# szhan227/text2protein

Hardware: AMD Instinct MI355X
Metric: 6D backbone samples/sec (128-res, 1000-step) (higher is better)
Workload: dtype f16; 1 GPU; cfg2: test_config.yml L=128 N=1000 chains/GPU=32 C=5 text_tokens=512 condition=none; step = 1 PC step (2 score evals + SDE updates); sample = 1000 PC steps; finite=True

## Files before the change

include/t2p.h:

```cpp
#ifndef T2P_H_
#define T2P_H_

#include <stdint.h>

#ifdef __cplusplus
extern "C" {
#endif

#define T2P_DTYPE_F32 0
#define T2P_DTYPE_BF16 1
#define T2P_DTYPE_F16 2

#define T2P_SDE_VE 0
#define T2P_SDE_VP 1
#define T2P_SDE_SUBVP 2

typedef struct t2p_model_config {
  int32_t num_channels;
  int32_t max_res_num;
  int32_t nf;
  int32_t num_res_blocks;
  int32_t n_ch_mult;
  int32_t ch_mult[8];
  int32_t n_attn_resolutions;
// ... 92 lines not shown
typedef struct t2p_train_config {
  double lr, beta1, eps, weight_decay;
  double warmup;
  double grad_clip;
  double ema_rate;
  double dropout;
  double t_eps;
  int32_t cond_flags;
  uint64_t seed;
} t2p_train_config;

typedef struct t2p_train_batch {
  const float* coords_6d;
  const uint8_t* mask_pair;
  const uint8_t* mask_inpaint;
  const float* context;
  int32_t batch, tokens;
  const float* t;
  const float* z;
} t2p_train_batch;

typedef struct t2p_trainer t2p_trainer;
int t2p_train_create(const t2p_model_config* model, const t2p_train_config* train, t2p_trainer** out);
void t2p_train_destroy(t2p_trainer* t);
int t2p_train_num_params(const t2p_trainer* t);
int t2p_train_param_info(const t2p_trainer* t, int i, const char** name, int64_t shape[4], int* ndim);
int t2p_train_load_param(t2p_trainer* t, const char* name, const float* host_data, const int64_t* shape, int ndim);
int t2p_train_read(t2p_trainer* t, int which, const char* name, float* host_out);
int t2p_train_write(t2p_trainer* t, int which, const char* name, const float* host_in);
int t2p_train_set_step(t2p_trainer* t, int64_t step, int64_t adam_updates, int64_t ema_updates);
int t2p_train_get_step(const t2p_trainer* t, int64_t out3[3]);
int t2p_train_set_sde(t2p_trainer* t, int sde, double beta_min, double beta_max, const float* std_table);
int t2p_train_set_ploss(t2p_trainer* t, int loss_type, int timesteps, const float* sqrt_alphas_cumprod,
                        const float* sqrt_one_minus_alphas_cumprod);
int t2p_train_set_dropout_masks(t2p_trainer* t, const uint8_t* const* device_masks, int n);
int t2p_train_set_ss_blocks(t2p_trainer* t, const int32_t* host_blocks, int n, const uint8_t* host_drop, double p);
int t2p_train_set_inpaint_draw(t2p_trainer* t, const int32_t* host_len_lo_hi, int B, double random_p, double contiguous_p);
int t2p_train_set_context_drop(t2p_trainer* t, const uint8_t* host_drop, int B, double p);
int t2p_train_loss(t2p_trainer* t, const t2p_train_batch* batch, int backward, float* loss_host, float* score_out, void* stream);
int t2p_train_step(t2p_trainer* t, const t2p_train_batch* batch, float* loss_host, void* stream);
int t2p_train_grad_buffer(t2p_trainer* t, float** device_ptr, int64_t* n);
int t2p_train_apply(t2p_trainer* t, void* stream);
int t2p_train_buffer(t2p_trainer* t, int which, float** device_ptr, int64_t* n);
int t2p_train_copy(t2p_trainer* t, int dst, int src, void* stream);
int t2p_engine_load_from_trainer(t2p_engine* e, t2p_trainer* t, int which, void* stream);
int t2p_train_eval_loss(t2p_trainer* t, const t2p_train_batch* batch, float* loss_host, void* stream);
int64_t t2p_train_device_bytes(const t2p_trainer* t);
int t2p_op_tgemm(const float* A, int64_t sAm, int64_t sAk, const float* B, int64_t sBk, int64_t sBn, float* C, int64_t ldc, int M, int N,
                 int K, int nz, int64_t sAz, int64_t sBz, int64_t sCz, float alpha, float beta, const float* bias_n, int ksplit, int conv,
                 int H, int W, int conv_C, void* stream);
int t2p_op_tgemm16(int dtype, const float* A, int64_t sAm, int64_t sAk, const float* B, int64_t sBk, int64_t sBn, float* C, int64_t ldc,
                   int M, int N, int K, int nz, int64_t sAz, int64_t sBz, int64_t sCz, float alpha, float beta, const float* bias_n, int ksplit,
                   int conv, int H, int W, int conv_C, void* stream);
int t2p_op_train_conv3x3(int dtype, const float* x, const float* w, const float* bias, const float* tbias, int batch, int H, int W, int Ci,
                         int Co, int Cip, int Cop, float* y, const float* dy, float* dx, float* dw, float* dbias, float* dtbias,
                         int fixed_order, void* stream);
int t2p_op_ss_block_dropout(const float* x, float* out, int batch, int C, int L, const int32_t* host_blocks, int n,
                            const uint8_t* host_drop, double p, uint64_t seed, uint64_t stream_id, uint8_t* drop_out_device, void* stream);
int t2p_op_inpaint_mask_draw(const int32_t* host_len_lo_hi, int B, int L, double random_p, double contiguous_p, uint64_t seed, uint64_t stream_id,
                             int force_mode, uint8_t* flags_out, uint8_t* pair_out, int* mode_out_host, void* stream);
int t2p_op_ploss_draw_t(uint64_t seed, uint64_t stream_id, int B, int timesteps, int32_t* out_dev, void* stream);
int t2p_op_context_drop(float* x, int batch, int64_t row_floats, const uint8_t* host_drop, double p, uint64_t seed, uint64_t stream_id,
                        uint8_t* drop_out_device, void* stream);
int t2p_op_groupnorm_backward(const float* x, const float* dy, const float* gamma, const float* beta, int silu, int batch, int HW, int C,
                              int groups, float eps, float* dx, float* dgamma, float* dbeta, void* stream);
int t2p_op_layernorm_backward(const float* x, const float* dy, const float* gamma, int64_t rows, int C, float eps, float* dx, float* dgamma,
                              float* dbeta, void* stream);
int t2p_op_groupnorm_backward_form(const float* x, const float* dy, const float* gamma, const float* beta, int silu, int batch, int HW,
                                   int C, int groups, float eps, float* dx, float* dgamma, float* dbeta, int fixed_order, void* stream);
int t2p_op_layernorm_backward_form(const float* x, const float* dy, const float* gamma, int64_t rows, int C, float eps, float* dx,
                                   float* dgamma, float* dbeta, int fixed_order, void* stream);
int t2p_op_colsum(const float* dy, int nz, int64_t rows_per_z, int N, int64_t ld, float* out, int64_t ld_out, int accumulate,
                  int fixed_order, void* stream);
int t2p_op_sumsq(const float* g, int64_t n, int fixed_order, double* result_host, void* stream);
int t2p_op_seed_scale(const float* x, int64_t n, float target, float* s2_host, void* stream);
int t2p_op_softmax_backward(const float* P, float* dP_inout, int64_t rows, int n, float scale, void* stream);
int t2p_op_geglu_backward(const float* u, const float* dy, float* du, int64_t rows, int inner, void* stream);

int t2p_op_gemm(int dtype, const void* A, int a_f32, const void* Bw, void* C, int c_f32, int M, int N, int K,
                int64_t lda, int64_t ldb, int64_t ldc, const float* bias_n, const float* residual, float alpha,
                void* stream);
int t2p_op_gemm_r16(int dtype, const void* A, int a_f32, const void* Bw, void* C, int c_f32, int M, int N, int K, int64_t lda,
                    int64_t ldb, int64_t ldc, const float* bias_n, const void* residual16, float alpha, void* stream);
int t2p_op_conv3x3(int dtype, const void* x, int a_f32, const void* w, const float* bias, float* out, int batch,
                   int H, int W, int Cin, int Cout, int upsample, void* stream);
int t2p_op_conv3x3_shortcut(int dtype, const void* a, const void* w, const float* bias, const void* x0, int CX0,
                            const void* x1, int CX1, float alpha, void* out, int c_f32, int batch, int H, int W, int C,
                            int Cout, void* stream);
int t2p_op_conv3x3_groupnorm(int dtype, const void* a, const void* w, const float* bias, const float* bias_bn, const void* residual,
                             float alpha, int upsample, int groups, const float* gamma, const float* beta, float eps, int silu,
                             void* out, int out_f32, void* normed, float* col_stats, int batch, int H, int W, int C, int Cout, void* stream);
int t2p_op_small_conv_groupnorm(int dtype, const void* a, const void* w, int64_t ldw, const void* x0, int CX0, const void* x1, int CX1,
                                const float* bias, const float* bias_bn, const void* residual, float alpha, void* out, int out_f32,
                                float* col_stats, void* normed, int groups, const float* gamma, const float* beta, float eps, int silu,
                                int batch, int H, int W, int C, int Cout, void* stream);
int t2p_op_st_entry(int dtype, const void* x, const float* col_stats, int groups, const float* gn_gamma, const float* gn_beta,
                    float gn_eps, const void* w_in, const float* b_in, const void* residual, const float* ln_gamma,
                    const float* ln_beta, float ln_eps, const void* w_2, int n2, const float* b_2, int geglu, void* t, void* out2,
                    const void* w_3, const float* b_3, const void* res3, void* y, float* y_stats, int batch, int n, int C,
                    void* stream);
int t2p_op_attn_proj(int dtype, const void* x, const float* col_stats, int groups, const float* gn_gamma, const float* gn_beta,
                     float gn_eps, const void* w_qk, const float* b_qk, const void* w_v, void* qk, void* vt, void* k_fm,
                     int64_t npad, int batch, int n, int C, void* stream);
int t2p_op_input_conv(const float* x, const float* w_tcn, const float* bias, void* out, int out_dtype, int batch, int C,
                      int H, int W, int nf, float* col_stats, void* stream);
int t2p_op_groupnorm(const float* x0, const float* x1, int C0, int C1, int batch, int H, int W, int groups,
                     const float* gamma, const float* beta, float eps, int silu, int down, void* out, int dtype,
                     void* stream);
int t2p_op_layernorm(const float* x, const float* gamma, const float* beta, void* out, int dtype, int64_t rows,
                     int C, float eps, void* stream);
int t2p_op_layernorm16(const void* x16, const float* gamma, const float* beta, void* out16, int dtype, int64_t rows, int C,
                       float eps, void* stream);
int t2p_op_softmax(const float* S, int64_t lds, void* P, int64_t ldp, int dtype, int64_t rows, int n, float scale,
                   void* stream);
int t2p_op_geglu(const float* u, void* out, int dtype, int64_t rows, int inner, void* stream);
int64_t t2p_op_attention_ws(int dtype, int batch, int heads, int nq, int nk);
int t2p_op_attention(int dtype, const void* q, int64_t ldq, const void* k, int64_t ldk, const void* vt,
                     int64_t ldvt, void* out, int batch, int heads, int nq, int nk, int d, float scale,
                     void* workspace, void* stream);
int t2p_op_attention_wide(int dtype, const void* q, int64_t ldq, const void* k, int64_t ldk, const void* vt, int64_t ldvt, void* out,
                          int out_f32, const float* bias, const void* residual, int residual_16bit, float alpha, float* col_stats,
                          int batch, int n, int d, float scale, void* stream);
int t2p_op_attention_wide_fm(int dtype, const void* q, int64_t ldq, const void* k_fm, const void* vt_fm, void* out, int out_f32,
                             const float* bias, const void* residual, int residual_16bit, float alpha, float* col_stats, int batch,
                             int n, int d, float scale, void* stream);
int t2p_op_gemm_frag_major(int dtype, const void* A, const void* Bw, void* C, void* c_frag, int M, int N, int K, int frag_col0,
                           int rows_per_batch, int batch, void* stream);
int t2p_op_attention_qkv(int dtype, const void* qkv, int64_t ld, void* out, int batch, int heads, int n, int d,
                         float scale, void* stream);
int t2p_op_langevin(const float* x, const float* grad, const float* noise, const uint8_t* mask,
                    const float* x_initial, float* x_out, float* x_mean_out, int batch, int64_t per_sample,
                    float snr, float alpha, float* sums_out , void* stream);
int t2p_op_langevin_norms(const float* grad, const float* noise, int batch, int64_t per_sample, float* workspace,
                          float* sums, void* stream);
int t2p_op_langevin_update(const float* x, const float* grad, const float* noise, const uint8_t* mask,
                           const float* x_initial, float* x_out, float* x_mean_out, int64_t n, const float* sums,
                           float batch_total, float snr, float alpha, void* stream);
int t2p_op_predictor(const float* x, const float* score, const float* noise, const uint8_t* mask,
                     const float* x_initial, float* x_out, float* x_mean_out, int64_t n, float G,
                     int probability_flow, void* stream);
int t2p_op_guided_langevin_norms(const float* o_c, const float* o_u, const float* noise, int batch, int64_t per_sample, float w, float w1,
                                 float scale, float* workspace, float* sums, void* stream);
int t2p_op_guided_langevin_update(const float* x, const float* o_c, const float* o_u, const float* noise, const uint8_t* mask,
                                  const float* x_initial, float* x_out, float* x_out2, float* x_mean_out, int64_t n, float w, float w1,
                                  float scale, const float* sums, float batch_total, float snr, float alpha, void* stream);
int t2p_op_guided_predictor(const float* x, const float* o_c, const float* o_u, const float* noise, const uint8_t* mask,
                            const float* x_initial, float* x_out, float* x_out2, float* x_mean_out, int64_t n, float w, float w1,
                            float scale, float G, float x_coef, int probability_flow, void* stream);
typedef struct t2p_inpaint_replace {
  const uint8_t* known;
  const float* data;
  const float* noise;
  const float* mean_table;
  const float* std_table;
  int32_t n_table;
  int32_t step;
  float mean_coef, std;
  uint64_t seed, stream_id;
} t2p_inpaint_replace;
int t2p_op_inpaint_langevin_update(const float* x, const float* o_c, const float* o_u, const float* noise, const uint8_t* mask,
                                   const float* x_initial, float* x_out, float* x_out2, float* x_mean_out, int64_t n, float w, float w1,
                                   float scale, const float* sums, float batch_total, float snr, float alpha,
                                   const t2p_inpaint_replace* replace, void* stream);
int t2p_op_inpaint_predictor(const float* x, const float* o_c, const float* o_u, const float* noise, const uint8_t* mask,
                             const float* x_initial, float* x_out, float* x_out2, float* x_mean_out, int64_t n, float w, float w1,
                             float scale, float G, float x_coef, int probability_flow, const t2p_inpaint_replace* replace, void* stream);
int t2p_op_philox_normal(float* out, int64_t n, uint64_t seed, uint64_t stream_id, void* stream);
int t2p_op_convert(const float* in, void* out, int dtype, int64_t n, void* stream);
int t2p_op_weight_pack(int kind, const float* src0, const float* src1, const float* src2, void* dst, const int64_t* dims, int ndims, int dtype,
                       void* stream);
int t2p_op_decode_6d(const float* x, int batch, int channels, int L, float* clipped, float* absval, int32_t* lengths, void* stream);
int t2p_op_encode_6d(const float* xyz, const int32_t* nres, const uint8_t* atom_ok, int batch, int channels, int L,
                     const int32_t* host_blocks, int n_blocks, float* coords_6d, uint8_t* mask_pair, void* stream);
int t2p_op_embedding_gather(const void* table, int table_dtype, const int32_t* ids, float* out, int64_t n_tokens, int dim, int vocab,
                            int32_t* bad_flag, void* stream);
int t2p_op_apply_mask(float* x, const uint8_t* mask, const float* x_initial, int64_t n, void* stream);

int t2p_profile_begin(void);
int t2p_debug_set(int key, int value);
int t2p_built_with_ablation(void);
int t2p_profile_end(double* out9);
int t2p_profile_dominant(double* out4, char* name, int name_len);
int t2p_profile_attention(double* out3);
int t2p_profile_shapes(char* buf, int len);
int t2p_profile_conv_kernels(char* buf, int len);
int t2p_debug_tap(int block_index, float* dst, int64_t capacity, int64_t* shape4);
int t2p_profile_layers_begin(void);
int t2p_profile_layers_end(char* buf, int len);

#ifdef __cplusplus
}
#endif
#endif
```

text2protein_amd/_lib.py:

```python
from __future__ import annotations

import ctypes as C

from . import build as _build

DT_F32, DT_BF16, DT_F16 = 0, 1, 2
DTYPE_NAMES = {"f32": DT_F32, "fp32": DT_F32, "float32": DT_F32, "bf16": DT_BF16, "bfloat16": DT_BF16,
               "f16": DT_F16, "fp16": DT_F16, "float16": DT_F16}
SDE_VE, SDE_VP, SDE_SUBVP = 0, 1, 2


class T2PError(RuntimeError):
    pass


class ModelConfig(C.Structure):
    _fields_ = [("num_channels", C.c_int32), ("max_res_num", C.c_int32), ("nf", C.c_int32),
                ("num_res_blocks", C.c_int32), ("n_ch_mult", C.c_int32), ("ch_mult", C.c_int32 * 8),
                ("n_attn_resolutions", C.c_int32), ("attn_resolutions", C.c_int32 * 8),
                ("n_heads", C.c_int32), ("context_dim", C.c_int32), ("num_scales", C.c_int32),
                ("sigma_min", C.c_double), ("sigma_max", C.c_double),
                ("skip_rescale", C.c_int32), ("scale_by_sigma", C.c_int32), ("compute_dtype", C.c_int32)]


# ... 16 lines not shown


class TrainConfig(C.Structure):
    _fields_ = [("lr", C.c_double), ("beta1", C.c_double), ("eps", C.c_double), ("weight_decay", C.c_double),
                ("warmup", C.c_double), ("grad_clip", C.c_double), ("ema_rate", C.c_double), ("dropout", C.c_double),
                ("t_eps", C.c_double), ("cond_flags", C.c_int32), ("seed", C.c_uint64)]


class TrainBatch(C.Structure):
    _fields_ = [("coords_6d", C.c_void_p), ("mask_pair", C.c_void_p), ("mask_inpaint", C.c_void_p), ("context", C.c_void_p),
                ("batch", C.c_int32), ("tokens", C.c_int32), ("t", C.c_void_p), ("z", C.c_void_p)]


class InpaintReplace(C.Structure):
    _fields_ = [("known", C.c_void_p), ("data", C.c_void_p), ("noise", C.c_void_p), ("mean_table", C.c_void_p),
                ("std_table", C.c_void_p), ("n_table", C.c_int32), ("step", C.c_int32), ("mean_coef", C.c_float), ("std", C.c_float),
                ("seed", C.c_uint64), ("stream_id", C.c_uint64)]


_vp, _i, _i64, _f, _u64 = C.c_void_p, C.c_int, C.c_int64, C.c_float, C.c_uint64

SIGNATURES = {
    "t2p_last_error": (C.c_char_p, []),
    "t2p_device_count": (_i, []),
    "t2p_engine_create": (_i, [C.POINTER(ModelConfig), C.POINTER(_vp)]),
    "t2p_engine_destroy": (None, [_vp]),
    "t2p_engine_num_params": (_i, [_vp]),
    "t2p_engine_param_info": (_i, [_vp, _i, C.POINTER(C.c_char_p), C.POINTER(_i64), C.POINTER(_i)]),
    "t2p_engine_load_param": (_i, [_vp, C.c_char_p, _vp, C.POINTER(_i64), _i]),
    "t2p_engine_finalize": (_i, [_vp]),
    "t2p_engine_load_flat": (_i, [_vp, _vp, _i64, _vp]),
    "t2p_engine_load_stats": (_i, [_vp, C.POINTER(_i64)]),
    "t2p_engine_set_context": (_i, [_vp, _vp, _i, _i, _vp]),
    "t2p_engine_score": (_i, [_vp, _vp, _vp, _vp, _i, _vp]),
    "t2p_engine_score_ex": (_i, [_vp, _vp, _vp, _vp, _vp, _i, _vp]),
    "t2p_engine_device_bytes": (_i64, [_vp]),
    "t2p_engine_pool_reclaimed": (_i, [_vp]),
    "t2p_sampler_create": (_i, [_vp, C.POINTER(SamplerConfig), _vp, _vp, C.POINTER(_vp)]),
    "t2p_sampler_set_seed": (_i, [_vp, _u64]),
    "t2p_sampler_set_norm_allreduce": (_i, [_vp, _vp, _vp, _vp]),
    "t2p_built_with_ablation": (_i, []),
    "t2p_sampler_destroy": (None, [_vp]),
    "t2p_sampler_set_condition": (_i, [_vp, _vp, _vp]),
    "t2p_sampler_reset": (_i, [_vp, _i, _vp]),
    "t2p_sampler_step": (_i, [_vp, _vp, _vp, _vp, _vp, _vp]),
    "t2p_sampler_step_graph": (_i, [_vp, _vp, _vp, _vp]),
    "t2p_sampler_run": (_i, [_vp, _vp, _vp, _i, _i, _vp]),
    "t2p_sampler_set_vp_tables": (_i, [_vp, _vp, _vp, _vp, _vp]),
    "t2p_sampler_count_dispatches": (_i, [_vp, _vp, _vp, _vp, C.POINTER(C.c_int)]),
    "t2p_sampler_set_guidance": (_i, [_vp, C.c_double, _i]),
    "t2p_sampler_set_context": (_i, [_vp, _vp, _i, _i, _vp]),
    "t2p_op_guided_langevin_norms": (_i, [_vp, _vp, _vp, _i, _i64, _f, _f, _f, _vp, _vp, _vp]),
    "t2p_op_guided_langevin_update": (_i, [_vp, _vp, _vp, _vp, _vp, _vp, _vp, _vp, _vp, _i64, _f, _f, _f, _vp, _f, _f, _f, _vp]),
    "t2p_op_guided_predictor": (_i, [_vp, _vp, _vp, _vp, _vp, _vp, _vp, _vp, _vp, _i64, _f, _f, _f, _f, _f, _i, _vp]),
    "t2p_sampler_set_inpaint": (_i, [_vp, _vp, _vp, _vp, _vp]),
    "t2p_sampler_set_inpaint_noise": (_i, [_vp, _vp, _vp]),
    "t2p_op_inpaint_langevin_update": (_i, [_vp, _vp, _vp, _vp, _vp, _vp, _vp, _vp, _vp, _i64, _f, _f, _f, _vp, _f, _f, _f,
                                            C.POINTER(InpaintReplace), _vp]),
    "t2p_op_inpaint_predictor": (_i, [_vp, _vp, _vp, _vp, _vp, _vp, _vp, _vp, _vp, _i64, _f, _f, _f, _f, _f, _i,
                                      C.POINTER(InpaintReplace), _vp]),
    "t2p_ddim_create": (_i, [_vp, C.POINTER(DdimConfig), C.POINTER(DdimStepRow), C.POINTER(_vp)]),
    "t2p_ddim_destroy": (None, [_vp]),
    "t2p_ddim_set_seed": (_i, [_vp, _u64]),
    "t2p_ddim_set_condition": (_i, [_vp, _vp, _vp]),
    "t2p_ddim_set_context": (_i, [_vp, _vp, _i, _i, _vp]),
    "t2p_ddim_reset": (_i, [_vp, _i, _vp]),
    "t2p_ddim_step": (_i, [_vp, _vp, _vp, _vp, _vp]),
    "t2p_ddim_run": (_i, [_vp, _vp, _vp, _i, _i, _vp]),
    "t2p_op_ddim_update": (_i, [_vp, _vp, _vp, _vp, _vp, _vp, _vp, _vp, _vp, _i64, _f, _f, _f, _f, _f, _f, _f, _i, _i, _u64, _u64, _vp]),
    "t2p_op_gemm": (_i, [_i, _vp, _i, _vp, _vp, _i, _i, _i, _i, _i64, _i64, _i64, _vp, _vp, _f, _vp]),
    "t2p_op_conv3x3_shortcut": (_i, [_i, _vp, _vp, _vp, _vp, _i, _vp, _i, _f, _vp, _i, _i, _i, _i, _i, _i, _vp]),
    "t2p_op_conv3x3_groupnorm": (_i, [_i, _vp, _vp, _vp, _vp, _vp, C.c_float, _i, _i, _vp, _vp, C.c_float, _i, _vp, _i, _vp, _vp,
                                      _i, _i, _i, _i, _i, _vp]),
    "t2p_op_attention_wide": (_i, [_i, _vp, _i64, _vp, _i64, _vp, _i64, _vp, _i, _vp, _vp, _i, _f, _vp, _i, _i, _i, _f, _vp]),
    "t2p_op_attention_wide_fm": (_i, [_i, _vp, _i64, _vp, _vp, _vp, _i, _vp, _vp, _i, _f, _vp, _i, _i, _i, _f, _vp]),
    "t2p_op_gemm_frag_major": (_i, [_i, _vp, _vp, _vp, _vp, _i, _i, _i, _i, _i, _i, _vp]),
    "t2p_op_small_conv_groupnorm": (_i, [_i, _vp, _vp, _i64, _vp, _i, _vp, _i, _vp, _vp, _vp, _f, _vp, _i, _vp, _vp, _i, _vp, _vp, _f, _i,
                                         _i, _i, _i, _i, _i, _vp]),
    "t2p_op_attn_proj": (_i, [_i, _vp, _vp, _i, _vp, _vp, _f, _vp, _vp, _vp, _vp, _vp, _vp, _i64, _i, _i, _i, _vp]),
    "t2p_op_st_entry": (_i, [_i, _vp, _vp, _i, _vp, _vp, _f, _vp, _vp, _vp, _vp, _vp, _f, _vp, _i, _vp, _i, _vp, _vp, _vp, _vp, _vp, _vp, _vp,
                             _i, _i, _i, _vp]),
    "t2p_op_input_conv": (_i, [_vp, _vp, _vp, _vp, _i, _i, _i, _i, _i, _i, _vp, _vp]),
    "t2p_op_gemm_r16": (_i, [_i, _vp, _i, _vp, _vp, _i, _i, _i, _i, _i64, _i64, _i64, _vp, _vp, _f, _vp]),
    "t2p_op_conv3x3": (_i, [_i, _vp, _i, _vp, _vp, _vp, _i, _i, _i, _i, _i, _i, _vp]),
    "t2p_op_groupnorm": (_i, [_vp, _vp, _i, _i, _i, _i, _i, _i, _vp, _vp, _f, _i, _i, _vp, _i, _vp]),
    "t2p_op_layernorm": (_i, [_vp, _vp, _vp, _vp, _i, _i64, _i, _f, _vp]),
    "t2p_op_layernorm16": (_i, [_vp, _vp, _vp, _vp, _i, _i64, _i, _f, _vp]),
    "t2p_op_softmax": (_i, [_vp, _i64, _vp, _i64, _i, _i64, _i, _f, _vp]),
    "t2p_op_geglu": (_i, [_vp, _vp, _i, _i64, _i, _vp]),
    "t2p_op_attention_ws": (_i64, [_i, _i, _i, _i, _i]),
    "t2p_op_attention_qkv": (_i, [_i, _vp, _i64, _vp, _i, _i, _i, _i, _f, _vp]),
    "t2p_op_attention": (_i, [_i, _vp, _i64, _vp, _i64, _vp, _i64, _vp, _i, _i, _i, _i, _i, _f, _vp, _vp]),
    "t2p_op_langevin": (_i, [_vp, _vp, _vp, _vp, _vp, _vp, _vp, _i, _i64, _f, _f, _vp, _vp]),
    "t2p_op_langevin_norms": (_i, [_vp, _vp, _i, _i64, _vp, _vp, _vp]),
    "t2p_op_langevin_update": (_i, [_vp, _vp, _vp, _vp, _vp, _vp, _vp, _i64, _vp, _f, _f, _f, _vp]),
    "t2p_op_apply_mask": (_i, [_vp, _vp, _vp, _i64, _vp]),
    "t2p_op_predictor": (_i, [_vp, _vp, _vp, _vp, _vp, _vp, _vp, _i64, _f, _i, _vp]),
    "t2p_op_philox_normal": (_i, [_vp, _i64, _u64, _u64, _vp]),
    "t2p_profile_begin": (_i, []),
    "t2p_debug_set": (_i, [_i, _i]),
    "t2p_op_decode_6d": (_i, [_vp, _i, _i, _i, _vp, _vp, _vp, _vp]),
    "t2p_op_encode_6d": (_i, [_vp, _vp, _vp, _i, _i, _i, _vp, _i, _vp, _vp, _vp]),
    "t2p_op_embedding_gather": (_i, [_vp, _i, _vp, _vp, _i64, _i, _i, _vp, _vp]),
    "t2p_profile_end": (_i, [C.POINTER(C.c_double)]),
    "t2p_profile_dominant": (_i, [C.POINTER(C.c_double), C.c_char_p, C.c_int]),
    "t2p_profile_attention": (_i, [C.POINTER(C.c_double)]),
    "t2p_profile_shapes": (_i, [C.c_char_p, C.c_int]),
    "t2p_profile_conv_kernels": (_i, [C.c_char_p, C.c_int]),
    "t2p_debug_tap": (_i, [_i, _vp, C.c_int64, C.POINTER(C.c_int64)]),
    "t2p_profile_layers_begin": (_i, []),
    "t2p_profile_layers_end": (_i, [C.c_char_p, C.c_int]),
    "t2p_op_convert": (_i, [_vp, _vp, _i, _i64, _vp]),
    "t2p_op_weight_pack": (_i, [_i, _vp, _vp, _vp, _vp, C.POINTER(_i64), _i, _i, _vp]),
    "t2p_train_create": (_i, [C.POINTER(ModelConfig), C.POINTER(TrainConfig), C.POINTER(_vp)]),
    "t2p_train_destroy": (None, [_vp]),
    "t2p_train_num_params": (_i, [_vp]),
    "t2p_train_param_info": (_i, [_vp, _i, C.POINTER(C.c_char_p), C.POINTER(_i64), C.POINTER(_i)]),
    "t2p_train_load_param": (_i, [_vp, C.c_char_p, _vp, C.POINTER(_i64), _i]),
    "t2p_train_read": (_i, [_vp, _i, C.c_char_p, _vp]),
    "t2p_train_write": (_i, [_vp, _i, C.c_char_p, _vp]),
    "t2p_train_set_step": (_i, [_vp, _i64, _i64, _i64]),
    "t2p_train_get_step": (_i, [_vp, C.POINTER(_i64)]),
    "t2p_train_set_sde": (_i, [_vp, _i, C.c_double, C.c_double, _vp]),
    "t2p_train_set_ploss": (_i, [_vp, _i, _i, _vp, _vp]),
    "t2p_train_set_dropout_masks": (_i, [_vp, C.POINTER(_vp), _i]),
    "t2p_train_set_ss_blocks": (_i, [_vp, _vp, _i, _vp, C.c_double]),
    "t2p_train_set_inpaint_draw": (_i, [_vp, _vp, _i, C.c_double, C.c_double]),
    "t2p_train_set_context_drop": (_i, [_vp, _vp, _i, C.c_double]),
    "t2p_train_loss": (_i, [_vp, C.POINTER(TrainBatch), _i, C.POINTER(_f), _vp, _vp]),
    "t2p_train_step": (_i, [_vp, C.POINTER(TrainBatch), C.POINTER(_f), _vp]),
    "t2p_train_eval_loss": (_i, [_vp, C.POINTER(TrainBatch), C.POINTER(_f), _vp]),
    "t2p_train_apply": (_i, [_vp, _vp]),
    "t2p_train_grad_buffer": (_i, [_vp, C.POINTER(_vp), C.POINTER(_i64)]),
    "t2p_train_buffer": (_i, [_vp, _i, C.POINTER(_vp), C.POINTER(_i64)]),
    "t2p_train_copy": (_i, [_vp, _i, _i, _vp]),
    "t2p_engine_load_from_trainer": (_i, [_vp, _vp, _i, _vp]),
    "t2p_train_device_bytes": (_i64, [_vp]),
    "t2p_op_tgemm": (_i, [_vp, _i64, _i64, _vp, _i64, _i64, _vp, _i64, _i, _i, _i, _i, _i64, _i64, _i64, _f, _f, _vp, _i, _i, _i, _i, _i, _vp]),
    "t2p_op_tgemm16": (_i, [_i, _vp, _i64, _i64, _vp, _i64, _i64, _vp, _i64, _i, _i, _i, _i, _i64, _i64, _i64, _f, _f, _vp, _i, _i, _i, _i, _i,
                            _vp]),
    "t2p_op_train_conv3x3": (_i, [_i, _vp, _vp, _vp, _vp, _i, _i, _i, _i, _i, _i, _i, _vp, _vp, _vp, _vp, _vp, _vp, _i, _vp]),
    "t2p_op_ss_block_dropout": (_i, [_vp, _vp, _i, _i, _i, _vp, _i, _vp, C.c_double, _u64, _u64, _vp, _vp]),
    "t2p_op_inpaint_mask_draw": (_i, [_vp, _i, _i, C.c_double, C.c_double, _u64, _u64, _i, _vp, _vp, C.POINTER(_i), _vp]),
    "t2p_op_context_drop": (_i, [_vp, _i, _i64, _vp, C.c_double, _u64, _u64, _vp, _vp]),
    "t2p_op_ploss_draw_t": (_i, [_u64, _u64, _i, _i, _vp, _vp]),
    "t2p_op_groupnorm_backward": (_i, [_vp, _vp, _vp, _vp, _i, _i, _i, _i, _i, _f, _vp, _vp, _vp, _vp]),
    "t2p_op_layernorm_backward": (_i, [_vp, _vp, _vp, _i64, _i, _f, _vp, _vp, _vp, _vp]),
    "t2p_op_groupnorm_backward_form": (_i, [_vp, _vp, _vp, _vp, _i, _i, _i, _i, _i, _f, _vp, _vp, _vp, _i, _vp]),
    "t2p_op_layernorm_backward_form": (_i, [_vp, _vp, _vp, _i64, _i, _f, _vp, _vp, _vp, _i, _vp]),
    "t2p_op_colsum": (_i, [_vp, _i, _i64, _i, _i64, _vp, _i64, _i, _i, _vp]),
    "t2p_op_sumsq": (_i, [_vp, _i64, _i, C.POINTER(C.c_double), _vp]),
    "t2p_op_seed_scale": (_i, [_vp, _i64, _f, C.POINTER(_f), _vp]),
    "t2p_op_softmax_backward": (_i, [_vp, _vp, _i64, _i, _f, _vp]),
    "t2p_op_geglu_backward": (_i, [_vp, _vp, _vp, _i64, _i, _vp]),
}

_lib = None


def lib_path() -> str:
    return _build.LIB


ALLREDUCE_FN = C.CFUNCTYPE(C.c_int, C.c_void_p, C.c_void_p, C.c_void_p)


def load_path(path):
    global _lib
    if _lib is not None:
        raise T2PError("load_path() must come before any other use of the library")
    lib = C.CDLL(path)
    for name, (res, args) in SIGNATURES.items():
        fn = getattr(lib, name, None)
        if fn is None:
            continue
        fn.restype = res
        fn.argtypes = args
    _lib = lib
    return lib


def load_ablation():
    global _lib
# ... 56 lines not shown
```

text2protein_amd/build.py:

```python
from __future__ import annotations

import hashlib
import os
import re
import subprocess
import sys

CSRC = os.path.join(os.path.dirname(os.path.abspath(__file__)), "csrc")
LIB = os.path.join(CSRC, "libt2p_hip.so")
LIB_ABLATION = os.path.join(CSRC, "libt2p_hip_ablation.so")
SOURCES = ["gemm.hip", "kernels.hip", "attention.hip", "smallconv.hip", "stfuse.hip", "ddim.hip", "weightpack.hip", "engine.cpp", "sampler.cpp", "capi.cpp",
           "train_kernels.hip", "train.cpp", "train_capi.cpp"]
GEMM_PARTS = 7
HEADERS = ["t2p_common.h", "t2p_kernels.h", "philox.h", "update_loop.h", "engine.h", "sampler.h", "ddim.h", "train_kernels.h", "train.h", os.path.join("..", "..", "include", "t2p.h")]
ARCH = "gfx950"


def _hipcc():
    for c in (os.environ.get("HIPCC"), "/opt/rocm/bin/hipcc", "hipcc"):
        if c and (os.path.isabs(c) and os.path.exists(c) or not os.path.isabs(c)):
            return c
    raise RuntimeError("hipcc not found")


STAMP = LIB + ".srchash"
FLAGS = ["-O3", "-std=c++17", "-fPIC", f"--offload-arch={ARCH}", "-Wall", "-Wno-unused-function"]
_COMPILER_ID = None


def compiler_id() -> str:
    global _COMPILER_ID
    if _COMPILER_ID is None:
        try:
            _COMPILER_ID = subprocess.run([_hipcc(), "--version"], capture_output=True, text=True, timeout=60).stdout.strip()
        except (OSError, RuntimeError, subprocess.SubprocessError):
            _COMPILER_ID = ""
    return _COMPILER_ID


def source_hash(ablation: bool = False) -> str:
    h = hashlib.sha256()
    h.update(" ".join(FLAGS + (["-DT2P_ABLATION"] if ablation else [])).encode())
    h.update(compiler_id().encode())
    for f in SOURCES + HEADERS:
        h.update(f.encode())
        with open(os.path.join(CSRC, f), "rb") as fh:
            h.update(fh.read())
    return h.hexdigest()


def unit_hash(src: str, flags) -> str:
    h = hashlib.sha256()
    h.update(" ".join(flags).encode())
    h.update(compiler_id().encode())
    seen, todo = [], [os.path.join(CSRC, src)]
    while todo:
        f = os.path.normpath(todo.pop())
        if f in seen or not os.path.exists(f):
            continue
        seen.append(f)
        with open(f, "rb") as fh:
            data = fh.read()
        h.update(os.path.relpath(f, CSRC).encode())
        h.update(data)
        for inc in re.findall(rb'^\s*#\s*include\s+"([^"]+)"', data, re.M):
            todo.append(os.path.join(os.path.dirname(f), inc.decode()))
    return h.hexdigest()


def _read(path) -> str:
    try:
        with open(path) as f:
            return f.read().strip()
    except OSError:
        return ""


def built_hash() -> str:
    return _read(STAMP)


def needs_build() -> bool:
    return not os.path.exists(LIB) or built_hash() != source_hash()


def scratch_users(remarks: str, kernel_prefix: str = "_kernel"):
    bad, name = [], None
    for line in remarks.splitlines():
        m = re.search(r"Function Name: (\S+)", line)
        if m:
            name = m.group(1)
        m = re.search(r"ScratchSize \[bytes/lane\]: (\d+)", line)
        if m and name and kernel_prefix in name and int(m.group(1)) > 0:
            bad.append((name, int(m.group(1))))
    return bad


# ... 79 lines not shown
```

text2protein_amd/csrc/capi.cpp:

```cpp
#include <new>

#include "ddim.h"
#include "engine.h"
#include "sampler.h"
#include "train.h"

using namespace t2p;

#define API_BEGIN try {
#define API_END                                        \
  }                                                    \
  catch (const std::bad_alloc&) {                      \
    set_last_error("out of host memory");              \
    return T2P_ERR_STATE;                              \
  }                                                    \
  catch (const std::exception& ex) {                   \
    set_last_error(std::string("exception: ") + ex.what()); \
    return T2P_ERR_STATE;                              \
  }

namespace t2p { extern bool g_pre_conv_mfma, g_gn_apply_cols; void layer_profile_begin(); int layer_profile_end(std::string* out);
void debug_tap_set(int index, float* dst, long capacity); void debug_tap_shape(long out[4]); }
extern "C" {

// ... 211 lines not shown

int t2p_sampler_run(t2p_sampler* s, float* x, float* out, int prior_given, int n_steps, void* stream) {
  API_BEGIN
  T2P_REQUIRE(s, "null sampler");
  return s->impl.run(x, out, prior_given, n_steps, (hipStream_t)stream);
  API_END
}

int t2p_ddim_create(t2p_engine* e, const t2p_ddim_config* cfg, const t2p_ddim_step_row* table, t2p_ddim** out) {
  API_BEGIN
  T2P_REQUIRE(e && cfg && out, "null argument");
  t2p_ddim* d = new t2p_ddim(&e->impl, *cfg);
  int rc = d->impl.init(table);
  if (rc != T2P_OK) {
    delete d;
    return rc;
  }
  *out = d;
  return T2P_OK;
  API_END
}

void t2p_ddim_destroy(t2p_ddim* d) { delete d; }

int t2p_ddim_set_seed(t2p_ddim* d, uint64_t seed) {
  API_BEGIN
  T2P_REQUIRE(d, "null ddim sampler");
  d->impl.set_seed(seed);
  return T2P_OK;
  API_END
}

int t2p_ddim_set_condition(t2p_ddim* d, const uint8_t* mask, const float* x_initial) {
  API_BEGIN
  T2P_REQUIRE(d, "null ddim sampler");
  T2P_REQUIRE((mask == nullptr) == (x_initial == nullptr), "mask and x_initial go together");
  return d->impl.set_condition(mask, x_initial);
  API_END
}

int t2p_ddim_set_context(t2p_ddim* d, const float* context, int batch, int tokens, void* stream) {
  API_BEGIN
  T2P_REQUIRE(d, "null ddim sampler");
  return d->impl.set_context(context, batch, tokens, (hipStream_t)stream);
  API_END
}

int t2p_ddim_reset(t2p_ddim* d, int step, void* stream) {
  API_BEGIN
  T2P_REQUIRE(d, "null ddim sampler");
  (void)stream;
  return d->impl.reset(step);
  API_END
}

int t2p_ddim_step(t2p_ddim* d, float* x, float* x0_out, const float* noise, void* stream) {
  API_BEGIN
  T2P_REQUIRE(d, "null ddim sampler");
  return d->impl.step(x, x0_out, noise, (hipStream_t)stream);
  API_END
}

int t2p_ddim_run(t2p_ddim* d, float* x, float* out, int prior_given, int n_steps, void* stream) {
  API_BEGIN
  T2P_REQUIRE(d, "null ddim sampler");
  return d->impl.run(x, out, prior_given, n_steps, (hipStream_t)stream);
  API_END
}

int t2p_op_ddim_update(const float* x, const float* eps_c, const float* eps_u, const float* z, const uint8_t* mask,
                       const float* x_initial, float* x_out, float* x_out2, float* x0_out, int64_t n, float w, float w1,
                       float sqrt_recip, float sqrt_recipm1, float sqrt_an, float c, float sigma, int clip, int last,
                       uint64_t seed, uint64_t stream_id, void* stream) {
  API_BEGIN
  DdimUpdateArgs a;
  a.x = x; a.eps_c = eps_c; a.eps_u = eps_u; a.z = z; a.mask = mask; a.x_initial = x_initial;
  a.x_out = x_out; a.x_out2 = x_out2; a.x0_out = x0_out; a.n = n; a.w = w; a.w1 = w1;
  a.sqrt_recip = sqrt_recip; a.sqrt_recipm1 = sqrt_recipm1; a.sqrt_an = sqrt_an; a.c = c; a.sigma = sigma;
  a.clip = clip; a.last = last; a.seed = seed; a.stream_id = stream_id;
  return launch_ddim_update(a, (hipStream_t)stream);
  API_END
}

int t2p_op_gemm(int dtype, const void* A, int a_f32, const void* Bw, void* C, int c_f32, int M, int N, int K, int64_t lda,
                int64_t ldb, int64_t ldc, const float* bias_n, const float* residual, float alpha, void* stream) {
  API_BEGIN
  GemmParams p;
  p.dtype = dtype; p.A0 = A; p.a_f32 = a_f32; p.C0 = K; p.lda0 = lda; p.Bw = Bw; p.ldb = ldb; p.M = M; p.N = N;
  p.bias_n = bias_n; p.R = residual; p.ldr = ldc; p.alpha = alpha; p.C = C; p.c_f32 = c_f32; p.ldc = ldc;
  return launch_gemm(p, (hipStream_t)stream);
  API_END
}

static void* g_op_ws = nullptr;
static size_t g_op_ws_bytes = 0, g_op_ws_alloc = 0;
static int attach_op_ws(GemmParams& p) {
  if (!g_op_ws_bytes) return T2P_OK;
  if (g_op_ws_alloc < g_op_ws_bytes) {
    if (g_op_ws) { T2P_HIP_CHECK(hipDeviceSynchronize()); T2P_HIP_CHECK(hipFree(g_op_ws)); g_op_ws = nullptr; g_op_ws_alloc = 0; }
    T2P_HIP_CHECK(hipMalloc(&g_op_ws, g_op_ws_bytes));
    g_op_ws_alloc = g_op_ws_bytes;
  }
  p.ws = g_op_ws; p.ws_bytes = g_op_ws_bytes;
  return T2P_OK;
}

int t2p_op_gemm_r16(int dtype, const void* A, int a_f32, const void* Bw, void* C, int c_f32, int M, int N, int K, int64_t lda,
                    int64_t ldb, int64_t ldc, const float* bias_n, const void* residual16, float alpha, void* stream) {
  API_BEGIN
  GemmParams p;
  p.dtype = dtype; p.A0 = A; p.a_f32 = a_f32; p.C0 = K; p.lda0 = lda; p.Bw = Bw; p.ldb = ldb; p.M = M; p.N = N;
  p.bias_n = bias_n; p.R = (const float*)residual16; p.r_lowp = 1; p.ldr = ldc; p.alpha = alpha; p.C = C; p.c_f32 = c_f32; p.ldc = ldc;
  T2P_TRY(attach_op_ws(p));
  return launch_gemm(p, (hipStream_t)stream);
  API_END
}

int t2p_op_conv3x3(int dtype, const void* x, int a_f32, const void* w, const float* bias, float* out, int batch, int H,
                   int W, int Cin, int Cout, int upsample, void* stream) {
  API_BEGIN
  GemmParams p;
  p.dtype = dtype; p.A0 = x; p.a_f32 = a_f32; p.C0 = Cin; p.lda0 = Cin; p.taps = 9; p.H = H; p.W = W; p.a_up = upsample;
  p.Bw = w; p.ldb = 9L * Cin; p.M = batch * H * W; p.N = Cout; p.bias_n = bias; p.rows_per_batch = H * W;
  p.C = out; p.c_f32 = 1; p.ldc = Cout;
  T2P_TRY(attach_op_ws(p));
  return launch_gemm(p, (hipStream_t)stream);
  API_END
}

int t2p_op_conv3x3_shortcut(int dtype, const void* a, const void* w, const float* bias, const void* x0, int CX0, const void* x1,
                            int CX1, float alpha, void* out, int c_f32, int batch, int H, int W, int C, int Cout, void* stream) {
  API_BEGIN
  GemmParams p;
  p.dtype = dtype; p.A0 = a; p.a_f32 = 0; p.C0 = C; p.lda0 = C; p.taps = 9; p.H = H; p.W = W;
  p.Bw = w; p.ldb = 9L * C + CX0 + CX1; p.M = batch * H * W; p.N = Cout; p.bias_n = bias; p.rows_per_batch = H * W;
  p.alpha = alpha; p.C = out; p.c_f32 = c_f32; p.ldc = Cout;
  T2P_TRY(attach_op_ws(p));
  T2P_REQUIRE(gemm_can_fuse_shortcut(p), "this convolution does not take the shortcut segment (LDS-DMA 3x3 convolutions only)");
  p.X0 = x0; p.CX0 = CX0; p.ldx0 = CX0; p.X1 = x1; p.CX1 = CX1; p.ldx1 = CX1;
  return launch_gemm(p, (hipStream_t)stream);
  API_END
}

int t2p_op_conv3x3_groupnorm(int dtype, const void* a, const void* w, const float* bias, const float* bias_bn, const void* residual,
                             float alpha, int upsample, int groups, const float* gamma, const float* beta, float eps, int silu,
                             void* out, int out_f32, void* normed, float* col_stats, int batch, int H, int W, int C, int Cout, void* stream) {
  API_BEGIN
  GemmParams p;
  p.dtype = dtype; p.A0 = a; p.a_f32 = 0; p.C0 = C; p.lda0 = C; p.taps = 9; p.H = H; p.W = W; p.a_up = upsample;
  p.Bw = w; p.ldb = 9L * C; p.M = batch * H * W; p.N = Cout; p.bias_n = bias; p.rows_per_batch = H * W;
  p.bias_bn = bias_bn; p.ld_bn = Cout;
  p.R = (const float*)residual; p.r_lowp = residual ? 1 : 0; p.ldr = Cout;
  p.alpha = alpha; p.C = out; p.c_f32 = out_f32; p.ldc = Cout; p.col_stats = col_stats;
  T2P_TRY(attach_op_ws(p));
  T2P_REQUIRE(gemm_fuses_post_gn(p, groups), "this convolution does not take the split-K plan whose second pass applies a GroupNorm");
  p.gn_gamma = gamma; p.gn_beta = beta; p.gn_groups = groups; p.gn_silu = silu; p.gn_eps = eps; p.gn_out = normed;
  return launch_gemm(p, (hipStream_t)stream);
  API_END
}

int t2p_op_small_conv_groupnorm(int dtype, const void* a, const void* w, int64_t ldw, const void* x0, int CX0, const void* x1, int CX1,
                                const float* bias, const float* bias_bn, const void* residual, float alpha, void* out, int out_f32,
                                float* col_stats, void* normed, int groups, const float* gamma, const float* beta, float eps, int silu,
                                int batch, int H, int W, int C, int Cout, void* stream) {
  API_BEGIN
  SmallConvArgs s;
  s.dtype = dtype; s.A = a; s.B = batch; s.H = H; s.W = W; s.C = C; s.N = Cout; s.Wt = w; s.ldw = ldw;
  s.X0 = x0; s.CX0 = CX0; s.X1 = x1; s.CX1 = CX1; s.bias = bias; s.bias_bn = bias_bn; s.ld_bn = Cout; s.R = residual; s.alpha = alpha;
  s.out = out; s.out_f32 = out_f32; s.col_stats = col_stats; s.normed = normed; s.gn_gamma = gamma; s.gn_beta = beta; s.groups = groups;
  s.gn_silu = silu; s.gn_eps = eps;
  return launch_small_conv_gn(s, (hipStream_t)stream);
  API_END
}

int t2p_op_st_entry(int dtype, const void* x, const float* col_stats, int groups, const float* gn_gamma, const float* gn_beta, float gn_eps,
                    const void* w_in, const float* b_in, const void* residual, const float* ln_gamma, const float* ln_beta, float ln_eps,
                    const void* w_qkv, int n2, const float* b2, int geglu, void* t, void* qkv, const void* w3, const float* b3,
                    const void* res3, void* y, float* y_stats, int batch, int n, int C, void* stream) {
  API_BEGIN
  StEntryArgs e;
  e.dtype = dtype; e.B = batch; e.n = n; e.C = C; e.x = x; e.cstats = col_stats; e.groups = groups; e.gn_gamma = gn_gamma;
  e.gn_beta = gn_beta; e.gn_eps = gn_eps; e.w_in = w_in; e.b_in = b_in; e.ln_gamma = ln_gamma; e.ln_beta = ln_beta; e.ln_eps = ln_eps;
  e.w_qkv = w_qkv; e.n2 = n2; e.b2 = b2; e.geglu = geglu; e.res = residual; e.t = t; e.qkv = qkv;
  e.w3 = w3; e.b3 = b3; e.res3 = res3; e.y = y; e.y_stats = y_stats;
  T2P_REQUIRE(st_entry_eligible(e), "st_entry: C = 256 (or 512 without geglu), n2 in {C, 3 C} (8 C with geglu), 16-bit dtype, n % 32 == 0 (64 with column sums), batch n <= 8192");
  void* fm = nullptr;
  T2P_HIP_CHECK(hipMalloc(&fm, ((size_t)C * C + (size_t)n2 * C + (w3 ? (size_t)5 * C * C : 0)) * 2));
  void* fm2 = (char*)fm + (size_t)C * C * 2;
  void* fm3 = (char*)fm2 + (size_t)n2 * C * 2;
  int rc = launch_sf_frag_major(dtype, w_in, fm, C, C, (hipStream_t)stream);
  if (rc == T2P_OK) rc = launch_sf_frag_major(dtype, w_qkv, fm2, n2, C, (hipStream_t)stream);
  if (rc == T2P_OK && w3) rc = launch_sf_frag_major(dtype, w3, fm3, C, 5 * C, (hipStream_t)stream);
  if (rc == T2P_OK && w3 && y_stats && hipMemsetAsync(y_stats, 0, (size_t)batch * n / 64 * C * 2 * 4, (hipStream_t)stream) != hipSuccess) rc = T2P_ERR_HIP;
  e.w_in = fm; e.w_qkv = fm2;
  if (w3) e.w3 = fm3;
  if (rc == T2P_OK) rc = launch_st_entry(e, (hipStream_t)stream);
// ... 325 lines not shown
  a.x = x; a.noise = noise; a.mask = mask; a.x_initial = x_initial; a.x_out = x_out; a.x_mean_out = x_mean_out; a.n = n;
  GuidedScore g;
  g.o_c = o_c; g.o_u = o_u; g.w = w; g.w1 = w1; g.scale = scale;
  InpaintReplace r;
  int* counter = nullptr;
  int rc = op_inpaint_replace(replace, &r, &counter, s);
  if (rc == T2P_OK) rc = launch_predictor_update(a, g, x_out2, nullptr, G, probability_flow, s, nullptr, x_coef, &r);
  return op_inpaint_done(rc, counter, s);
  API_END
}

int t2p_op_philox_normal(float* out, int64_t n, uint64_t seed, uint64_t stream_id, void* stream) {
  API_BEGIN
  return launch_philox_normal(out, n, seed, stream_id, nullptr, (hipStream_t)stream);
  API_END
}

int t2p_op_convert(const float* in, void* out, int dtype, int64_t n, void* stream) {
  API_BEGIN
  return launch_convert(in, out, dtype, n, (hipStream_t)stream);
  API_END
}

int t2p_op_decode_6d(const float* x, int batch, int channels, int L, float* clipped, float* absval, int32_t* lengths, void* stream) {
  API_BEGIN
  return launch_decode6d(x, batch, channels, L, clipped, absval, lengths, (hipStream_t)stream);
  API_END
}

int t2p_op_encode_6d(const float* xyz, const int32_t* nres, const uint8_t* atom_ok, int batch, int channels, int L,
                     const int32_t* host_blocks, int n_blocks, float* coords_6d, uint8_t* mask_pair, void* stream) {
  API_BEGIN
  T2P_REQUIRE(xyz && nres && coords_6d && mask_pair && batch > 0 && L > 0, "encode_6d arguments");
  T2P_REQUIRE(channels == 5 || channels == 8, "encode_6d: the channel count must be 5 or 8, not " + std::to_string(channels));
  T2P_REQUIRE(n_blocks >= 0 && (n_blocks == 0 || host_blocks), "encode_6d: block list arguments");
  T2P_REQUIRE(n_blocks == 0 || channels == 8, "encode_6d: secondary-structure blocks need the 8-channel layout");
  T2P_REQUIRE((long)L * L < (1L << 30) && batch <= 65535, "encode_6d: map or batch too large");
  hipStream_t s = (hipStream_t)stream;
  std::vector<int32_t> n((size_t)batch);
  T2P_HIP_CHECK(hipMemcpyAsync(n.data(), nres, (size_t)batch * 4, hipMemcpyDeviceToHost, s));
  T2P_HIP_CHECK(hipStreamSynchronize(s));
  for (int b = 0; b < batch; ++b)
    T2P_REQUIRE(n[b] >= 1 && n[b] <= L, "encode_6d: nres[" + std::to_string(b) + "] = " + std::to_string(n[b]) + " is outside [1, " + std::to_string(L) + "]");
  std::vector<std::vector<int32_t>> of_sample((size_t)batch);
  for (int k = 0; k < n_blocks; ++k) {
    const int32_t* q = host_blocks + 4 * (size_t)k;
    const std::string name = "encode_6d: block " + std::to_string(k);
    T2P_REQUIRE(q[0] >= 0 && q[0] < batch, name + " names a sample outside the batch");
    T2P_REQUIRE(q[1] <= q[2], name + " starts after its last residue");
    T2P_REQUIRE(q[1] >= 0 && q[2] < n[q[0]], name + " lies outside the " + std::to_string(n[q[0]]) + " residues of its sample");
    T2P_REQUIRE(q[3] == 0 || q[3] == 1, name + " is neither a helix (0) nor a strand (1)");
    of_sample[q[0]].push_back(k);
  }
  if (n_blocks == 0) return launch_encode6d(xyz, nres, atom_ok, batch, channels, L, nullptr, nullptr, 0, coords_6d, mask_pair, s);
  std::vector<int32_t> up(host_blocks, host_blocks + 4 * (size_t)n_blocks);
  for (const auto& ks : of_sample)
    for (int32_t k1 : ks)
      for (int32_t k2 : ks) { up.push_back(k1); up.push_back(k2); }
  const size_t npairs = (up.size() - 4 * (size_t)n_blocks) / 2;
  T2P_REQUIRE(npairs < (1u << 30), "encode_6d: too many block pairs");
  struct Scratch {
    int32_t* p = nullptr; hipStream_t s;
    ~Scratch() { if (p) { (void)hipStreamSynchronize(s); (void)hipFree(p); } }
  } dev;
  dev.s = s;
  T2P_HIP_CHECK(hipMalloc(&dev.p, up.size() * 4));
  T2P_HIP_CHECK(hipMemcpyAsync(dev.p, up.data(), up.size() * 4, hipMemcpyHostToDevice, s));
  return launch_encode6d(xyz, nres, atom_ok, batch, channels, L, dev.p, dev.p + 4 * (size_t)n_blocks, (int)npairs, coords_6d, mask_pair, s);
  API_END
}

int t2p_op_embedding_gather(const void* table, int table_dtype, const int32_t* ids, float* out, int64_t n_tokens, int dim, int vocab,
                            int32_t* bad_flag, void* stream) {
  API_BEGIN
  return launch_embedding_gather(table, table_dtype, ids, out, n_tokens, dim, vocab, bad_flag, (hipStream_t)stream);
  API_END
}

int t2p_op_apply_mask(float* x, const uint8_t* mask, const float* x_initial, int64_t n, void* stream) {
  API_BEGIN
  return launch_apply_mask(x, mask, x_initial, n, (hipStream_t)stream);
  API_END
}

int t2p_debug_set(int key, int value) {
  if (key == 10) { g_op_ws_bytes = (size_t)value << 20; return T2P_OK; }
  if (key == 11) { set_gemm_force_nsplit(value); return T2P_OK; }
  if (key == 12) { set_gemm_midsplit(value != 0); return T2P_OK; }
  if (key == 13) { g_gn_small = value != 0; return T2P_OK; }
  if (key == 14) { g_lowp_residual = value != 0; return T2P_OK; }
  if (key == 15) { set_gemm_thin_conv(value != 0); return T2P_OK; }
  if (key == 17) { g_gn_apply16 = value != 0; return T2P_OK; }
  if (key == 20) { g_layernorm16 = value != 0; return T2P_OK; }
  if (key == 21) { set_gemm_up4(value != 0); return T2P_OK; }
  if (key == 22) { set_gemm_deep_ring(value != 0); return T2P_OK; }
  if (key == 23) { set_gemm_fuse_shortcut(value != 0); return T2P_OK; }
  if (key == 25) { g_qkv_fused = value != 0; return T2P_OK; }
  if (key == 26) { t2p::g_pre_conv_mfma = value != 0; return T2P_OK; }
  if (key == 27) { t2p::g_gn_apply_cols = value != 0; return T2P_OK; }
  if (key == 28) { set_gemm_post_gn(value != 0); return T2P_OK; }
  if (key == 29) { t2p::g_attn_strip = value != 0; return T2P_OK; }
  if (key == 36) { t2p::g_small_conv = value != 0; return T2P_OK; }
  if (key == 38) { t2p::g_pre_conv_split = value != 0; return T2P_OK; }
  if (key == 39) { t2p::g_st_fuse = value != 0; return T2P_OK; }
  if (key == 40) { t2p::g_st_tail = value != 0; return T2P_OK; }
  if (key == 41) { t2p::g_small_conv_fm = value != 0; return T2P_OK; }
  if (key == 42) { t2p::g_st_ffpo = value != 0; return T2P_OK; }
  if (key == 43) { t2p::g_st_tail_rows = value; return T2P_OK; }
  if (key == 45) { t2p::g_attn_fm = value != 0; return T2P_OK; }
  if (key == 46) { t2p::g_attn_proj = value != 0; return T2P_OK; }
  if (key == 47) { set_gemm_dxs(value != 0); return T2P_OK; }
  if (key == 48) { t2p::g_train_plumbing16 = value != 0; return T2P_OK; }
  if (key == 34) { set_gemm_a_norm(value != 0); return T2P_OK; }
  if (key == 32) { g_attn_merged = value != 0; return T2P_OK; }
  if (key == 33) { g_ffpo_merged = value != 0; return T2P_OK; }
  if (key == 30) { set_gemm_split_consts(value, 0); return T2P_OK; }
  if (key == 31) { set_gemm_split_consts(0, value); return T2P_OK; }
  if (key == 0) set_gemm_dma(value != 0);
  else if (key == 1) {
#ifndef T2P_ABLATION
    if (value & ~(128 | 256 | 4096 | 8192)) {
      set_last_error("ablation bits that skip work exist only in a -DT2P_ABLATION build");
      return T2P_ERR_INVALID;
    }
#endif
    set_gemm_debug(value);
  }
  else if (key == 2) set_gemm_geom(value);
  else if (key == 3) set_gemm_splitk(value != 0);
  else if (key == 4) g_raw_copies = value != 0;
  else if (key == 5) g_flash_attention = value != 0;
  else if (key == 6) g_fuse_gn_stats = value != 0;
  else if (key == 7) g_fuse_geglu = value != 0;
  else if (key == 8) set_gemm_ring(value);
  else if (key == 9) g_lowp_h1 = value != 0;
  else return T2P_ERR_INVALID;
  return T2P_OK;
}

#ifdef T2P_ABLATION
extern "C" int t2p_ablation_dxs_stamps(unsigned long long* out, int n) { return t2p::dxs_stamps_read(out, n); }
#endif

int t2p_built_with_ablation(void) {
#ifdef T2P_ABLATION
  return 1;
#else
  return 0;
#endif
}

int t2p_profile_begin(void) {
  profile_begin();
  return T2P_OK;
}

int t2p_profile_end(double* out9) {
  API_BEGIN
  T2P_REQUIRE(out9, "null argument");
  double o[3][3];
  T2P_TRY(profile_end(o));
  for (int k = 0; k < 3; ++k)
    for (int j = 0; j < 3; ++j) out9[k * 3 + j] = o[k][j];
  return T2P_OK;
  API_END
}

int t2p_profile_attention(double* out3) {
  API_BEGIN
  T2P_REQUIRE(out3, "null argument");
  return profile_attention(out3);
  API_END
}

int t2p_profile_shapes(char* buf, int len) {
  API_BEGIN
  T2P_REQUIRE(buf && len > 0, "null argument");
  return profile_shapes(buf, len);
  API_END
}

int t2p_profile_conv_kernels(char* buf, int len) {
  API_BEGIN
  T2P_REQUIRE(buf && len > 0, "null argument");
  return profile_conv_kernels(buf, len);
  API_END
}

int t2p_debug_tap(int block_index, float* dst, int64_t capacity, int64_t* shape4) {
  API_BEGIN
  if (shape4) {
    long sh[4];
    t2p::debug_tap_shape(sh);
    for (int i = 0; i < 4; ++i) shape4[i] = sh[i];
  }
// ... 33 lines not shown
```

text2protein_amd/csrc/engine.cpp:

```cpp
#include "engine.h"

#include <algorithm>
#include <cmath>
#include <cstdio>
#include <cstring>
#include <map>
#include <mutex>
#include <thread>

namespace t2p {

bool g_fuse_gn_stats = true;
bool g_fuse_geglu = true;
bool g_lowp_h1 = true;
bool g_gn_small = true;
bool g_lowp_residual = true;
bool g_raw_copies = true;
bool g_flash_attention = true;
bool g_attn_merged = true;
bool g_ffpo_merged = true;
bool g_qkv_fused = true;
static thread_local std::string g_last_error;
void set_last_error(const std::string& msg) { g_last_error = msg; }
const char* get_last_error() { return g_last_error.c_str(); }
// ... 406 lines not shown
              for (int64_t n = 0; n < co; ++n)
                for (int64_t c = 0; c < ci; ++c)
                  m[((ph * co + n) * 4 + tap) * ci + c] += s[0][(((size_t)n * ci + c) * 3 + kh) * 3 + kw];
            }
      break;
    }
    case WP_ADD:
      m.resize((size_t)d[0]);
      for (int64_t i = 0; i < d[0]; ++i) m[i] = s[0][i] + s[1][i];
      break;
    case WP_PRODUCT: {
      const int64_t M = d[0], K = d[1], N = d[2];
      m = host_matmul(s[0], s[1], M, K, N);
      if (s[2])
        for (int64_t i = 0; i < M; ++i)
          for (int64_t n = 0; n < N; ++n) m[i * N + n] += s[2][n];
      if (d[3]) {
        std::vector<float> t((size_t)M * N);
        for (int64_t i = 0; i < M; ++i)
          for (int64_t n = 0; n < N; ++n) t[n * M + i] = m[i * N + n];
        m.swap(t);
      }
      break;
    }
    case WP_DOT64: {
      const int64_t N = d[0], K = d[1];
      m.resize((size_t)N);
      for (int64_t n = 0; n < N; ++n) {
        double acc = s[2][n];
        for (int64_t j = 0; j < K; ++j) acc += (double)s[0][n * K + j] * s[1][j];
        m[n] = (float)acc;
      }
      break;
    }
  }
}

int Engine::dest(void** slot, size_t bytes) {
  if (!*slot) *slot = pool_.persistent(bytes);
  return *slot ? T2P_OK : T2P_ERR_HIP;
}

const float* Engine::psrc(const std::string& name, int64_t numel) {
  auto it = poff_.find(name);
  if (it == poff_.end() || it->second.second != numel) {
    set_last_error((it == poff_.end() ? "no parameter " : "unexpected shape for ") + name);
    return nullptr;
  }
  if (flat_) return flat_ + it->second.first;
  auto h = host_.find(name);
  if (h == host_.end() || (int64_t)h->second.data.size() != numel) {
    set_last_error("parameter not loaded: " + name);
    return nullptr;
  }
  return h->second.data.data();
}
#define T2P_SRC(var, name, numel)                         \
  const float* var = psrc((name), (int64_t)(numel));      \
  if (!var) return T2P_ERR_STATE;

int Engine::pack(int kind, void* dst, int64_t off, int dtype, std::initializer_list<const float*> srcs, std::initializer_list<int64_t> dims) {
  WeightPack p;
  p.kind = kind; p.dtype = dtype; p.dst = (char*)dst + (size_t)off * dtype_size(dtype);
  int i = 0;
  for (const float* s : srcs) p.src[i++] = s;
  i = 0;
  for (int64_t d : dims) p.d[i++] = d;
  int64_t rows = 0, width = 0, ld = 0, rd = 0, wr = 0;
  T2P_TRY(weight_pack_shape(p, &rows, &width, &ld));
  weight_pack_bytes(p, rows, width, &rd, &wr);
  load_stats_[0] += rd; load_stats_[1] += wr; load_stats_[2] += 1;
  if (flat_) return launch_weight_pack(p, pack_stream_);
  std::vector<float> m;
  weight_pack_host(p, &m);
  return upload_block(m, dtype, p.dst, rows, width, ld);
}

int Engine::pack_frag(void** slot, const void* w, int N, int K) {
  T2P_TRY(dest(slot, (size_t)N * K * 2));
  load_stats_[0] += (int64_t)N * K * 2; load_stats_[1] += (int64_t)N * K * 2; load_stats_[2] += 1;
  return launch_sf_frag_major(cfg_.compute_dtype, w, *slot, N, K, pack_stream_);
}

int Engine::pack_linear(const std::string& wname, const std::string& bname, int N, int K, DevLinear* out, bool conv3x3, bool nin,
                        int force_dtype, int cin_pad) {
  const int dt = force_dtype >= 0 ? force_dtype : cfg_.compute_dtype;
  const int ci = K / 9, cp = cin_pad ? cin_pad : ci;
  const int Kd = conv3x3 ? 9 * cp : K;
  T2P_SRC(w, wname, (int64_t)N * K);
  T2P_TRY(dest(&out->w, (size_t)N * Kd * dtype_size(dt)));
  if (conv3x3) T2P_TRY(pack(WP_CONV3, out->w, 0, dt, {w}, {N, ci, cp, 0}));
  else if (nin) T2P_TRY(pack(WP_NIN, out->w, 0, dt, {w}, {K, N, 1}));
  else T2P_TRY(pack(WP_COPY, out->w, 0, dt, {w}, {(int64_t)N * K}));
  out->N = N;
  out->K = Kd;
  if (!bname.empty()) {
    T2P_SRC(b, bname, N);
    T2P_TRY(dest((void**)&out->b, (size_t)N * 4));
    T2P_TRY(pack(WP_COPY, out->b, 0, DT_F32, {b}, {N}));
  }
  return T2P_OK;
}

int Engine::pack_stack2(const std::string& w0, const std::string& b0, const std::string& w1, const std::string& b1,
                        int N, int K, bool nin, bool has_bias, DevLinear* out) {
  const int dt = cfg_.compute_dtype;
  T2P_SRC(t0, w0, (int64_t)N * K);
  T2P_SRC(t1, w1, (int64_t)N * K);
  T2P_TRY(dest(&out->w, (size_t)2 * N * K * dtype_size(dt)));
  if (nin) T2P_TRY(pack(WP_NIN, out->w, 0, dt, {t0, t1}, {K, N, 2}));
  else T2P_TRY(pack(WP_COPY, out->w, 0, dt, {t0, t1}, {(int64_t)N * K, (int64_t)N * K}));
  out->N = 2 * N;
  out->K = K;
  if (has_bias) {
    T2P_SRC(c0, b0, N);
    T2P_SRC(c1, b1, N);
    T2P_TRY(dest((void**)&out->b, (size_t)2 * N * 4));
    T2P_TRY(pack(WP_COPY, out->b, 0, DT_F32, {c0, c1}, {N, N}));
  }
  return T2P_OK;
}

int Engine::pack_norm(const std::string& prefix, int C, int G, DevNorm* out) {
  T2P_SRC(g, prefix + ".weight", C);
  T2P_SRC(b, prefix + ".bias", C);
  T2P_TRY(dest((void**)&out->gamma, (size_t)C * 4));
  T2P_TRY(dest((void**)&out->beta, (size_t)C * 4));
  T2P_TRY(pack(WP_COPY, out->gamma, 0, DT_F32, {g}, {C}));
  T2P_TRY(pack(WP_COPY, out->beta, 0, DT_F32, {b}, {C}));
  out->C = C;
  out->G = G;
  return T2P_OK;
}

int Engine::pack_weights() {
  load_stats_[0] = load_stats_[1] = load_stats_[2] = 0;
  const int td = arch_.temb_dim, dt = cfg_.compute_dtype, nf = arch_.nf, Cx = cfg_.num_channels;
  const size_t es = dtype_size(dt);
  T2P_TRY(pack_linear("pre_blocks.0.weight", "pre_blocks.0.bias", td, nf, &pre0_, false, false, DT_F32));
  T2P_TRY(pack_linear("pre_blocks.1.weight", "pre_blocks.1.bias", td, td, &pre1_, false, false, DT_F32));
  T2P_TRY(pack_linear("pre_conv.weight", "pre_conv.bias", nf, 9 * Cx, &pre_conv_, true, false, DT_F32, cpad_));
  {
    T2P_SRC(w, "pre_conv.weight", (int64_t)nf * Cx * 9);
    T2P_TRY(dest((void**)&pre_conv_direct_, (size_t)9 * Cx * nf * 4));
    T2P_TRY(pack(WP_CONV3_T, pre_conv_direct_, 0, DT_F32, {w}, {nf, Cx}));
    if (dt != DT_F32 && (Cx == 5 || Cx == 8) && cfg_.sigma_max <= 4096.0) {
      T2P_TRY(dest(&pre_conv_split_, pre_conv_split_weight_bytes(Cx, nf)));
      T2P_TRY(launch_pre_conv_split_weights(pre_conv_direct_, pre_conv_split_, Cx, nf, pack_stream_));
      load_stats_[0] += (int64_t)9 * Cx * nf * 4; load_stats_[1] += (int64_t)pre_conv_split_weight_bytes(Cx, nf); load_stats_[2] += 1;
    }
  }
  T2P_TRY(dest(&dense_all_.w, (size_t)arch_.temb_total * td * 4));
  T2P_TRY(dest((void**)&dense_all_.b, (size_t)arch_.temb_total * 4));
  dense_all_.N = arch_.temb_total;
  dense_all_.K = td;
  auto each_layer = [&](auto&& fn) -> int {
    for (Stage& st : arch_.input_stages) for (Layer& l : st.layers) T2P_TRY(fn(l));
    for (Layer& l : arch_.mid_stage.layers) T2P_TRY(fn(l));
    for (Stage& st : arch_.out_stages) for (Layer& l : st.layers) T2P_TRY(fn(l));
    return T2P_OK;
  };
  T2P_TRY(each_layer([&](Layer& l) -> int {
    const std::string& p = l.prefix;
    const int ci = l.in_ch, co = l.out_ch;
    if (l.kind == 0) {
      T2P_TRY(pack_norm(p + ".GroupNorm_0", ci, gn_groups(ci), &l.gn0));
// ... 12 lines not shown
        T2P_SRC(b1, p + ".Conv_1.bias", co);
        T2P_SRC(b2, p + ".Conv_2.bias", co);
        const int64_t K1 = (int64_t)9 * co, Kx = K1 + ci;
        T2P_TRY(dest(&l.conv1x.w, (size_t)co * Kx * es));
        T2P_TRY(dest((void**)&l.conv1x.b, (size_t)co * 4));
        T2P_TRY(pack(WP_CONV3, l.conv1x.w, 0, dt, {w1}, {co, co, co, Kx}));
        T2P_TRY(pack(WP_ROWS, l.conv1x.w, K1, dt, {w2}, {co, ci, Kx}));
        T2P_TRY(pack(WP_ADD, l.conv1x.b, 0, DT_F32, {b1, b2}, {co}));
        l.conv1x.N = co; l.conv1x.K = (int)Kx;
      }
      T2P_SRC(w, p + ".Dense_0.weight", (int64_t)co * td);
      T2P_SRC(b, p + ".Dense_0.bias", co);
      T2P_TRY(pack(WP_COPY, dense_all_.w, (int64_t)l.temb_off * td, DT_F32, {w}, {(int64_t)co * td}));
      T2P_TRY(pack(WP_COPY, dense_all_.b, l.temb_off, DT_F32, {b}, {co}));
      if (l.fm_conv0) {
        const DevLinear& c1 = l.has_conv2 ? l.conv1x : l.conv1;
        T2P_TRY(pack_frag(&l.fm_conv0, l.conv0.w, co, l.conv0.K));
        T2P_TRY(pack_frag(&l.fm_conv1, c1.w, co, c1.K));
      }
    } else if (l.kind == 1) {
      T2P_TRY(pack_norm(p + ".GroupNorm_0", ci, gn_groups(ci), &l.gn0));
      T2P_TRY(pack_stack2(p + ".NIN_0.W", p + ".NIN_0.b", p + ".NIN_1.W", p + ".NIN_1.b", ci, ci, true, true, &l.qk));
      T2P_TRY(pack_linear(p + ".NIN_2.W", p + ".NIN_2.b", ci, ci, &l.v, false, true));
      T2P_TRY(pack_linear(p + ".NIN_3.W", p + ".NIN_3.b", ci, ci, &l.out, false, true));
      if (dt != DT_F32) {
        T2P_SRC(w2, p + ".NIN_2.W", (int64_t)ci * ci);
        T2P_SRC(w3, p + ".NIN_3.W", (int64_t)ci * ci);
        T2P_SRC(b2, p + ".NIN_2.b", ci);
        T2P_SRC(b3, p + ".NIN_3.b", ci);
        T2P_TRY(dest(&l.v3.w, (size_t)ci * ci * es));
        T2P_TRY(dest((void**)&l.v3.b, (size_t)ci * 4));
        T2P_TRY(pack(WP_PRODUCT, l.v3.w, 0, dt, {w2, w3}, {ci, ci, ci, 1, 0}));
        T2P_TRY(pack(WP_PRODUCT, l.v3.b, 0, DT_F32, {b2, w3, b3}, {1, ci, ci, 0, 0}));
        l.v3.N = ci; l.v3.K = ci;
        if (ci == 256 && l.qk.w && l.qk.b) {
          T2P_TRY(pack_frag(&l.fm_qk, l.qk.w, 2 * ci, ci));
          T2P_TRY(pack_frag(&l.fm_v3, l.v3.w, ci, ci));
        }
      }
    } else {
      const std::string t = p + ".transformer_blocks.0";
      const int ctx = cfg_.context_dim;
      T2P_TRY(pack_norm(p + ".norm", ci, 32, &l.gn0));
      T2P_TRY(pack_linear(p + ".proj_in.weight", p + ".proj_in.bias", ci, ci, &l.proj_in));
      T2P_TRY(pack_linear(p + ".proj_out.weight", p + ".proj_out.bias", ci, ci, &l.proj_out));
      T2P_TRY(pack_stack2(t + ".attn1.to_q.weight", "", t + ".attn1.to_k.weight", "", ci, ci, false, false, &l.a1_qk));
      T2P_TRY(pack_linear(t + ".attn1.to_v.weight", "", ci, ci, &l.a1_v));
      if (dt != DT_F32) {
        const int64_t cc = (int64_t)ci * ci;
        T2P_SRC(wq, t + ".attn1.to_q.weight", cc);
        T2P_SRC(wk, t + ".attn1.to_k.weight", cc);
        T2P_SRC(wv, t + ".attn1.to_v.weight", cc);
        T2P_TRY(dest(&l.a1_qkv.w, (size_t)3 * cc * es));
        T2P_TRY(pack(WP_COPY, l.a1_qkv.w, 0, dt, {wq, wk, wv}, {cc, cc, cc}));
        l.a1_qkv.N = 3 * ci; l.a1_qkv.K = ci; l.a1_qkv.b = nullptr;
      }
      T2P_TRY(pack_linear(t + ".attn1.to_out.0.weight", t + ".attn1.to_out.0.bias", ci, ci, &l.a1_out));
      T2P_TRY(pack_linear(t + ".attn2.to_q.weight", "", ci, ci, &l.a2_q));
      T2P_TRY(pack_linear(t + ".attn2.to_k.weight", "", ci, ctx, &l.a2_k));
      T2P_TRY(pack_linear(t + ".attn2.to_v.weight", "", ci, ctx, &l.a2_v));
      T2P_TRY(pack_linear(t + ".attn2.to_out.0.weight", t + ".attn2.to_out.0.bias", ci, ci, &l.a2_out));
      {
        const int64_t inner = 4 * ci;
        T2P_SRC(w, t + ".ff.net.0.proj.weight", 2 * inner * ci);
        T2P_SRC(b, t + ".ff.net.0.proj.bias", 2 * inner);
        T2P_TRY(dest(&l.ff1.w, (size_t)2 * inner * ci * es));
        T2P_TRY(dest((void**)&l.ff1.b, (size_t)2 * inner * 4));
        T2P_TRY(pack(WP_GEGLU, l.ff1.w, 0, dt, {w}, {inner, ci}));
        T2P_TRY(pack(WP_GEGLU, l.ff1.b, 0, DT_F32, {b}, {inner, 1}));
        l.ff1.N = 8 * ci;
        l.ff1.K = ci;
      }
      T2P_TRY(pack_linear(t + ".ff.net.2.weight", t + ".ff.net.2.bias", ci, 4 * ci, &l.ff2));
      if (dt != DT_F32 && ci == 256 && l.a1_qkv.w) {
        T2P_TRY(pack_frag(&l.fm_in, l.proj_in.w, ci, ci));
        T2P_TRY(pack_frag(&l.fm_qkv, l.a1_qkv.w, 3 * ci, ci));
        T2P_TRY(pack_frag(&l.fm_out1, l.a1_out.w, ci, ci));
        T2P_TRY(pack_frag(&l.fm_q2, l.a2_q.w, ci, ci));
        if (ci == 256) {
          T2P_TRY(pack_frag(&l.fm_out2, l.a2_out.w, ci, ci));
          T2P_TRY(pack_frag(&l.fm_ff1, l.ff1.w, 8 * ci, ci));
        }
      }
      if (dt != DT_F32 && ci % 64 == 0) {
        T2P_SRC(wpo, p + ".proj_out.weight", (int64_t)ci * ci);
        T2P_SRC(bpo, p + ".proj_out.bias", ci);
        T2P_SRC(wf, t + ".ff.net.2.weight", (int64_t)ci * 4 * ci);
        T2P_SRC(bf, t + ".ff.net.2.bias", ci);
        T2P_TRY(dest(&l.ffpo.w, (size_t)ci * 5 * ci * es));
        T2P_TRY(dest((void**)&l.ffpo.b, (size_t)ci * 4));
        T2P_TRY(pack(WP_PRODUCT, l.ffpo.w, 0, dt, {wpo, wf}, {ci, ci, 4 * ci, 0, 5 * ci}));
        T2P_TRY(pack(WP_ROWS, l.ffpo.w, 4 * ci, dt, {wpo}, {ci, ci, 5 * ci}));
        T2P_TRY(pack(WP_DOT64, l.ffpo.b, 0, DT_F32, {wpo, bf, bpo}, {ci, ci}));
        l.ffpo.N = ci; l.ffpo.K = 5 * ci;
        if (ci == 256 && l.fm_in) T2P_TRY(pack_frag(&l.fm_ffpo, l.ffpo.w, ci, 5 * ci));
      }
      T2P_TRY(pack_norm(t + ".norm1", ci, 1, &l.ln1));
      T2P_TRY(pack_norm(t + ".norm2", ci, 1, &l.ln2));
      T2P_TRY(pack_norm(t + ".norm3", ci, 1, &l.ln3));
    }
    return T2P_OK;
  }));
  T2P_TRY(pack_norm("out.0", arch_.final_ch, gn_groups(arch_.final_ch), &head_norm_));
  T2P_TRY(pack_linear("out.2.weight", "out.2.bias", Cx, 9 * arch_.final_ch, &head_conv_, true));

  if (!inv_sigma_) {
    const int N = cfg_.num_scales;
    std::vector<float> inv(N);
    const double a = std::log(cfg_.sigma_max), b = std::log(cfg_.sigma_min);
    for (int i = 0; i < N; ++i) {
      const double s = std::exp(a + (b - a) * (double)i / (double)(N - 1));
      inv[i] = (float)(1.0 / s);
    }
    T2P_TRY(dest((void**)&inv_sigma_, (size_t)N * 4));
    T2P_TRY(dest((void**)&unit_scale_, (size_t)N * 4));
    T2P_TRY(upload_block(inv, DT_F32, inv_sigma_, 1, N, N));
    T2P_TRY(upload_block(std::vector<float>(N, 1.f), DT_F32, unit_scale_, 1, N, N));
  }
  return T2P_OK;
}

int Engine::finalize() {
  T2P_REQUIRE(!finalized_, "engine already finalized");
  for (const ParamInfo& p : arch_.params) {
    if (!host_.count(p.name)) {
      set_last_error("parameter not loaded: " + p.name);
      return T2P_ERR_STATE;
    }
  }
  flat_ = nullptr;
  pack_stream_ = nullptr;
  T2P_TRY(pack_weights());
  T2P_HIP_CHECK(hipStreamSynchronize(nullptr));
  host_.clear();
  finalized_ = true;
  return T2P_OK;
}

int Engine::load_flat(const float* device_flat, int64_t n, hipStream_t s) {
  T2P_REQUIRE(device_flat, "load_flat: null buffer");
  T2P_REQUIRE(n == total_, "load_flat: n must equal the element count of the engine's parameter table (" + std::to_string(total_) + ")");
  int dev = -1;
  T2P_HIP_CHECK(hipGetDevice(&dev));
  T2P_REQUIRE(dev == device_, "load_flat: the engine lives on device " + std::to_string(device_) + ", the current device is " + std::to_string(dev));
  flat_ = device_flat;
  pack_stream_ = s;
  const int rc = pack_weights();
  flat_ = nullptr;
  pack_stream_ = nullptr;
  T2P_TRY(rc);
  host_.clear();
  finalized_ = true;
  ctx_B_ = 0;
  return T2P_OK;
}

int Engine::attach_ws(GemmParams& p) {
  if (!splitk_ws_) {
    splitk_ws_bytes_ = (size_t)256 << 20;
    splitk_ws_ = pool_.persistent(splitk_ws_bytes_);
    if (!splitk_ws_) return T2P_ERR_HIP;
  }
  p.ws = splitk_ws_;
  p.ws_bytes = splitk_ws_bytes_;
  return T2P_OK;
}

int Engine::gemm(GemmParams& p, hipStream_t s) {
  T2P_TRY(attach_ws(p));
  return launch_gemm(p, s);
}

int Engine::gemm_stats(GemmParams& p, float** cstats, hipStream_t s) {
  *cstats = nullptr;
  T2P_TRY(attach_ws(p));
  if (g_fuse_gn_stats && (gemm_fuses_col_stats(p) || gemm_fuses_col_stats_lowp(p))) {
    *cstats = (float*)pool_.get((size_t)(p.M / 64) * p.N * 2 * 4);
    if (!*cstats) return T2P_ERR_HIP;
    p.col_stats = *cstats;
  }
  return gemm(p, s);
}

int Engine::linear(const void* a, bool a_is_f32, const DevLinear& w, long rows, void* c, bool c_f32,
                   const float* residual, float alpha, hipStream_t s, bool use_bias, float** cstats, bool r_lowp) {
  GemmParams p;
  p.dtype = dtype();
  p.A0 = a; p.a_f32 = a_is_f32 || p.dtype == DT_F32; p.C0 = w.K; p.lda0 = w.K;
  p.Bw = w.w; p.ldb = w.K;
  p.M = (int)rows; p.N = w.N;
  p.bias_n = use_bias ? w.b : nullptr;
  p.R = residual; p.ldr = w.N; p.r_lowp = (residual && r_lowp) ? 1 : 0;
  p.alpha = alpha;
  p.C = c; p.c_f32 = c_f32; p.ldc = w.N;
  if (cstats) return gemm_stats(p, cstats, s);
  return gemm(p, s);
}

int Engine::group_norm(const Act& x, const Act* x1, const DevNorm& n, float eps, int silu, int down, int B, void** out,
                       hipStream_t s, void** raw_out) {
  const int C = x.C + (x1 ? x1->C : 0);
  T2P_REQUIRE(C == n.C, "GroupNorm channel mismatch");
  T2P_REQUIRE(!x1 || x1->lowp == x.lowp, "concatenated sources must share a storage type");
  T2P_REQUIRE(!x.lowp || dtype() != DT_F32, "16-bit activations exist in the 16-bit modes only");
  if (x.pre_norm && !x1 && x.pre_for == &n && x.pre_silu == silu && !down && !raw_out) {
    *out = x.pre_norm;
    x.pre_norm = nullptr;
    return T2P_OK;
  }
  {
    GroupNormApplyArgs g;
    g.x0 = (const float*)x.p; g.x1 = x1 ? (const float*)x1->p : nullptr; g.C0 = x.C; g.C1 = x1 ? x1->C : 0;
    g.B = B; g.H = x.H; g.W = x.W; g.G = n.G; g.gamma = n.gamma; g.beta = n.beta; g.silu = silu; g.down = down;
    g.dtype = dtype(); g.x0_lowp = x.lowp; g.eps = eps;
    if (g_gn_small && gn_small_eligible(g)) {
      const size_t bytes = (size_t)B * x.H * x.W * C * dtype_size(dtype());
      POOL_GET(o, void*, bytes);
      g.out = o;
      if (raw_out) {
        *raw_out = pool_.get(bytes);
        if (!*raw_out) return T2P_ERR_HIP;
        g.raw_out = *raw_out;
      }
      T2P_TRY(launch_gn_small(g, s));
      *out = o;
      return T2P_OK;
    }
  }
  GroupNormArgs a;
  a.x0 = x.p; a.x1 = x1 ? x1->p : nullptr; a.C0 = x.C; a.C1 = x1 ? x1->C : 0;
  a.B = B; a.HW = x.H * x.W; a.G = n.G; a.eps = eps;
  const bool have_cols = x.cstats && (!x1 || x1->cstats) && a.HW % 64 == 0;
  if (have_cols && !raw_out) {
    GroupNormApplyArgs g;
    g.x0 = a.x0; g.x1 = a.x1; g.C0 = a.C0; g.C1 = a.C1; g.B = B; g.H = x.H; g.W = x.W; g.G = n.G;
    g.gamma = n.gamma; g.beta = n.beta; g.silu = silu; g.down = down; g.dtype = dtype(); g.x0_lowp = x.lowp;
    g.cs0 = x.cstats; g.cs1 = x1 ? x1->cstats : nullptr; g.eps = eps;
    if (gn_apply_cols_eligible(g)) {
      POOL_GET(o, void*, (size_t)B * a.HW * C * dtype_size(dtype()));
      g.out = o;
      T2P_TRY(launch_gn_apply_cols(g, s));
      *out = o;
      return T2P_OK;
    }
  }
  const int nparts = gn_num_chunks(a.HW) * ((C + 1023) / 1024);
  POOL_GET(stats, float*, (size_t)B * n.G * 2 * 4);
  float* partial = nullptr;
  if (have_cols) {
    T2P_TRY(launch_gn_finalize_cols(x.cstats, x1 ? x1->cstats : nullptr, a.C0, a.C1, B, a.HW, n.G, eps, stats, s));
  } else {
    partial = (float*)pool_.get((size_t)B * nparts * n.G * 2 * 4);
    if (!partial) return T2P_ERR_HIP;
    a.partial = partial; a.stats = stats;
    a.lowp_dtype = x.lowp ? dtype() : DT_F32;
    T2P_TRY(launch_gn_stats(a, s));
  }
  GroupNormApplyArgs g;
  g.x0 = a.x0; g.x1 = a.x1; g.C0 = a.C0; g.C1 = a.C1; g.B = B; g.H = x.H; g.W = x.W; g.G = n.G;
  g.stats = stats; g.gamma = n.gamma; g.beta = n.beta; g.silu = silu; g.down = down; g.dtype = dtype();
  g.x0_lowp = x.lowp;
  const size_t opix = (size_t)B * (down ? x.H / 2 : x.H) * (down ? x.W / 2 : x.W);
  POOL_GET(o, void*, opix * C * dtype_size(dtype()));
  g.out = o;
  if (raw_out) {
    *raw_out = pool_.get(opix * C * dtype_size(dtype()));
    if (!*raw_out) return T2P_ERR_HIP;
    g.raw_out = *raw_out;
  }
  T2P_TRY(launch_gn_apply(g, s));
  pool_.put(partial);
  pool_.put(stats);
// ... 399 lines not shown
    StEntryArgs e;
    e.dtype = dt; e.B = B; e.n = n; e.C = C;
    const bool normed = x.pre_norm && x.pre_for == &L.gn0 && x.pre_silu == 0;
    e.x = normed ? x.pre_norm : (const void*)x.p;
    e.cstats = normed ? nullptr : x.cstats;
    e.gn_gamma = L.gn0.gamma; e.gn_beta = L.gn0.beta; e.groups = L.gn0.G; e.gn_eps = 1e-6f;
    e.w_in = L.fm_in; e.b_in = L.proj_in.b;
    e.ln_gamma = L.ln1.gamma; e.ln_beta = L.ln1.beta; e.ln_eps = 1e-5f;
    e.w_qkv = L.fm_qkv; e.n2 = 3 * C;
    void* a_small = nullptr;
    if (!normed && !x.cstats && L.proj_in.b && L.fm_in && g_st_fuse) {
      StEntryArgs probe = e;
      probe.x = x.p; probe.cstats = nullptr;
      if (st_entry_eligible(probe)) {
        T2P_TRY(group_norm(x, nullptr, L.gn0, 1e-6f, 0, 0, B, &a_small, s));
        e.x = a_small; e.cstats = nullptr;
      }
    }
    if ((normed || x.cstats || a_small) && L.proj_in.b && L.fm_in && st_entry_eligible(e)) {
      qkv_pre = (char*)pool_.get((size_t)rows * 3 * C * es);
      if (!qkv_pre) return T2P_ERR_HIP;
      if (mega) {
        y2 = (float*)pool_.get((size_t)rows * C * es);
        if (!y2) return T2P_ERR_HIP;
        if (g_fuse_gn_stats) {
          y2_stats = (float*)pool_.get((size_t)(rows / 64) * C * 2 * 4);
          if (!y2_stats) return T2P_ERR_HIP;
          e.zero = y2_stats; e.zero_n = (long)(rows / 64) * C * 2;
        }
      }
      e.t = t; e.qkv = qkv_pre;
      T2P_TRY(launch_st_entry(e, s));
      if (normed) { pool_.put(x.pre_norm); x.pre_norm = nullptr; }
    }
    pool_.put(a_small);
  }
  if (!qkv_pre) {
    void* a = nullptr;
    T2P_TRY(group_norm(x, nullptr, L.gn0, 1e-6f, 0, 0, B, &a, s));
    T2P_TRY(linear(a, false, L.proj_in, rows, t, !tl, nullptr, 1.f, s));
    pool_.put(a);
  }
  POOL_GET(ln, void*, (size_t)rows * C * es);
  POOL_GET(o, void*, (size_t)rows * C * es);
  if (!qkv_pre) T2P_TRY(launch_layernorm(t, L.ln1.gamma, L.ln1.beta, ln, dt, rows, C, 1e-5f, s, tl));
  if (qkv_flash) {
    char* qkv = qkv_pre;
    if (!qkv) {
      qkv = (char*)pool_.get((size_t)rows * 3 * C * es);
      if (!qkv) return T2P_ERR_HIP;
      T2P_TRY(linear(ln, false, L.a1_qkv, rows, qkv, false, nullptr, 1.f, s, false));
    }
    T2P_TRY(launch_attention_flash(dt, qkv, 3 * C, qkv + (size_t)C * es, 3 * C, qkv + (size_t)2 * C * es, 3 * C, o, B, heads, n, n, d, scale, s,
                                   true));
    pool_.put(qkv);
  } else {
    POOL_GET(qk, char*, (size_t)rows * 2 * C * es);
    T2P_TRY(linear(ln, false, L.a1_qk, rows, qk, false, nullptr, 1.f, s, false));
    POOL_GET(vt, void*, (size_t)B * C * npad * es);
    T2P_TRY(project_vt(dt, L.a1_v, ln, C, B, n, npad, vt, s));
    T2P_TRY(attention(qk, 2 * C, qk + (size_t)C * es, 2 * C, vt, npad, o, B, heads, n, n, d, scale, s));
    pool_.put(qk);
    pool_.put(vt);
  }
  {
    POOL_GET(q, void*, (size_t)rows * C * es);
    StEntryArgs e;
    e.dtype = dt; e.B = B; e.n = n; e.C = C; e.x = o; e.w_in = L.fm_out1; e.b_in = L.a1_out.b; e.res = t;
    e.ln_gamma = L.ln2.gamma; e.ln_beta = L.ln2.beta; e.ln_eps = 1e-5f; e.w_qkv = L.fm_q2; e.n2 = C; e.t = t; e.qkv = q;
    if (tl && qkv_pre && L.a1_out.b && !L.a2_q.b && st_entry_eligible(e)) {
      T2P_TRY(launch_st_entry(e, s));
    } else {
      T2P_TRY(linear(o, false, L.a1_out, rows, t, !tl, t, 1.f, s, true, nullptr, tl));
      T2P_TRY(launch_layernorm(t, L.ln2.gamma, L.ln2.beta, ln, dt, rows, C, 1e-5f, s, tl));
      T2P_TRY(linear(ln, false, L.a2_q, rows, q, false, nullptr, 1.f, s, false));
    }
    T2P_TRY(attention(q, C, L.ctx_k, C, L.ctx_vt, ctx_Tpad_, o, B, heads, n, ctx_T_, d, scale, s));
    pool_.put(q);
  }
  {
    POOL_GET(g, void*, (size_t)rows * 4 * C * es);
    GemmParams p;
    p.dtype = dt; p.A0 = ln; p.a_f32 = dt == DT_F32; p.C0 = C; p.lda0 = C;
    p.Bw = L.ff1.w; p.ldb = C; p.M = (int)rows; p.N = 8 * C; p.bias_n = L.ff1.b;
    p.C = g; p.c_f32 = 0; p.ldc = 4 * C; p.geglu = 1;
    T2P_TRY(attach_ws(p));
    StEntryArgs e;
    e.dtype = dt; e.B = B; e.n = n; e.C = C; e.x = o; e.w_in = L.fm_out2; e.b_in = L.a2_out.b; e.res = t;
    e.ln_gamma = L.ln3.gamma; e.ln_beta = L.ln3.beta; e.ln_eps = 1e-5f; e.w_qkv = L.fm_ff1; e.b2 = L.ff1.b; e.n2 = 8 * C; e.geglu = 1;
    e.t = t; e.qkv = g;
    const bool tail_chain = tl && qkv_pre && g_st_tail && (y2 || rows >= 2 * g_st_tail_rows) && L.fm_ff1 && g_fuse_geglu && gemm_fuses_geglu(p) && L.a2_out.b && L.ff1.b && st_entry_eligible(e);
    if (tail_chain && y2) {
      e.w3 = L.fm_ffpo; e.b3 = L.ffpo.b; e.res3 = x.p; e.y = y2; e.y_stats = y2_stats; e.qkv = nullptr;
      T2P_REQUIRE(st_entry_eligible(e), "row chain with the third product");
      T2P_TRY(launch_st_entry(e, s));
      pool_.put(g); pool_.put(o); pool_.put(ln); pool_.put(t);
      *out = Act{y2, C, x.H, x.W, y2_stats, true};
      return T2P_OK;
    }
    if (y2) { pool_.put(y2); pool_.put(y2_stats); y2 = nullptr; y2_stats = nullptr; }
    if (tail_chain) {
      T2P_TRY(launch_st_entry(e, s));
    } else {
      T2P_TRY(linear(o, false, L.a2_out, rows, t, !tl, t, 1.f, s, true, nullptr, tl));
      T2P_TRY(launch_layernorm(t, L.ln3.gamma, L.ln3.beta, ln, dt, rows, C, 1e-5f, s, tl));
    }
    if (tail_chain) {
    } else if (g_fuse_geglu && gemm_fuses_geglu(p)) {
      T2P_TRY(gemm(p, s));
    } else {
      POOL_GET(u, float*, (size_t)rows * 8 * C * 4);
      T2P_TRY(linear(ln, false, L.ff1, rows, u, true, nullptr, 1.f, s));
      T2P_TRY(launch_geglu(u, g, dt, rows, 4 * C, s, 1));
      pool_.put(u);
    }
    if (g_ffpo_merged && tl && L.ffpo.w) {
      pool_.put(o);
      const bool olp2 = res_lowp();
      POOL_GET(y2, float*, (size_t)rows * C * (olp2 ? es : 4));
      float* y2_stats = nullptr;
      GemmParams q;
      q.dtype = dt; q.a_f32 = 0; q.A0 = g; q.C0 = 4 * C; q.lda0 = 4 * C; q.A1 = t; q.C1 = C; q.lda1 = C;
      q.Bw = L.ffpo.w; q.ldb = L.ffpo.K; q.M = (int)rows; q.N = C; q.bias_n = L.ffpo.b;
      q.R = x.p; q.ldr = C; q.r_lowp = x.lowp ? 1 : 0;
      q.C = y2; q.c_f32 = olp2 ? 0 : 1; q.ldc = C; q.rows_per_batch = n;
      T2P_TRY(gemm_stats(q, &y2_stats, s));
      pool_.put(g);
      pool_.put(ln);
      pool_.put(t);
      *out = Act{y2, C, x.H, x.W, y2_stats, olp2};
      return T2P_OK;
    }
    T2P_TRY(linear(g, false, L.ff2, rows, t, !tl, t, 1.f, s, true, nullptr, tl));
    pool_.put(g);
  }
  pool_.put(o);
  const bool olp = res_lowp();
  POOL_GET(y, float*, (size_t)rows * C * (olp ? es : 4));
  float* y_stats = nullptr;
  if (tl) {
    T2P_TRY(linear(t, false, L.proj_out, rows, y, !olp, x.p, 1.f, s, true, &y_stats, x.lowp));
  } else if (dt != DT_F32 && g_raw_copies) {
    T2P_TRY(launch_convert(t, ln, dt, rows * C, s));
    T2P_TRY(linear(ln, false, L.proj_out, rows, y, !olp, x.p, 1.f, s, true, &y_stats, x.lowp));
  } else {
    T2P_TRY(linear(t, true, L.proj_out, rows, y, !olp, x.p, 1.f, s, true, &y_stats, x.lowp));
  }
  pool_.put(ln);
  pool_.put(t);
  *out = Act{y, C, x.H, x.W, y_stats, olp};
  return T2P_OK;
}

static NormHint first_norm_of(const Layer* l, bool concat_input) {
  NormHint h;
  if (!l || concat_input || l->down) return h;
  h.norm = &l->gn0;
  h.silu = l->kind == 0 ? 1 : 0;
  return h;
}

int Engine::run_stage(Stage& st, Act& h, const Act* skip, int B, hipStream_t s, const Layer* next_after) {
  Act cur = h;
  bool own = false;
  for (size_t i = 0; i < st.layers.size(); ++i) {
    Layer& L = st.layers[i];
    Act nxt;
// ... 179 lines not shown
```

text2protein_amd/csrc/engine.h:

```cpp
#pragma once
#include <initializer_list>
#include <map>
#include <memory>
#include <string>
#include <unordered_map>
#include <unordered_set>
#include <vector>

#include "../../include/t2p.h"
#include "t2p_kernels.h"

namespace t2p {

class DevPool {
 public:
  ~DevPool();
  void* get(size_t bytes);
  void put(void* p);
  size_t held_bytes() const { return held_; }
  void* persistent(size_t bytes);
  void lease_begin();
  int lease_end();
  void keep(void* p) { leased_.erase(p); }
  int last_reclaimed() const { return last_reclaimed_; }
 private:
  std::multimap<size_t, void*> free_;
  std::unordered_map<void*, size_t> size_of_;
  std::vector<void*> all_;
  std::unordered_set<void*> leased_;
  int lease_depth_ = 0, last_reclaimed_ = 0;
  size_t held_ = 0;
};
struct PoolLease {
  explicit PoolLease(DevPool& p) : pool(p) { pool.lease_begin(); }
  ~PoolLease() { pool.lease_end(); }
  PoolLease(const PoolLease&) = delete;
  PoolLease& operator=(const PoolLease&) = delete;
  DevPool& pool;
};

struct HostTensor {
  std::vector<float> data;
  std::vector<int64_t> shape;
};

struct ParamInfo {
  std::string name;
  std::vector<int64_t> shape;
};

struct DevLinear {
  void* w = nullptr;
  float* b = nullptr;
  int N = 0, K = 0;
};
struct DevNorm {
  float* gamma = nullptr;
  float* beta = nullptr;
  int C = 0, G = 0;
};

struct Layer {
  int kind = 0;
  std::string prefix;
  int in_ch = 0, out_ch = 0, up = 0, down = 0;
  DevNorm gn0, gn1;
  DevLinear conv0, conv1, conv2;
  void* conv0_up4 = nullptr;
  DevLinear conv1x;
  void* fm_conv0 = nullptr; void* fm_conv1 = nullptr;
  bool has_conv2 = false;
  int temb_off = 0;
  DevLinear qk, v, out;
  DevLinear v3;
  void* fm_qk = nullptr; void* fm_v3 = nullptr;
  DevLinear a1_qkv;
  DevLinear proj_in, proj_out, a1_qk, a1_v, a1_out, a2_q, a2_k, a2_v, a2_out, ff1, ff2;
  DevLinear ffpo;
  void* fm_in = nullptr; void* fm_qkv = nullptr; void* fm_out1 = nullptr; void* fm_q2 = nullptr; void* fm_out2 = nullptr; void* fm_ff1 = nullptr; void* fm_ffpo = nullptr;
  DevNorm ln1, ln2, ln3;
  void* ctx_k = nullptr;
  void* ctx_vt = nullptr;
};

struct Stage {
  std::vector<Layer> layers;
  int skip_ch = 0;
};

struct NetArch {
  std::vector<Stage> input_stages, out_stages;
  Stage mid_stage;
  std::vector<ParamInfo> params;
  int nf = 0, temb_dim = 0, temb_total = 0, final_ch = 0;
  int build(const t2p_model_config& c);
};

struct Act {
  float* p = nullptr;
  int C = 0, H = 0, W = 0;
  float* cstats = nullptr;
  bool lowp = false;
  mutable void* pre_norm = nullptr;
  const DevNorm* pre_for = nullptr;
  int pre_silu = 0;
};
struct NormHint {
  const DevNorm* norm = nullptr;
  int silu = 0;
};

class Engine {
 public:
  explicit Engine(const t2p_model_config& cfg);
  ~Engine();
  int build();
  const std::vector<ParamInfo>& params() const { return arch_.params; }
  int load_param(const char* name, const float* data, const int64_t* shape, int ndim);
  int finalize();
  int load_flat(const float* device_flat, int64_t n, hipStream_t s);
  int64_t num_elements() const { return total_; }
  const int64_t* load_stats() const { return load_stats_; }
  int device() const { return device_; }
  bool finalized() const { return finalized_; }
  int set_context(const float* ctx, int B, int T, hipStream_t s);
  int score(const float* x, const int* labels, const int* step_counter, float* out, int B, hipStream_t s,
            const float* labels_f = nullptr, const int* label_table = nullptr, const float* label_f_table = nullptr);
  int64_t device_bytes() const { return (int64_t)pool_.held_bytes(); }
  int pool_reclaimed() const { return pool_.last_reclaimed(); }
  const t2p_model_config& cfg() const { return cfg_; }
  DevPool& pool() { return pool_; }
  int dtype() const { return cfg_.compute_dtype; }

 private:
  int pack_weights();
  int dest(void** slot, size_t bytes);
  const float* psrc(const std::string& name, int64_t numel);
  int pack(int kind, void* dst, int64_t off, int dtype, std::initializer_list<const float*> srcs, std::initializer_list<int64_t> dims);
  int pack_frag(void** slot, const void* w, int N, int K);
  int pack_linear(const std::string& wname, const std::string& bname, int N, int K, DevLinear* out,
                  bool conv3x3 = false, bool nin = false, int force_dtype = -1, int cin_pad = 0);
  int pack_stack2(const std::string& w0, const std::string& b0, const std::string& w1, const std::string& b1,
                  int N, int K, bool nin, bool has_bias, DevLinear* out);
  int pack_norm(const std::string& prefix, int C, int G, DevNorm* out);

  int run_stage(Stage& st, Act& h, const Act* skip, int B, hipStream_t s, const Layer* next_after = nullptr);
  int res_block(Layer& L, const Act& x, const Act* skip, Act* out, int B, hipStream_t s, NormHint hint = NormHint());
  int attn_block(Layer& L, const Act& x, Act* out, int B, hipStream_t s);
  int st_block(Layer& L, const Act& x, Act* out, int B, hipStream_t s);
  int group_norm(const Act& x, const Act* x1, const DevNorm& n, float eps, int silu, int down, int B, void** out,
                 hipStream_t s, void** raw_out = nullptr);
  int gemm(GemmParams& p, hipStream_t s);
  int attach_ws(GemmParams& p);
  int gemm_stats(GemmParams& p, float** cstats, hipStream_t s);
  void free_act(Act& a) { pool_.put(a.p); pool_.put(a.cstats); pool_.put(a.pre_norm); a.p = nullptr; a.cstats = nullptr; a.pre_norm = nullptr; }
  void drop_pre_norm(const Act& a) { pool_.put(a.pre_norm); a.pre_norm = nullptr; }
  int attention(const void* q, long ldq, const void* k, long ldk, const void* vt, long ldvt, void* out, int B,
                int heads, int nq, int nk, int d, float scale, hipStream_t s);
  int linear(const void* a, bool a_is_f32, const DevLinear& w, long rows, void* c, bool c_f32, const float* residual,
             float alpha, hipStream_t s, bool use_bias = true, float** cstats = nullptr, bool r_lowp = false);
  bool res_lowp() const { return g_lowp_residual && cfg_.compute_dtype == DT_F16; }

  t2p_model_config cfg_;
  NetArch arch_;
  std::unordered_map<std::string, HostTensor> host_;
  bool finalized_ = false;
  DevPool pool_;
  std::unordered_map<std::string, std::pair<int64_t, int64_t>> poff_;
  int64_t total_ = 0;
  int device_ = 0;
  const float* flat_ = nullptr;
  hipStream_t pack_stream_ = nullptr;
  int64_t load_stats_[3] = {0, 0, 0};

  int cpad_ = 8;
  DevLinear pre0_, pre1_, pre_conv_, head_conv_, dense_all_;
  DevNorm head_norm_;
  float* pre_conv_direct_ = nullptr;
  void* pre_conv_split_ = nullptr;
  float* inv_sigma_ = nullptr;
  float* unit_scale_ = nullptr;
  int ctx_B_ = 0, ctx_T_ = 0, ctx_Tpad_ = 0;
  int ctx_cap_B_ = 0, ctx_cap_T_ = 0;
  void* splitk_ws_ = nullptr;
  size_t splitk_ws_bytes_ = 0;
  const float* tb_ = nullptr;
  long tb_ld_ = 0;
};

}

struct t2p_engine { t2p::Engine impl; explicit t2p_engine(const t2p_model_config& c) : impl(c) {} };
```

text2protein_amd/csrc/gemm.hip:

```cpp
#include <algorithm>
#include <array>
#include <cstdio>
#include <cstring>
#include <map>
#include <string>
#include <type_traits>
#include <vector>

#include "t2p_common.h"

namespace t2p {

typedef float f32x16 __attribute__((ext_vector_type(16)));
typedef __bf16 bf16x8_t __attribute__((ext_vector_type(8)));
typedef _Float16 f16x8_t __attribute__((ext_vector_type(8)));

[[maybe_unused]] static constexpr int ROWB = 144;

template <typename TC> struct VecInfo { static constexpr int VEC = 16 / (int)sizeof(TC); };

template <typename TC> __device__ inline uint4 pack16(const float* f);
template <> __device__ inline uint4 pack16<float>(const float* f) {
  uint4 r;
  r.x = __builtin_bit_cast(uint32_t, f[0]); r.y = __builtin_bit_cast(uint32_t, f[1]);
  r.z = __builtin_bit_cast(uint32_t, f[2]); r.w = __builtin_bit_cast(uint32_t, f[3]);
  return r;
}
template <> __device__ inline uint4 pack16<bf16_t>(const float* f) {
  uint4 r;
  r.x = (uint32_t)f32_to_bf16_bits(f[0]) | ((uint32_t)f32_to_bf16_bits(f[1]) << 16);
  r.y = (uint32_t)f32_to_bf16_bits(f[2]) | ((uint32_t)f32_to_bf16_bits(f[3]) << 16);
  r.z = (uint32_t)f32_to_bf16_bits(f[4]) | ((uint32_t)f32_to_bf16_bits(f[5]) << 16);
  r.w = (uint32_t)f32_to_bf16_bits(f[6]) | ((uint32_t)f32_to_bf16_bits(f[7]) << 16);
  return r;
}
template <> __device__ inline uint4 pack16<f16_t>(const float* f) {
  typedef _Float16 h2 __attribute__((ext_vector_type(2)));
  uint4 r;
  h2 a = {(_Float16)f[0], (_Float16)f[1]}, b = {(_Float16)f[2], (_Float16)f[3]};
  h2 c = {(_Float16)f[4], (_Float16)f[5]}, d = {(_Float16)f[6], (_Float16)f[7]};
  r.x = __builtin_bit_cast(uint32_t, a); r.y = __builtin_bit_cast(uint32_t, b);
  r.z = __builtin_bit_cast(uint32_t, c); r.w = __builtin_bit_cast(uint32_t, d);
  return r;
}

template <typename TC> __device__ inline uint4 mask_tail(uint4 v, int nvalid) {
  constexpr int VEC = VecInfo<TC>::VEC;
  union { uint4 u; TC e[VEC]; } x;
  x.u = v;
#pragma unroll
  for (int i = 0; i < VEC; ++i)
    if (i >= nvalid) x.e[i] = from_f32<TC>(0.f);
  return x.u;
}

template <typename TC, bool SRC_F32>
__device__ inline uint4 load_vec(const void* base, long off) {
  constexpr int VEC = VecInfo<TC>::VEC;
  if constexpr (SRC_F32) {
    const float* p = (const float*)base + off;
    float f[VEC];
#pragma unroll
    for (int i = 0; i < VEC; i += 4) {
      float4 t = *(const float4*)(p + i);
      f[i] = t.x; f[i + 1] = t.y; f[i + 2] = t.z; f[i + 3] = t.w;
    }
    return pack16<TC>(f);
  } else {
    return *(const uint4*)((const TC*)base + off);
  }
}

template <typename TC> struct Mma;
template <> struct Mma<float> {
  __device__ static inline void run(const uint4& a, const uint4& b, f32x16& c) {
    c = __builtin_amdgcn_mfma_f32_32x32x2f32(__builtin_bit_cast(float, a.x), __builtin_bit_cast(float, b.x), c, 0, 0, 0);
    c = __builtin_amdgcn_mfma_f32_32x32x2f32(__builtin_bit_cast(float, a.y), __builtin_bit_cast(float, b.y), c, 0, 0, 0);
    c = __builtin_amdgcn_mfma_f32_32x32x2f32(__builtin_bit_cast(float, a.z), __builtin_bit_cast(float, b.z), c, 0, 0, 0);
    c = __builtin_amdgcn_mfma_f32_32x32x2f32(__builtin_bit_cast(float, a.w), __builtin_bit_cast(float, b.w), c, 0, 0, 0);
  }
};
template <> struct Mma<bf16_t> {
  __device__ static inline void run(const uint4& a, const uint4& b, f32x16& c) {
    c = __builtin_amdgcn_mfma_f32_32x32x16_bf16(__builtin_bit_cast(bf16x8_t, a), __builtin_bit_cast(bf16x8_t, b), c, 0, 0, 0);
  }
};
template <> struct Mma<f16_t> {
  __device__ static inline void run(const uint4& a, const uint4& b, f32x16& c) {
    c = __builtin_amdgcn_mfma_f32_32x32x16_f16(__builtin_bit_cast(f16x8_t, a), __builtin_bit_cast(f16x8_t, b), c, 0, 0, 0);
  }
};

typedef float f32x4_res_t __attribute__((ext_vector_type(4)));
typedef unsigned u32x2_res_t __attribute__((ext_vector_type(2)));
template <typename TC> __device__ inline float res_load1(const float* R, long idx, int lowp) {
  if constexpr (sizeof(TC) == 2) { if (lowp) return to_f32(((const TC*)R)[idx]); }
  return R[idx];
}
template <typename TC> __device__ inline f32x4_res_t unpack4(u32x2_res_t u) {
  TC e[4];
  e[0] = __builtin_bit_cast(TC, (uint16_t)u.x); e[1] = __builtin_bit_cast(TC, (uint16_t)(u.x >> 16));
  e[2] = __builtin_bit_cast(TC, (uint16_t)u.y); e[3] = __builtin_bit_cast(TC, (uint16_t)(u.y >> 16));
  return (f32x4_res_t){to_f32(e[0]), to_f32(e[1]), to_f32(e[2]), to_f32(e[3])};
}
template <typename TC> __device__ inline float4 res_load4(const float* R, long idx, int lowp) {
  if constexpr (sizeof(TC) == 2) {
    if (lowp) {
      const f32x4_res_t v = unpack4<TC>(*(const u32x2_res_t*)((const TC*)R + idx));
      return make_float4(v[0], v[1], v[2], v[3]);
    }
  }
  return *(const float4*)(R + idx);
}

#ifndef T2P_GEMM_PART
#define T2P_GEMM_PART -1
#endif
#define T2P_PART_HOST (T2P_GEMM_PART <= 0)
#define T2P_PART_DMA (T2P_GEMM_PART != 0)

struct ProfRec { hipEvent_t a, b; double flops; int kind; const char* name; double bytes; int M = 0, N = 0, K = 0, taps = 0, z = 0; };
inline void prof_shape(ProfRec& r, const GemmParams& p) {
  r.M = p.M; r.N = p.N; r.K = p.C0 + p.C1; r.taps = p.a_up ? -p.taps : p.taps; r.z = p.nz0 * p.nz1;
  if (p.CX0 + p.CX1) r.K = r.K * 1000000 + p.CX0 + p.CX1;
}
struct DmaPlan { int geom, nsplit; };
extern bool g_prof_on;
extern std::vector<ProfRec> g_prof;
extern int g_dma_ring, g_dbg;
extern bool g_up4, g_deep_ring, g_dxs;
int num_cus();
DmaPlan dma_plan(const GemmParams& p);
int launch_splitk_reduce(const GemmParams& p, int nsplit, hipStream_t stream);
template <typename TC, int MODE> int launch_dma_mode(const GemmParams& p, hipStream_t stream);

__host__ __device__ __forceinline__ bool reg_epilogue_ok(const GemmParams& p, const int nsplit, const int dbg) {
  if (dbg & 4096) return false;
  const long c_cols = p.geglu ? p.N / 2 : p.N;
  const long c_bytes = nsplit > 1 ? (long)p.M * p.N * 4 : ((long)(p.M - 1) * p.ldc + c_cols) * (p.c_f32 ? 4 : 2);
  const int HW = p.H * p.W;
  const long r_rows = p.r_up ? (long)(p.M / HW) * (p.H >> 1) * (p.W >> 1) : (long)p.M;
  const long r_bytes = p.R ? ((r_rows - 1) * p.ldr + p.N) * (p.r_lowp ? 2 : 4) : 0;
  if ((p.N & 7) || c_bytes >= (1L << 31) || r_bytes >= (1L << 31)) return false;
  if (nsplit > 1) return true;
  if (p.geglu ? (p.ldc & 3) : (p.ldc & 7)) return false;
  if (p.R && (p.ldr & 7)) return false;
  if (p.bias_bn && ((p.ld_bn & 3) || p.rows_per_batch % 16)) return false;
  if (p.r_up && (p.W % 16 || p.rows_per_batch != HW)) return false;
  return true;
}


#if T2P_PART_HOST
template <typename TC, bool AF32, int BM, int BN>
__global__ __launch_bounds__(256) void gemm_kernel(const GemmParams p) {
  constexpr int VEC = VecInfo<TC>::VEC;
  constexpr int BK = 8 * VEC;
  constexpr int AR = BM / 32, BR = BN / 32;
  constexpr int TM = BM / 64, TN = BN / 64;
  extern __shared__ __attribute__((aligned(16))) unsigned char smem[];
  unsigned char* As = smem;
  unsigned char* Bs = smem + 2 * BM * ROWB;

  const int tid = threadIdx.x;
  const int lane = tid & 63, wave = tid >> 6;
  const int wm = wave >> 1, wn = wave & 1;
  const int lr = lane & 31, lh = lane >> 5;
  const int n0 = blockIdx.x * BN, m0 = blockIdx.y * BM;
  const int z0 = blockIdx.z / p.nz1, z1 = blockIdx.z % p.nz1;

  const int Ctot = p.C0 + p.C1;
  const int nch = (Ctot + BK - 1) / BK;
  const int nk = nch * p.taps;
  const bool spatial = (p.taps == 9) || p.a_up;
  const int HW = p.H * p.W;
  const int Hs = p.a_up ? (p.H >> 1) : p.H, Ws = p.a_up ? (p.W >> 1) : p.W;

  const long aoff = (long)z0 * p.sA_z0 + (long)z1 * p.sA_z1;
  const char* A0 = (const char*)p.A0 + aoff * (AF32 ? 4 : (long)sizeof(TC));
  const char* A1 = (const char*)p.A1;
  const TC* Bw = (const TC*)p.Bw + (long)z0 * p.sB_z0 + (long)z1 * p.sB_z1;

  const int cv = tid & 7, srow = tid >> 3;
  int a_b[AR], a_y[AR], a_x[AR];
  bool a_ok[AR];
#pragma unroll
// ... 52 lines not shown
  };
  auto sstore = [&](int buf) {
    unsigned char* a = As + buf * BM * ROWB;
    unsigned char* b = Bs + buf * BN * ROWB;
#pragma unroll
    for (int i = 0; i < AR; ++i) *(uint4*)(a + (srow + 32 * i) * ROWB + cv * 16) = ra[i];
#pragma unroll
    for (int j = 0; j < BR; ++j) *(uint4*)(b + (srow + 32 * j) * ROWB + cv * 16) = rb[j];
  };

  f32x16 acc[TM][TN];
#pragma unroll
  for (int i = 0; i < TM; ++i)
#pragma unroll
    for (int j = 0; j < TN; ++j)
#pragma unroll
      for (int v = 0; v < 16; ++v) acc[i][j][v] = 0.f;

  gload(0);
  sstore(0);
  __syncthreads();
  for (int kt = 0; kt < nk; ++kt) {
    const int buf = kt & 1;
    if (kt + 1 < nk) gload(kt + 1);
    const unsigned char* a = As + buf * BM * ROWB + (wm * (BM / 2) + lr) * ROWB + lh * 16;
    const unsigned char* b = Bs + buf * BN * ROWB + (wn * (BN / 2) + lr) * ROWB + lh * 16;
#pragma unroll
    for (int s = 0; s < 4; ++s) {
      uint4 af[TM], bf[TN];
#pragma unroll
      for (int i = 0; i < TM; ++i) af[i] = *(const uint4*)(a + i * 32 * ROWB + s * 32);
#pragma unroll
      for (int j = 0; j < TN; ++j) bf[j] = *(const uint4*)(b + j * 32 * ROWB + s * 32);
#pragma unroll
      for (int i = 0; i < TM; ++i)
#pragma unroll
        for (int j = 0; j < TN; ++j) Mma<TC>::run(af[i], bf[j], acc[i][j]);
    }
    if (kt + 1 < nk) sstore(buf ^ 1);
    __syncthreads();
  }

  const long coff = (long)z0 * p.sC_z0 + (long)z1 * p.sC_z1;
  const float* R = p.R ? (p.r_lowp ? (const float*)((const uint16_t*)p.R + (long)z0 * p.sR_z0 + (long)z1 * p.sR_z1)
                                   : p.R + (long)z0 * p.sR_z0 + (long)z1 * p.sR_z1) : nullptr;
#pragma unroll
  for (int i = 0; i < TM; ++i) {
#pragma unroll
    for (int v = 0; v < 16; ++v) {
      const int row = m0 + wm * (BM / 2) + i * 32 + (v & 3) + 8 * (v >> 2) + 4 * lh;
      if (row >= p.M) continue;
      const int bidx = row / p.rows_per_batch;
      long rrow = row;
      if (p.r_up) {
        int rem = row - bidx * HW;
        int y = rem / p.W, x = rem - y * p.W;
        rrow = ((long)bidx * (p.H >> 1) + (y >> 1)) * (p.W >> 1) + (x >> 1);
      }
      const float bm = p.bias_m ? p.bias_m[row] : 0.f;
#pragma unroll
      for (int j = 0; j < TN; ++j) {
        const int col = n0 + wn * (BN / 2) + j * 32 + lr;
        if (col >= p.N) continue;
        float val = acc[i][j][v] + bm;
        if (p.bias_n) val += p.bias_n[col];
        if (p.bias_bn) val += p.bias_bn[(long)bidx * p.ld_bn + col];
        if (R) val += res_load1<TC>(R, rrow * p.ldr + col, p.r_lowp);
        val *= p.alpha;
        if (p.c_nchw) {
          const int pix = row - bidx * p.rows_per_batch;
          ((float*)p.C)[((long)bidx * p.N + col) * p.rows_per_batch + pix] = val * p.row_scale[bidx];
        } else if (p.c_f32) {
          ((float*)p.C)[coff + (long)row * p.ldc + col] = val;
        } else {
          ((TC*)p.C)[coff + (long)row * p.ldc + col] = from_f32<TC>(val);
        }
      }
    }
  }
}

#endif

typedef int v4i_t __attribute__((ext_vector_type(4)));
typedef unsigned u32x4_t __attribute__((ext_vector_type(4)));
#define T2P_LDS_PTR(p) ((__attribute__((address_space(3))) void*)(p))
[[maybe_unused]] static constexpr unsigned DMA_OOB = 0x80000000u;

__device__ inline float gelu_erf_fast(float g) {
  const float x = g * 0.70710678118654752440f, ax = fabsf(x);
  const float t = __builtin_amdgcn_rcpf(fmaf(0.3275911f, ax, 1.f));
  float q = fmaf(t, 1.061405429f, -1.453152027f);
  q = fmaf(q, t, 1.421413741f);
  q = fmaf(q, t, -0.284496736f);
  q = fmaf(q, t, 0.254829592f);
  const float e = __builtin_amdgcn_exp2f(-ax * ax * 1.44269504088896340736f);
  const float erf_abs = fmaf(-q * t, e, 1.f);
  return 0.5f * g * (1.f + copysignf(erf_abs, x));
}
typedef unsigned u32x2_t __attribute__((ext_vector_type(2)));
template <typename TC> __device__ inline uint32_t pack2(float a, float b) {
  const TC x = from_f32<TC>(a), y = from_f32<TC>(b);
  return (uint32_t)__builtin_bit_cast(uint16_t, x) | ((uint32_t)__builtin_bit_cast(uint16_t, y) << 16);
}

template <int I> __device__ inline void lds_read_b128(u32x4_t& dst, unsigned addr) {
  asm volatile("ds_read_b128 %0, %1 offset:%2" : "=v"(dst) : "v"(addr), "n"(I * 4096));
}

typedef float f32x4_t __attribute__((ext_vector_type(4)));
template <typename TC> struct Mma16;
template <> struct Mma16<bf16_t> {
  __device__ static inline void run(const u32x4_t& a, const u32x4_t& b, f32x4_t& c) {
    c = __builtin_amdgcn_mfma_f32_16x16x32_bf16(__builtin_bit_cast(bf16x8_t, a), __builtin_bit_cast(bf16x8_t, b), c, 0, 0, 0);
  }
};
template <> struct Mma16<f16_t> {
  __device__ static inline void run(const u32x4_t& a, const u32x4_t& b, f32x4_t& c) {
    c = __builtin_amdgcn_mfma_f32_16x16x32_f16(__builtin_bit_cast(f16x8_t, a), __builtin_bit_cast(f16x8_t, b), c, 0, 0, 0);
  }
};
#if T2P_PART_DMA
__device__ inline bool g_stagger_dbg(int dbg) { return (dbg & 128) == 0; }
template <int I> __device__ inline void lds_read_b128_2k(u32x4_t& dst, unsigned addr) {
  asm volatile("ds_read_b128 %0, %1 offset:%2" : "=v"(dst) : "v"(addr), "n"(I * 2048));
}
template <int I> __device__ inline void lds_read_b128_1k(u32x4_t& dst, unsigned addr) {
  asm volatile("ds_read_b128 %0, %1 offset:%2" : "=v"(dst) : "v"(addr), "n"(I * 1024));
}

struct LeanRup { int on, W, HW, b_first, b_edge, hw4, w2; unsigned row_bytes, col_bytes; };

template <typename TC, int OUT, bool HAS_R, bool STATS, bool RL = false>
__device__ __forceinline__ void lean_slab(const float* sp, const __amdgpu_buffer_rsrc_t rC, const __amdgpu_buffer_rsrc_t rR,
                                          unsigned voc, const unsigned stc, unsigned vor, const unsigned str,
                                          const float4 bn0, const float4 bn1, const int row_first, const int b_edge,
                                          const float alpha, float* stats_dst, const LeanRup rup) {
  if constexpr (OUT == 3) {
#pragma unroll
    for (int h8 = 0; h8 < 2; ++h8) {
      f32x4_t v[8];
#pragma unroll
      for (int i = 0; i < 8; ++i) v[i] = *(const f32x4_t*)(sp + (h8 * 8 + i) * 256);
#pragma unroll
      for (int i = 0; i < 8; ++i) {
        __builtin_amdgcn_raw_buffer_store_b128(__builtin_bit_cast(u32x4_t, v[i]), rC, voc, 0, 0);
        voc += stc;
      }
    }
    return;
  }
  float cs0 = 0.f, cs1 = 0.f, cs2 = 0.f, cs3 = 0.f, cq0 = 0.f, cq1 = 0.f, cq2 = 0.f, cq3 = 0.f;
#pragma unroll
  for (int h8 = 0; h8 < 2; ++h8) {
    f32x4_t v[8], rv[8];
    if constexpr (!HAS_R) {
#pragma unroll
      for (int i = 0; i < 8; ++i) v[i] = *(const f32x4_t*)(sp + (h8 * 8 + i) * 256);
    }
    if constexpr (HAS_R) {
#pragma unroll
      for (int i = 0; i < 8; ++i) {
        unsigned off = vor;
        if (rup.on) {
          const int row = row_first + 4 * (h8 * 8 + i);
          const int bidx = rup.b_first + (row >= rup.b_edge ? 1 : 0);
          const int rem = row - bidx * rup.HW;
          const int y = rem / rup.W, x = rem - y * rup.W;
          off = vor == DMA_OOB ? DMA_OOB : (unsigned)(bidx * rup.hw4 + (y >> 1) * rup.w2 + (x >> 1)) * rup.row_bytes + rup.col_bytes;
        }
        if constexpr (RL) rv[i] = unpack4<TC>(__builtin_amdgcn_raw_buffer_load_b64(rR, off, 0, 0));
        else rv[i] = __builtin_bit_cast(f32x4_t, __builtin_amdgcn_raw_buffer_load_b128(rR, off, 0, 0));
        if (!rup.on) vor += str;
      }
    }
#pragma unroll
    for (int i = 0; i < 8; ++i) {
      const int it = h8 * 8 + i;
      if constexpr (HAS_R) {
        if (i % 4 == 0) {
#pragma unroll
          for (int k = 0; k < 4; ++k) v[i + k] = *(const f32x4_t*)(sp + (it + k) * 256);
        }
      }
      const bool second = row_first + 4 * it >= b_edge;
      float a0 = v[i][0] + (second ? bn1.x : bn0.x), a1 = v[i][1] + (second ? bn1.y : bn0.y);
      float a2 = v[i][2] + (second ? bn1.z : bn0.z), a3 = v[i][3] + (second ? bn1.w : bn0.w);
      if constexpr (HAS_R) { a0 += rv[i][0]; a1 += rv[i][1]; a2 += rv[i][2]; a3 += rv[i][3]; }
      if constexpr (OUT == 2) {
        __builtin_amdgcn_raw_buffer_store_b32(pack2<TC>(a0 * gelu_erf_fast(a1), a2 * gelu_erf_fast(a3)), rC, voc, 0, 0);
      } else {
        a0 *= alpha; a1 *= alpha; a2 *= alpha; a3 *= alpha;
        if constexpr (STATS) {
          cs0 += a0; cs1 += a1; cs2 += a2; cs3 += a3;
          cq0 += a0 * a0; cq1 += a1 * a1; cq2 += a2 * a2; cq3 += a3 * a3;
        }
        if constexpr (OUT == 0) {
          __builtin_amdgcn_raw_buffer_store_b128(__builtin_bit_cast(u32x4_t, (f32x4_t){a0, a1, a2, a3}), rC, voc, 0, 0);
        } else {
          __builtin_amdgcn_raw_buffer_store_b64((u32x2_t){pack2<TC>(a0, a1), pack2<TC>(a2, a3)}, rC, voc, 0, 0);
        }
      }
      voc += stc;
    }
  }
  if constexpr (STATS) {
    cs0 += __shfl_xor(cs0, 16, 64); cs1 += __shfl_xor(cs1, 16, 64); cs2 += __shfl_xor(cs2, 16, 64); cs3 += __shfl_xor(cs3, 16, 64);
    cq0 += __shfl_xor(cq0, 16, 64); cq1 += __shfl_xor(cq1, 16, 64); cq2 += __shfl_xor(cq2, 16, 64); cq3 += __shfl_xor(cq3, 16, 64);
    cs0 += __shfl_xor(cs0, 32, 64); cs1 += __shfl_xor(cs1, 32, 64); cs2 += __shfl_xor(cs2, 32, 64); cs3 += __shfl_xor(cs3, 32, 64);
    cq0 += __shfl_xor(cq0, 32, 64); cq1 += __shfl_xor(cq1, 32, 64); cq2 += __shfl_xor(cq2, 32, 64); cq3 += __shfl_xor(cq3, 32, 64);
    if (stats_dst) {
      *(float4*)stats_dst = make_float4(cs0, cq0, cs1, cq1);
      *(float4*)(stats_dst + 4) = make_float4(cs2, cq2, cs3, cq3);
    }
  }
}


__device__ __forceinline__ __amdgpu_buffer_rsrc_t make_rsrc(const void* base, int bytes) {
  const unsigned long long b = (unsigned long long)base;
  const unsigned lo = __builtin_amdgcn_readfirstlane((unsigned)b);
  const unsigned hi = __builtin_amdgcn_readfirstlane((unsigned)(b >> 32));
  const int nb = __builtin_amdgcn_readfirstlane(bytes);
  return __builtin_amdgcn_make_buffer_rsrc((void*)(((unsigned long long)hi << 32) | lo), 0, nb, 0x00020000);
}

template <typename TC, int BM, int BN, int WM, int WN, bool MF16, int TI, int TJ>
__device__ __forceinline__ void dma_epilogue(const GemmParams& p, unsigned char* smem, f32x16 (&acc)[MF16 ? 1 : TI][MF16 ? 1 : TJ],
                                             f32x4_t (&acc16)[MF16 ? 8 : 1][MF16 ? 4 : 1], const int m0, const int n0, const int z0,
                                             const int z1, const int nsplit, const int ks, const int dbg) {
  const int tid = threadIdx.x;
  const int lane = tid & 63;
  const int wave = __builtin_amdgcn_readfirstlane(tid >> 6);
  const int wm = wave / WN, wn = wave % WN;
  const int lr = lane & 31, lh = lane >> 5;
  const int HW = p.H * p.W;

  if ((dbg & 1) && (MF16 ? acc16[0][0][0] : acc[0][0][0]) != 123.456f) return;
  __builtin_amdgcn_s_barrier();
  float* stg = (float*)(smem + wave * 16384);
  const long coff = (long)z0 * p.sC_z0 + (long)z1 * p.sC_z1;
  const float* R = p.R ? (p.r_lowp ? (const float*)((const uint16_t*)p.R + (long)z0 * p.sR_z0 + (long)z1 * p.sR_z1)
                                   : p.R + (long)z0 * p.sR_z0 + (long)z1 * p.sR_z1) : nullptr;
  const bool need_b = p.bias_bn || p.r_up;
  const int rpb = p.rows_per_batch;
  const int b_first = need_b ? m0 / rpb : 0;
  const int b_edge = (b_first + 1) * rpb;
  const int cq = (lane & 15) * 4;
  float* ws = nsplit > 1 ? (float*)p.ws + (long)ks * p.M * p.N : nullptr;

  const int c_cols = p.geglu ? p.N / 2 : p.N;
  const long c_bytes = ws ? (long)p.M * p.N * 4 : ((long)(p.M - 1) * p.ldc + c_cols) * (p.c_f32 ? 4 : 2);
  const long r_rows = p.r_up ? (long)(p.M / HW) * (p.H >> 1) * (p.W >> 1) : (long)p.M;
  const long r_bytes = R ? ((r_rows - 1) * p.ldr + p.N) * (p.r_lowp ? 2 : 4) : 0;
  const bool lean = !(dbg & 512) && (p.N & 3) == 0 && c_bytes < (1L << 31) && r_bytes < (1L << 31) &&
                    (ws != nullptr || (!p.bias_m && (!need_b || rpb >= BM) && (p.geglu ? p.ldc % 2 == 0 : p.ldc % 4 == 0) &&
                                       (!R || p.ldr % 4 == 0) && (!p.bias_bn || p.ld_bn % 4 == 0)));
  const __amdgpu_buffer_rsrc_t rC =
      make_rsrc(ws ? (const void*)ws : (p.c_f32 ? (const void*)((float*)p.C + coff) : (const void*)((TC*)p.C + coff)), lean ? (int)c_bytes : 0);
  const __amdgpu_buffer_rsrc_t rR = make_rsrc(R ? (const void*)R : (const void*)p.C, lean ? (int)r_bytes : 0);
  const bool two_b = p.bias_bn && b_edge < m0 + BM && b_edge < p.M;

  auto slab = [&](auto HI, auto HJ) {
      constexpr int hi = decltype(HI)::value, hj = decltype(HJ)::value;
      if (hi + hj > 0) asm volatile("s_waitcnt lgkmcnt(0)" ::: "memory");
      if (!(dbg & 2048)) {
      if constexpr (MF16) {
#pragma unroll
        for (int i = 0; i < 4; ++i)
#pragma unroll
          for (int j = 0; j < 4; ++j)
            *(f32x4_t*)(stg + (i * 16 + (lane & 15)) * 64 + 32 * (j >> 1) + 8 * (lane >> 4) + 4 * (j & 1)) = acc16[4 * hi + i][4 * hj + j];
      } else {
#pragma unroll
        for (int i = 0; i < 2; ++i)
#pragma unroll
          for (int j = 0; j < 2; ++j)
#pragma unroll
            for (int v = 0; v < 16; ++v)
              stg[(i * 32 + (v & 3) + 8 * (v >> 2) + 4 * lh) * 64 + j * 32 + lr] = acc[2 * hi + i][2 * hj + j][v];
      }
      }
      const int row0 = m0 + wm * (BM / WM) + hi * 64;
      const int col = n0 + wn * (BN / WN) + hj * 64 + cq;
      if (lean) {
        const int rq = lane >> 4;
        const bool col_ok = col < p.N;
        const float* sp = stg + rq * 64 + cq;
        const unsigned esz = (ws || p.c_f32) ? 4u : 2u;
        const unsigned ldc_e = ws ? (unsigned)p.N : (unsigned)p.ldc;
        const unsigned voc = (col_ok && !(dbg & 1024)) ? ((unsigned)(row0 + rq) * ldc_e + (unsigned)(p.geglu ? col >> 1 : col)) * esz : DMA_OOB;
        const unsigned stc = 4u * ldc_e * esz;
        const unsigned rsz = p.r_lowp ? 2u : 4u;
        const unsigned vor = col_ok ? ((unsigned)(row0 + rq) * (unsigned)p.ldr + (unsigned)col) * rsz : DMA_OOB;
        const unsigned str = 4u * rsz * (unsigned)p.ldr;
        const LeanRup rup = {p.r_up, p.W, HW, b_first, b_edge, (p.H >> 1) * (p.W >> 1), p.W >> 1, rsz * (unsigned)p.ldr, rsz * (unsigned)col};
        float4 bn0 = make_float4(0.f, 0.f, 0.f, 0.f);
        if (!ws && p.bias_n && col_ok) bn0 = *(const float4*)(p.bias_n + col);
        float4 bn1 = bn0;
        if (!ws && p.bias_bn && col_ok) {
          const float4 t = *(const float4*)(p.bias_bn + (long)b_first * p.ld_bn + col);
          bn0.x += t.x; bn0.y += t.y; bn0.z += t.z; bn0.w += t.w;
          if (two_b) {
            const float4 u = *(const float4*)(p.bias_bn + (long)(b_first + 1) * p.ld_bn + col);
            bn1.x += u.x; bn1.y += u.y; bn1.z += u.z; bn1.w += u.w;
          }
        }
        const int edge = two_b ? b_edge : 0x7fffffff;
// ... 43 lines not shown
          if (col + 2 < p.N) bn.z = p.bias_n[col + 2];
        }
      }
      const bool vec_ok = full4 && (p.ldc % 4 == 0 || p.geglu) && (!R || p.ldr % 4 == 0) && (!p.bias_bn || p.ld_bn % 4 == 0);
      float cs0 = 0.f, cs1 = 0.f, cs2 = 0.f, cs3 = 0.f, cq0 = 0.f, cq1 = 0.f, cq2 = 0.f, cq3 = 0.f;
#pragma unroll 4
      for (int it = 0; it < 16; ++it) {
        const int rl = it * 4 + (lane >> 4);
        const int row = row0 + rl;
        if (row >= p.M || col >= p.N) continue;
        float4 a = *(const float4*)(stg + rl * 64 + cq);
        int bidx = 0;
        if (need_b) bidx = rpb >= BM ? b_first + (row >= b_edge ? 1 : 0) : row / rpb;
        long rrow = row;
        if (p.r_up) {
          const int rem = row - bidx * HW;
          const int y = rem / p.W, x = rem - y * p.W;
          rrow = ((long)bidx * (p.H >> 1) + (y >> 1)) * (p.W >> 1) + (x >> 1);
        }
        const float bm = p.bias_m ? p.bias_m[row] : 0.f;
        a.x += bm + bn.x; a.y += bm + bn.y; a.z += bm + bn.z; a.w += bm + bn.w;
        if (vec_ok) {
          if (p.bias_bn) {
            const float4 t = *(const float4*)(p.bias_bn + (long)bidx * p.ld_bn + col);
            a.x += t.x; a.y += t.y; a.z += t.z; a.w += t.w;
          }
          if (R) {
            const float4 t = res_load4<TC>(R, rrow * p.ldr + col, p.r_lowp);
            a.x += t.x; a.y += t.y; a.z += t.z; a.w += t.w;
          }
          if (p.geglu) {
            const float g0 = 0.5f * a.y * (1.f + erff(a.y * 0.70710678118654752440f));
            const float g1 = 0.5f * a.w * (1.f + erff(a.w * 0.70710678118654752440f));
            TC* dst = (TC*)p.C + coff + (long)row * p.ldc + (col >> 1);
            union { TC e[2]; uint32_t u; } o;
            o.e[0] = from_f32<TC>(a.x * g0); o.e[1] = from_f32<TC>(a.z * g1);
            *(uint32_t*)dst = o.u;
            continue;
          }
          a.x *= p.alpha; a.y *= p.alpha; a.z *= p.alpha; a.w *= p.alpha;
          cs0 += a.x; cs1 += a.y; cs2 += a.z; cs3 += a.w;
          cq0 += a.x * a.x; cq1 += a.y * a.y; cq2 += a.z * a.z; cq3 += a.w * a.w;
          if (p.c_f32) {
            *(float4*)((float*)p.C + coff + (long)row * p.ldc + col) = a;
          } else {
            TC* dst = (TC*)p.C + coff + (long)row * p.ldc + col;
            union { TC e[4]; uint2 u; } o;
            o.e[0] = from_f32<TC>(a.x); o.e[1] = from_f32<TC>(a.y); o.e[2] = from_f32<TC>(a.z); o.e[3] = from_f32<TC>(a.w);
            *(uint2*)dst = o.u;
          }
        } else {
          float vals[4] = {a.x, a.y, a.z, a.w};
          for (int k = 0; k < 4; ++k) {
            if (col + k >= p.N) break;
            float val = vals[k];
            if (p.bias_bn) val += p.bias_bn[(long)bidx * p.ld_bn + col + k];
            if (R) val += res_load1<TC>(R, rrow * p.ldr + col + k, p.r_lowp);
            val *= p.alpha;
            if (p.c_f32) ((float*)p.C)[coff + (long)row * p.ldc + col + k] = val;
            else ((TC*)p.C)[coff + (long)row * p.ldc + col + k] = from_f32<TC>(val);
          }
        }
      }
      if (p.col_stats) {
        cs0 += __shfl_xor(cs0, 16, 64); cs1 += __shfl_xor(cs1, 16, 64); cs2 += __shfl_xor(cs2, 16, 64); cs3 += __shfl_xor(cs3, 16, 64);
        cq0 += __shfl_xor(cq0, 16, 64); cq1 += __shfl_xor(cq1, 16, 64); cq2 += __shfl_xor(cq2, 16, 64); cq3 += __shfl_xor(cq3, 16, 64);
        cs0 += __shfl_xor(cs0, 32, 64); cs1 += __shfl_xor(cs1, 32, 64); cs2 += __shfl_xor(cs2, 32, 64); cs3 += __shfl_xor(cs3, 32, 64);
        cq0 += __shfl_xor(cq0, 32, 64); cq1 += __shfl_xor(cq1, 32, 64); cq2 += __shfl_xor(cq2, 32, 64); cq3 += __shfl_xor(cq3, 32, 64);
        if (lane < 16 && vec_ok) {
          float* dst = p.col_stats + ((long)(row0 >> 6) * p.N + col) * 2;
          *(float4*)dst = make_float4(cs0, cq0, cs1, cq1);
          *(float4*)(dst + 4) = make_float4(cs2, cq2, cs3, cq3);
        }
      }
  };
  slab(std::integral_constant<int, 0>{}, std::integral_constant<int, 0>{});
  if constexpr (TJ / 2 > 1) slab(std::integral_constant<int, 0>{}, std::integral_constant<int, 1>{});
  if constexpr (TI / 2 > 1) {
    slab(std::integral_constant<int, 1>{}, std::integral_constant<int, 0>{});
    if constexpr (TJ / 2 > 1) slab(std::integral_constant<int, 1>{}, std::integral_constant<int, 1>{});
  }
}

__device__ __forceinline__ int hperm(int rho) {
  const int j = rho >> 4, g = (rho >> 2) & 3, v = rho & 3;
  return 32 * (j >> 1) + 8 * g + 4 * (j & 1) + v;
}
__device__ __forceinline__ float row16_sum(float x) {
  x += __builtin_bit_cast(float, __builtin_amdgcn_update_dpp(0, __builtin_bit_cast(int, x), 0xB1, 0xF, 0xF, false));
  x += __builtin_bit_cast(float, __builtin_amdgcn_update_dpp(0, __builtin_bit_cast(int, x), 0x4E, 0xF, 0xF, false));
  x += __builtin_bit_cast(float, __builtin_amdgcn_update_dpp(0, __builtin_bit_cast(int, x), 0x141, 0xF, 0xF, false));
  x += __builtin_bit_cast(float, __builtin_amdgcn_update_dpp(0, __builtin_bit_cast(int, x), 0x140, 0xF, 0xF, false));
  return x;
}

#ifndef T2P_C_AUX
#define T2P_C_AUX 0
#endif
typedef __attribute__((address_space(4))) GemmParams KernArgs;
__device__ __forceinline__ const KernArgs* kernel_args() {
  const KernArgs* pk = (const KernArgs*)__builtin_amdgcn_kernarg_segment_ptr();
  asm volatile("" : "+s"(pk));
  return pk;
}
template <typename TC, int BM, int BN, int WM, int WN, bool CFRAG = false, bool PLAIN = false, typename PT = GemmParams>
__device__ __forceinline__ void reg_epilogue(const PT& p, f32x4_t (&acc16)[8][4], const int m0, const int n0, const int z0,
                                             const int z1, const int nsplit, const int ks, const int dbg) {
  if ((dbg & 1) && acc16[0][0][0] != 123.456f) return;
  int tx = threadIdx.x;
  asm volatile("" : "+v"(tx));
  const int lane = tx & 63;
  const int wave = __builtin_amdgcn_readfirstlane(tx >> 6);
  const int wm = wave / WN, wn = wave % WN;
  const int l16 = lane & 15, g4 = lane >> 4;
  const int HW = p.H * p.W;
  const long coff = (long)z0 * p.sC_z0 + (long)z1 * p.sC_z1;
  const float* R = p.R ? (p.r_lowp ? (const float*)((const uint16_t*)p.R + (long)z0 * p.sR_z0 + (long)z1 * p.sR_z1)
                                   : p.R + (long)z0 * p.sR_z0 + (long)z1 * p.sR_z1) : nullptr;
  static_assert(!(PLAIN && CFRAG), "the plain form stores row-major only");
  float* ws = (!PLAIN && nsplit > 1) ? (float*)p.ws + (long)ks * p.M * p.N : nullptr;
  const bool p_geglu = PLAIN ? false : p.geglu != 0, p_c_f32 = PLAIN ? false : p.c_f32 != 0;
  const float* const p_bias_m = PLAIN ? nullptr : p.bias_m;
  const int c_cols = p_geglu ? p.N / 2 : p.N;
  const long c_bytes = ws ? (long)p.M * p.N * 4 : ((long)(p.M - 1) * p.ldc + c_cols) * (p_c_f32 ? 4 : 2);
  const long r_rows = p.r_up ? (long)(p.M / HW) * (p.H >> 1) * (p.W >> 1) : (long)p.M;
  const long r_bytes = R ? ((r_rows - 1) * p.ldr + p.N) * (p.r_lowp ? 2 : 4) : 0;
  const __amdgpu_buffer_rsrc_t rC =
      make_rsrc(ws ? (const void*)ws : (p_c_f32 ? (const void*)((float*)p.C + coff) : (const void*)((TC*)p.C + coff)), (int)c_bytes);
  const __amdgpu_buffer_rsrc_t rR = make_rsrc(R ? (const void*)R : (const void*)p.C, (int)r_bytes);

  const int row_w = m0 + wm * (BM / WM);
  const int upp = PLAIN ? 0 : (p.up_phase == 5 ? 1 + (int)blockIdx.y : p.up_phase);
  const int Mrows = upp ? p.M >> 2 : p.M;
  const int Wl = p.W >> 1, HWl = (p.H >> 1) * (p.W >> 1);
  const int col0 = n0 + wn * (BN / WN) + 8 * g4;
  const bool ok0 = col0 < p.N, ok1 = col0 + 32 < p.N;
  float bs[16];
#pragma unroll
  for (int k = 0; k < 16; ++k) bs[k] = 0.f;
  const int rpb = p.rows_per_batch;
  const bool need_b = p.bias_bn || p.r_up;
  const int b_first = upp ? m0 / HWl : (need_b ? m0 / rpb : 0);
  if (!ws) {
#pragma unroll
    for (int h = 0; h < 2; ++h) {
      const int c = col0 + 32 * h;
      if (c < p.N) {
#pragma unroll
        for (int q = 0; q < 2; ++q) {
          float4 t = make_float4(0.f, 0.f, 0.f, 0.f);
          if (p.bias_n) t = *(const float4*)(p.bias_n + c + 4 * q);
          if (p.bias_bn) {
            const float4 a = *(const float4*)(p.bias_bn + (long)b_first * p.ld_bn + c + 4 * q);
            t.x += a.x; t.y += a.y; t.z += a.z; t.w += a.w;
          }
          const int k = 8 * h + 4 * q;
          bs[k] = t.x; bs[k + 1] = t.y; bs[k + 2] = t.z; bs[k + 3] = t.w;
        }
      }
    }
  }
  const unsigned esz = (ws || p_c_f32) ? 4u : 2u;
  const unsigned ldc_e = ws ? (unsigned)p.N : (unsigned)p.ldc;
  const unsigned rsz = p.r_lowp ? 2u : 4u;
  const bool nostore = (dbg & 1024) != 0;
  const bool alpha_not_one = p.alpha != 1.0f;
  float cs[16], cq[16];

  auto rows_of = [&](int i, int& row, unsigned& rrow, int& bsel) __attribute__((always_inline)) {
    row = row_w + 16 * i + l16;
// ... 1540 lines not shown
        v = *(const u32x4_t*)(xb + ((long)gy * a.W + gx) * a.Cin + c0 + j * 8);
        if (norm) {
          union { u32x4_t u; TC e[8]; } in, o;
          in.u = v;
#pragma unroll
          for (int e = 0; e < 8; ++e) {
            const int c = c0 + j * 8 + e;
            float y = to_f32(in.e[e]) * nsc[c] + nsh[c];
            if (a.gn_silu) y = y * __builtin_amdgcn_rcpf(1.f + __builtin_amdgcn_exp2f(y * -1.44269504088896341f));
            o.e[e] = from_f32<TC>(y);
          }
          v = o.u;
        }
      }
      *(u32x4_t*)(halo + P * cb + (((j & ~sw) | ((j ^ P) & sw)) << 4)) = v;
    }
    for (int i = tid; i < a.Cout * 9 * nchunk; i += 512) {
      const int co = i / (9 * nchunk), k = i - co * 9 * nchunk, tap = k / nchunk, j = k - tap * nchunk;
      *(u32x4_t*)(wl + co * wrow + k * 16) = *(const u32x4_t*)((const TC*)a.w + (long)co * a.ldw + (long)tap * a.Cin + c0 + j * 8);
    }
    __syncthreads();
#pragma unroll
    for (int tap = 0; tap < 9; ++tap) {
      const int dy = tap / 3, dx = tap % 3;
      const int P = (wave + dy) * WP + r + dx;
      u32x4_t af[CH / 32], bf[CH / 32];
#pragma unroll
      for (int kc = 0; kc < CH / 32; ++kc) {
        const int j = kc * 4 + g;
        af[kc] = *(const u32x4_t*)(halo + P * cb + (((j & ~sw) | ((j ^ P) & sw)) << 4));
        bf[kc] = (u32x4_t){0u, 0u, 0u, 0u};
        if (colv) bf[kc] = *(const u32x4_t*)(wl + r * wrow + (tap * nchunk + j) * 16);
      }
#pragma unroll
      for (int kc = 0; kc < CH / 32; ++kc) Mma16<TC>::run(af[kc], bf[kc], acc);
    }
  }
  if (!colv) return;
  const int y = y0 + wave;
  if (y >= a.H) return;
  const float bias = a.bias ? a.bias[r] : 0.f, sc = a.row_scale ? a.row_scale[b] : 1.f;
  float* o = a.out + (((long)b * a.Cout + r) * a.H + y) * a.W;
#pragma unroll
  for (int v = 0; v < 4; ++v) {
    const int x = x0 + g * 4 + v;
    if (x < a.W) o[x] = (acc[v] + bias) * sc;
  }
}

static bool g_thin_conv = true;
static bool g_a_norm = true;
void set_gemm_thin_conv(bool on) { g_thin_conv = on; }
void set_gemm_a_norm(bool on) { g_a_norm = on; }

static bool thin_conv_eligible(const GemmParams& p) {
  if (p.dtype == DT_F32 || p.a_f32 || p.taps != 9 || p.a_up || !p.c_nchw || !p.c_f32) return false;
  if (p.A1 || p.R || p.bias_m || p.bias_bn || p.nz0 * p.nz1 != 1 || p.alpha != 1.f || p.geglu) return false;
  if (p.N > 8 || (p.C0 != 32 && p.C0 != 64 && p.C0 != 128 && p.C0 != 256) || p.lda0 != p.C0) return false;
  return p.rows_per_batch == p.H * p.W && p.M % (p.H * p.W) == 0;
}

bool gemm_applies_a_norm(const GemmParams& p) { return g_thin_conv && g_a_norm && thin_conv_eligible(p) && p.C0 <= 256; }

template <typename TC, int CH>
static int launch_thin_conv_ch(const ThinConvArgs& a, hipStream_t stream) {
  constexpr int smem = 180 * CH * 2 + 8 * (9 * CH * 2 + 16);
  const int tiles = ((a.W + 15) / 16) * ((a.H + 7) / 8);
  hipLaunchKernelGGL((thin_conv_kernel<TC, CH>), dim3((unsigned)((long)a.B * tiles)), dim3(512), smem, stream, a);
  T2P_HIP_CHECK(hipGetLastError());
  return T2P_OK;
}

template <typename TC>
static int launch_thin_conv(const GemmParams& p, hipStream_t stream) {
  ThinConvArgs a;
  a.x = p.A0; a.w = p.Bw; a.bias = p.bias_n; a.row_scale = p.row_scale; a.out = (float*)p.C;
  a.B = p.M / (p.H * p.W); a.H = p.H; a.W = p.W; a.Cin = p.C0; a.Cout = p.N; a.ldw = p.ldb;
  a.gn_stats = p.an_stats; a.gn_gamma = p.an_gamma; a.gn_beta = p.an_beta; a.gn_groups = p.an_groups; a.gn_silu = p.an_silu;
  if (p.C0 == 32) return launch_thin_conv_ch<TC, 32>(a, stream);
  if (p.C0 == 64) return launch_thin_conv_ch<TC, 64>(a, stream);
  return launch_thin_conv_ch<TC, 128>(a, stream);
}

int launch_gemm(const GemmParams& p, hipStream_t stream) {
  const int vec = p.dtype == DT_F32 ? 4 : 8;
  const int Ctot = p.C0 + p.C1;
  T2P_REQUIRE(p.A0 && p.Bw && (p.C || p.gn_out), "null operand");
  if (p.gn_out) {
    GemmParams q = p;
    q.gn_out = nullptr; q.gn_gamma = q.gn_beta = nullptr;
    T2P_REQUIRE(p.gn_gamma && p.gn_beta && gemm_fuses_post_gn(q, p.gn_groups), "a following GroupNorm rides only on the split-K second pass (ask gemm_fuses_post_gn)");
  }
  T2P_REQUIRE(p.M > 0 && p.N > 0 && Ctot > 0, "empty problem");
  T2P_REQUIRE(p.taps == 1 || p.taps == 9, "taps must be 1 or 9");
  T2P_REQUIRE(p.dtype != DT_F32 || p.a_f32, "fp32 compute takes fp32 sources");
  T2P_REQUIRE(!p.r_lowp || (p.R && p.dtype != DT_F32), "a 16-bit residual needs a 16-bit compute dtype");
  T2P_REQUIRE(p.lda0 % vec == 0 && p.ldb % vec == 0, "row strides must be multiples of the 16-byte vector");
  T2P_REQUIRE(p.lda0 >= ((p.C0 + vec - 1) / vec) * vec, "lda0 too small");
  T2P_REQUIRE(p.ldb >= (long)(p.taps - 1) * Ctot + ((Ctot + vec - 1) / vec) * vec, "ldb too small");
  if (p.A1) {
    T2P_REQUIRE(p.C0 % vec == 0 && p.lda1 % vec == 0 && p.C1 % vec == 0, "concat sources must be vector aligned");
    T2P_REQUIRE(p.nz0 * p.nz1 == 1, "batched GEMM takes a single A source");
  } else {
    T2P_REQUIRE(p.C1 == 0, "C1 without A1");
  }
  if (p.taps == 9) T2P_REQUIRE(Ctot % vec == 0, "3x3 convolution needs channels % vector == 0");
  if (p.taps == 9 || p.a_up || p.r_up || p.c_nchw) {
    T2P_REQUIRE(p.H > 0 && p.W > 0 && p.M % (p.H * p.W) == 0, "spatial mode needs H, W with M = batch*H*W");
    T2P_REQUIRE(p.nz0 * p.nz1 == 1, "spatial modes are not batched");
  }
  if (p.a_up || p.r_up) T2P_REQUIRE(p.H % 2 == 0 && p.W % 2 == 0, "up-sampling needs even H, W");
  if (p.r_up || p.c_nchw) T2P_REQUIRE(p.rows_per_batch == p.H * p.W, "rows_per_batch must be H*W");
  T2P_REQUIRE(p.rows_per_batch > 0, "rows_per_batch");
  T2P_REQUIRE(!p.c_nchw || (p.row_scale && p.c_f32), "nchw store needs row_scale and fp32 output");
  T2P_REQUIRE(((uintptr_t)p.A0 % 16) == 0 && ((uintptr_t)p.Bw % 16) == 0 && ((uintptr_t)p.A1 % 16) == 0,
              "operands must be 16-byte aligned");
  T2P_REQUIRE((long)(p.M + 127) / 128 < 65536, "M too large for grid.y");
  if (p.X0 || p.X1 || p.CX0 || p.CX1) {
    GemmParams q = p;
    q.X0 = q.X1 = nullptr; q.CX0 = q.CX1 = 0;
    T2P_REQUIRE(p.X0 && p.CX0 > 0 && p.CX0 % 64 == 0 && p.CX1 % 64 == 0 && (p.X1 != nullptr) == (p.CX1 > 0), "shortcut segment: whole 64-channel K-tiles");
    T2P_REQUIRE(gemm_can_fuse_shortcut(q), "shortcut segment: only on the LDS-DMA 3x3 convolution (ask gemm_can_fuse_shortcut)");
    T2P_REQUIRE(((uintptr_t)p.X0 % 16) == 0 && ((uintptr_t)p.X1 % 16) == 0 && p.ldx0 % 8 == 0 && p.ldx1 % 8 == 0, "shortcut segment: 16-byte aligned rows");
    T2P_REQUIRE(((long)p.M + 512) * std::max(p.ldx0, p.ldx1) * 2 < (1L << 31) - 64 && std::max(p.ldx0, p.ldx1) * 2 < (1L << 24), "shortcut segment: 32-bit offsets");
    T2P_REQUIRE(p.ldb >= 9L * (p.C0 + p.C1) + p.CX0 + p.CX1, "shortcut segment: weight rows hold 9 (C0 + C1) + CX0 + CX1 columns");
  }
  if (p.an_stats) {
    GemmParams q = p;
    q.an_stats = nullptr;
    T2P_REQUIRE(p.an_gamma && p.an_beta && p.an_groups > 0 && p.C0 % p.an_groups == 0 && gemm_applies_a_norm(q),
                "a GroupNorm of the A operand rides only on the thin-output head convolution (ask gemm_applies_a_norm)");
  }
  if (g_thin_conv && thin_conv_eligible(p)) {
    ProfRec rec;
    if (g_prof_on) {
      T2P_HIP_CHECK(hipEventCreate(&rec.a));
      T2P_HIP_CHECK(hipEventCreate(&rec.b));
      prof_shape(rec, p);
    prof_shape(rec, p);
      rec.flops = 2.0 * p.M * p.N * 9.0 * p.C0; rec.kind = 2; rec.name = nullptr; rec.bytes = 0;
      T2P_HIP_CHECK(hipEventRecord(rec.a, stream));
    }
    const int rc = p.dtype == DT_BF16 ? launch_thin_conv<bf16_t>(p, stream) : launch_thin_conv<f16_t>(p, stream);
    if (g_prof_on) {
      T2P_HIP_CHECK(hipEventRecord(rec.b, stream));
      g_prof.push_back(rec);
    }
    return rc;
  }
  if (dma_eligible(p)) return p.dtype == DT_BF16 ? launch_dma<bf16_t>(p, stream) : launch_dma<f16_t>(p, stream);
  switch (p.dtype) {
    case DT_F32: return launch_tile<float, true>(p, stream);
    case DT_BF16: return p.a_f32 ? launch_tile<bf16_t, true>(p, stream) : launch_tile<bf16_t, false>(p, stream);
    case DT_F16: return p.a_f32 ? launch_tile<f16_t, true>(p, stream) : launch_tile<f16_t, false>(p, stream);
  }
  set_last_error("launch_gemm: unknown dtype");
  return T2P_ERR_INVALID;
}

#endif

#if T2P_GEMM_PART == -1 || T2P_GEMM_PART == 1
template int launch_dma_mode<f16_t, 0>(const GemmParams&, hipStream_t);
#endif
#if T2P_GEMM_PART == -1 || T2P_GEMM_PART == 2
template int launch_dma_mode<f16_t, 1>(const GemmParams&, hipStream_t);
#endif
#if T2P_GEMM_PART == -1 || T2P_GEMM_PART == 3
template int launch_dma_mode<f16_t, 2>(const GemmParams&, hipStream_t);
#endif
#if T2P_GEMM_PART == -1 || T2P_GEMM_PART == 4
template int launch_dma_mode<bf16_t, 0>(const GemmParams&, hipStream_t);
#endif
#if T2P_GEMM_PART == -1 || T2P_GEMM_PART == 5
template int launch_dma_mode<bf16_t, 1>(const GemmParams&, hipStream_t);
#endif
#if T2P_GEMM_PART == -1 || T2P_GEMM_PART == 6
template int launch_dma_mode<bf16_t, 2>(const GemmParams&, hipStream_t);
#endif

}
```

text2protein_amd/csrc/t2p_common.h:

```cpp
#pragma once
#include <hip/hip_runtime.h>
#include <stdint.h>
#include <string>

namespace t2p {

enum DType : int { DT_F32 = 0, DT_BF16 = 1, DT_F16 = 2 };

inline size_t dtype_size(int dt) { return dt == DT_F32 ? 4 : 2; }

struct bf16_t { uint16_t v; };
struct f16_t { _Float16 v; };

template <typename T> struct dtype_of;
template <> struct dtype_of<float> { static constexpr int value = DT_F32; };
template <> struct dtype_of<bf16_t> { static constexpr int value = DT_BF16; };
template <> struct dtype_of<f16_t> { static constexpr int value = DT_F16; };

__host__ __device__ inline uint16_t f32_to_bf16_bits(float f) {
#if defined(__HIP_DEVICE_COMPILE__)
  return __builtin_bit_cast(uint16_t, (__bf16)f);
#endif
  uint32_t u = __builtin_bit_cast(uint32_t, f);
  if ((u & 0x7fffffffu) > 0x7f800000u) return (uint16_t)((u >> 16) | 0x40);
// ... 22 lines not shown
#define T2P_ERR_HIP 2
#define T2P_ERR_STATE 3

#define T2P_HIP_CHECK(expr)                                                                   \
  do {                                                                                        \
    hipError_t _e = (expr);                                                                   \
    if (_e != hipSuccess) {                                                                   \
      ::t2p::set_last_error(std::string(#expr) + ": " + hipGetErrorString(_e) + " at " +      \
                            __FILE__ + ":" + std::to_string(__LINE__));                       \
      return T2P_ERR_HIP;                                                                     \
    }                                                                                         \
  } while (0)

#define T2P_REQUIRE(cond, msg)                                                                \
  do {                                                                                        \
    if (!(cond)) {                                                                            \
      ::t2p::set_last_error(std::string("requirement failed: ") + #cond + " -- " + (msg) +    \
                            " at " + __FILE__ + ":" + std::to_string(__LINE__));              \
      return T2P_ERR_INVALID;                                                                 \
    }                                                                                         \
  } while (0)

#define T2P_TRY(expr)                                                                         \
  do {                                                                                        \
    int _rc = (expr);                                                                         \
    if (_rc != T2P_OK) return _rc;                                                            \
  } while (0)

int ensure_dynamic_lds(const void* kernel, int bytes);

struct GemmParams {
  const void* A0 = nullptr;
  const void* A1 = nullptr;
  int a_f32 = 0;
  int C0 = 0, C1 = 0;
  long lda0 = 0, lda1 = 0;
  int taps = 1;
  int H = 0, W = 0;
  int a_up = 0;
  const void* Bw = nullptr;
  long ldb = 0;
  const void* Bw4 = nullptr;
  long ldb4 = 0;
  int up_phase = 0;
  const void* X0 = nullptr;
  const void* X1 = nullptr;
  int CX0 = 0, CX1 = 0;
  long ldx0 = 0, ldx1 = 0;
  int M = 0, N = 0;
  int nz0 = 1, nz1 = 1;
  long sA_z0 = 0, sA_z1 = 0, sB_z0 = 0, sB_z1 = 0, sC_z0 = 0, sC_z1 = 0, sR_z0 = 0, sR_z1 = 0;
  const float* bias_n = nullptr;
  const float* bias_m = nullptr;
  const float* bias_bn = nullptr;
  int rows_per_batch = 1;
  long ld_bn = 0;
  const float* R = nullptr;
  int r_lowp = 0;
  long ldr = 0;
  int r_up = 0;
  float alpha = 1.f;
  void* C = nullptr;
  int c_f32 = 1;
  long ldc = 0;
  int c_nchw = 0;
  const float* row_scale = nullptr;
  int dtype = DT_F32;
  int geglu = 0;
  float* col_stats = nullptr;
  void* ws = nullptr;
  size_t ws_bytes = 0;
  const float* gn_gamma = nullptr;
  const float* gn_beta = nullptr;
  int gn_groups = 0, gn_silu = 0;
  float gn_eps = 1e-6f;
  void* gn_out = nullptr;
  const float* an_stats = nullptr;
  const float* an_gamma = nullptr;
  const float* an_beta = nullptr;
  int an_groups = 0, an_silu = 0;
  void* c_frag = nullptr;
  int frag_col0 = 0, frag_ns = 0;
  long frag_bstride = 0;
};
bool gemm_writes_frag_major(const GemmParams& p);

int launch_gemm(const GemmParams& p, hipStream_t stream);
bool gemm_fuses_col_stats(const GemmParams& p);
bool gemm_can_fuse_shortcut(const GemmParams& p);
bool gemm_fuses_geglu(const GemmParams& p);
bool gemm_fuses_col_stats_lowp(const GemmParams& p);
bool gemm_fuses_post_gn(const GemmParams& p, int groups);
void set_gemm_post_gn(bool on);
bool gemm_applies_a_norm(const GemmParams& p);
void set_gemm_split_consts(int tiles, int target);
void set_gemm_dma(bool on);
void set_gemm_debug(int v);
void set_gemm_geom(int v);
void set_gemm_ring(int v);
void set_gemm_splitk(bool on);
void set_gemm_force_nsplit(int v);
void set_gemm_midsplit(bool on);
void set_gemm_thin_conv(bool on);
void set_gemm_a_norm(bool on);
void set_gemm_up4(bool on);
void set_gemm_deep_ring(bool on);
void set_gemm_fuse_shortcut(bool on);
void set_gemm_dxs(bool on);
#ifdef T2P_ABLATION
int dxs_stamps_read(unsigned long long* out, int n);
#endif
extern bool g_qkv_fused;
extern bool g_attn_merged, g_ffpo_merged;
extern bool g_flash_attention;
extern bool g_lowp_h1;
extern bool g_lowp_residual;
extern bool g_layernorm16;
extern bool g_gn_apply16;
extern bool g_gn_small;
extern bool g_fuse_geglu;
extern bool g_fuse_gn_stats;
extern bool g_raw_copies;
void profile_begin();
int profile_end(double out[3][3]);
int profile_dominant(double out[4], const char** name);
int profile_shapes(char* buf, int len);
int profile_conv_kernels(char* buf, int len);
bool prof_on();
void prof_attention(hipEvent_t a, hipEvent_t b, double flops);
int profile_attention(double out[3]);

}
```

text2protein_amd/csrc/t2p_kernels.h:

```cpp
#pragma once
#include "t2p_common.h"

namespace t2p {

struct GroupNormArgs {
  const float* x0 = nullptr; const float* x1 = nullptr;
  int C0 = 0, C1 = 0;
  int B = 0, HW = 0;
  int G = 0;
  float eps = 1e-6f;
  int lowp_dtype = DT_F32;
  float* partial = nullptr;
  float* stats = nullptr;
};
int gn_num_chunks(int HW);
int launch_gn_stats(const GroupNormArgs& a, hipStream_t s);

int launch_gn_finalize_cols(const float* cs0, const float* cs1, int C0, int C1, int B, int HW, int G, float eps,
                            float* stats, hipStream_t s);

struct GroupNormApplyArgs {
  const float* x0 = nullptr; const float* x1 = nullptr;
  int C0 = 0, C1 = 0, B = 0, H = 0, W = 0, G = 0;
  const float* stats = nullptr;
// ... 92 lines not shown
                           void* out, int B, int heads, int nq, int nk, int d, float scale, hipStream_t s, bool v_rowmajor = false);

extern bool g_attn_strip;
bool attention_strip_eligible(int dtype, int heads, int nq, int nk, int d, long ldq, long ldk, long ldvt, long ldo);
struct StripEpilogue {
  const float* bias = nullptr;
  const void* residual = nullptr;
  int r_lowp = 0;
  long ldr = 0;
  float alpha = 1.f;
  int out_f32 = 0;
  float* col_stats = nullptr;
  int frag_major = 0;
};
bool attention_strip_frag_major_ok(int dtype, int n, int d);
int launch_attention_strip(int dtype, const void* q, long ldq, const void* k, long ldk, const void* vt, long ldvt, void* out, long ldo,
                           int B, int n, int d, float scale, hipStream_t s, const StripEpilogue* ep = nullptr);

struct SmallConvArgs {
  int dtype = DT_F16;
  const void* A = nullptr;
  int B = 0, H = 0, W = 0, C = 0, N = 0;
  const void* Wt = nullptr;
  long ldw = 0;
  int w_fm = 0;
  const void* X0 = nullptr; const void* X1 = nullptr;
  int CX0 = 0, CX1 = 0;
  const float* bias = nullptr;
  const float* bias_bn = nullptr;
  long ld_bn = 0;
  const void* R = nullptr;
  float alpha = 1.f;
  void* out = nullptr;
  int out_f32 = 0;
  float* col_stats = nullptr;
  void* normed = nullptr;
  const float* gn_gamma = nullptr; const float* gn_beta = nullptr;
  int groups = 0, gn_silu = 0;
  float gn_eps = 1e-6f;
};
extern bool g_small_conv;

struct StEntryArgs {
  int dtype = DT_F16;
  int B = 0, n = 0, C = 0;
  const void* x = nullptr;
  const float* cstats = nullptr;
  const float* gn_gamma = nullptr; const float* gn_beta = nullptr; int groups = 0; float gn_eps = 1e-6f;
  const void* w_in = nullptr; const float* b_in = nullptr;
  const float* ln_gamma = nullptr; const float* ln_beta = nullptr; float ln_eps = 1e-5f;
  const void* res = nullptr;
  const void* w_qkv = nullptr;
  int n2 = 0;
  const float* b2 = nullptr;
  int geglu = 0;
  const void* w3 = nullptr; const float* b3 = nullptr; const void* res3 = nullptr; void* y = nullptr; float* y_stats = nullptr;
  float* zero = nullptr; long zero_n = 0;
  void* t = nullptr;
  void* qkv = nullptr;
};
struct AttnProjArgs {
  int dtype = DT_F16;
  int B = 0, n = 0, C = 0;
  long npad = 0;
  const void* x = nullptr; const float* cstats = nullptr;
  const float* gn_gamma = nullptr; const float* gn_beta = nullptr; int groups = 0; float gn_eps = 1e-6f;
  const void* w_qk = nullptr; const float* b_qk = nullptr;
  const void* w_v = nullptr;
  void* qk = nullptr; void* vt = nullptr;
  void* k_fm = nullptr;
};
bool attn_proj_eligible(const AttnProjArgs& a);
int launch_attn_proj(const AttnProjArgs& a, hipStream_t s);
extern bool g_st_fuse;
extern bool g_small_conv_fm;
extern bool g_attn_proj;
extern bool g_attn_fm;
extern int g_st_tail_rows;
extern bool g_st_ffpo;
extern bool g_st_tail;
bool st_entry_eligible(const StEntryArgs& a);
int launch_st_entry(const StEntryArgs& a, hipStream_t s);
int launch_sf_frag_major(int dtype, const void* W, void* out, int N, int K, hipStream_t s);
bool small_conv_eligible(const SmallConvArgs& a);
int launch_small_conv_gn(const SmallConvArgs& a, hipStream_t s);

int launch_convert(const float* in, void* out, int dtype, long n, hipStream_t s);
int launch_widen(const void* in, int dtype, float* out, long n, hipStream_t s);
int launch_gather_label(const int* labels, const int* step_counter, const float* table, float* out, int B, int N,
                        hipStream_t s, const int* label_table = nullptr);
int launch_apply_mask(float* x, const unsigned char* mask, const float* x_initial, long n, hipStream_t s);
int launch_put_known(float* x, const unsigned char* known, const float* data, long n, hipStream_t s);
int launch_decode6d(const float* x, int B, int C, int L, float* clipped, float* absval, int* lengths, hipStream_t s);
int launch_encode6d(const float* xyz, const int* nres, const unsigned char* atom_ok, int B, int C, int L, const int* blocks, const int* pairs,
                    int npairs, float* coords_6d, unsigned char* mask_pair, hipStream_t s);
int launch_embedding_gather(const void* table, int dtype, const int* ids, float* out, long ntok, int dim, int vocab, int* bad, hipStream_t s);

enum { WP_COPY = 0, WP_ROWS = 1, WP_CONV3 = 2, WP_CONV3_T = 3, WP_NIN = 4, WP_GEGLU = 5, WP_UP4 = 6, WP_ADD = 7, WP_PRODUCT = 8, WP_DOT64 = 9 };
struct WeightPack {
  int kind = WP_COPY;
  const float* src[3] = {nullptr, nullptr, nullptr};
  void* dst = nullptr;
  int64_t d[6] = {0, 0, 0, 0, 0, 0};
  int dtype = DT_F32;
};
int weight_pack_shape(WeightPack& p, int64_t* rows, int64_t* width, int64_t* ld);
int launch_weight_pack(const WeightPack& p, hipStream_t s);
void weight_pack_bytes(const WeightPack& p, int64_t rows, int64_t width, int64_t* bytes_read, int64_t* bytes_written);

}
```

text2protein_amd/csrc/weightpack.hip:

```cpp
#include <algorithm>

#include "t2p_kernels.h"

#pragma clang fp contract(off)

namespace t2p {
namespace {

constexpr int CT = 256;
constexpr int NT = 64;
constexpr int PT = 32;

inline int wp_grid(long n, int per_block = 256) { return (int)std::min<long>((n + per_block - 1) / per_block, 4096); }

template <typename T>
__global__ __launch_bounds__(256) void wp_copy_kernel(const float* __restrict__ s0, long n0, const float* __restrict__ s1, long n1,
                                                      const float* __restrict__ s2, long n2, T* __restrict__ dst) {
  const long n = n0 + n1 + n2;
  for (long i = (long)blockIdx.x * 256 + threadIdx.x; i < n; i += (long)gridDim.x * 256) {
    const float v = i < n0 ? s0[i] : (i < n0 + n1 ? s1[i - n0] : s2[i - n0 - n1]);
    dst[i] = from_f32<T>(v);
  }
}
template <typename T>
// ... 222 lines not shown
      break;
    case WP_ROWS:
      T2P_REQUIRE(d[0] > 0 && d[1] > 0 && (d[2] == 0 || d[2] >= d[1]), "weight_pack rows: rows, rowlen > 0, ld >= rowlen");
      if (!d[2]) d[2] = d[1];
      R = d[0]; W = d[1]; L = d[2];
      break;
    case WP_CONV3:
      T2P_REQUIRE(d[0] > 0 && d[0] <= 65535 && d[1] > 0 && (d[2] == 0 || d[2] >= d[1]), "weight_pack conv3: N, Ci > 0, cin_pad >= Ci");
      if (!d[2]) d[2] = d[1];
      T2P_REQUIRE(d[3] == 0 || d[3] >= 9 * d[2], "weight_pack conv3: ld >= 9 * cin_pad");
      if (!d[3]) d[3] = 9 * d[2];
      R = d[0]; W = 9 * d[2]; L = d[3];
      break;
    case WP_CONV3_T:
      T2P_REQUIRE(d[0] > 0 && d[1] > 0 && d[1] <= 32, "weight_pack conv3_t: N > 0, 0 < C <= 32");
      W = 9 * d[0] * d[1];
      break;
    case WP_NIN:
      T2P_REQUIRE(d[0] > 0 && d[1] > 0 && (d[2] == 1 || d[2] == 2), "weight_pack nin: K, N > 0, one or two sources");
      nsrc = (int)d[2]; W = d[2] * d[0] * d[1];
      break;
    case WP_GEGLU:
      T2P_REQUIRE(d[0] > 0 && d[1] > 0, "weight_pack geglu: inner, rowlen > 0");
      W = 2 * d[0] * d[1];
      break;
    case WP_UP4:
      T2P_REQUIRE(d[0] > 0 && d[0] <= 65535 && d[1] > 0, "weight_pack up4: co, ci > 0");
      W = 16 * d[0] * d[1];
      break;
    case WP_ADD:
      T2P_REQUIRE(d[0] > 0, "weight_pack add: n > 0");
      nsrc = 2; W = d[0];
      break;
    case WP_PRODUCT: {
      T2P_REQUIRE(d[0] > 0 && d[1] > 0 && d[2] > 0 && (d[3] == 0 || d[3] == 1), "weight_pack product: M, K, N > 0, transposed 0 / 1");
      R = d[3] ? d[2] : d[0]; W = d[3] ? d[0] : d[2];
      T2P_REQUIRE(d[4] == 0 || d[4] >= W, "weight_pack product: ld >= row width");
      if (!d[4]) d[4] = W;
      L = d[4]; nsrc = 2;
      break;
    }
    case WP_DOT64:
      T2P_REQUIRE(d[0] > 0 && d[1] > 0, "weight_pack dot64: N, K > 0");
      nsrc = 3; W = d[0];
      break;
    default:
      T2P_REQUIRE(false, "weight_pack: unknown kind");
  }
  for (int i = 0; i < nsrc; ++i) T2P_REQUIRE(p.src[i], "weight_pack: null source");
  T2P_REQUIRE(p.dst, "weight_pack: null destination");
  T2P_REQUIRE(p.dtype == DT_F32 || p.dtype == DT_F16 || p.dtype == DT_BF16, "weight_pack: bad dtype");
  *rows = R; *width = W; *ld = L ? L : W;
  return T2P_OK;
}

void weight_pack_bytes(const WeightPack& p, int64_t rows, int64_t width, int64_t* rd, int64_t* wr) {
  const int64_t* d = p.d;
  int64_t n = 0;
  switch (p.kind) {
    case WP_COPY: n = d[0] + d[1] + d[2]; break;
    case WP_ROWS: n = d[0] * d[1]; break;
    case WP_CONV3: case WP_CONV3_T: case WP_UP4: n = d[0] * d[1] * 9; break;
    case WP_NIN: n = d[0] * d[1] * d[2]; break;
    case WP_GEGLU: n = 2 * d[0] * d[1]; break;
    case WP_ADD: n = 2 * d[0]; break;
    case WP_PRODUCT: n = d[0] * d[1] + d[1] * d[2] + (p.src[2] ? d[2] : 0); break;
    case WP_DOT64: n = d[0] * d[1] + d[1] + d[0]; break;
  }
  *rd = 4 * n;
  *wr = rows * width * (int64_t)dtype_size(p.dtype);
}

int launch_weight_pack(const WeightPack& pack, hipStream_t s) {
  WeightPack p = pack;
  int64_t rows, width, ld;
  T2P_TRY(weight_pack_shape(p, &rows, &width, &ld));
  switch (p.dtype) {
    case DT_F32: return launch_typed<float>(p, s);
    case DT_BF16: return launch_typed<bf16_t>(p, s);
    default: return launch_typed<f16_t>(p, s);
  }
}

}
```

Before: 0.6474 samples/s.

## Add row-resident MFMA GEMM for K=512 transformer linears with fragment-major weights

Adds a new GEMM kernel where each 512-thread block keeps a 128-row slab of A resident in LDS and walks all 64-column output slices. It streams weights that were pre-packed at load time into a fragment-major layout, with bias, residual and GEGLU epilogues. The engine packs these weights for the K=512 transformer linears and uses the kernel when the planner judges it worthwhile (large M, single split, a particular DMA plan geometry). The aim is to avoid re-reading A per column tile and to make weight loads cheap. The cost is extra weight memory, a new code path and planner heuristics that may rarely trigger.

```diff
diff --git a/include/t2p.h b/include/t2p.h
--- a/include/t2p.h
+++ b/include/t2p.h
@@ -198,6 +198,7 @@
                 void* stream);
 int t2p_op_gemm_r16(int dtype, const void* A, int a_f32, const void* Bw, void* C, int c_f32, int M, int N, int K, int64_t lda,
                     int64_t ldb, int64_t ldc, const float* bias_n, const void* residual16, float alpha, void* stream);
+int t2p_op_gemm_geglu(int dtype, const void* A, const void* Bw, void* C, int M, int N, int K, int64_t ldc, const float* bias_n, void* stream);
 int t2p_op_conv3x3(int dtype, const void* x, int a_f32, const void* w, const float* bias, float* out, int batch,
                    int H, int W, int Cin, int Cout, int upsample, void* stream);
 int t2p_op_conv3x3_shortcut(int dtype, const void* a, const void* w, const float* bias, const void* x0, int CX0,
@@ -294,6 +295,7 @@
 
 int t2p_profile_begin(void);
 int t2p_debug_set(int key, int value);
+int64_t t2p_debug_rowres_launches(void);
 int t2p_built_with_ablation(void);
 int t2p_profile_end(double* out9);
 int t2p_profile_dominant(double* out4, char* name, int name_len);
diff --git a/text2protein_amd/_lib.py b/text2protein_amd/_lib.py
--- a/text2protein_amd/_lib.py
+++ b/text2protein_amd/_lib.py
@@ -122,6 +122,7 @@
                              _i, _i, _i, _vp]),
     "t2p_op_input_conv": (_i, [_vp, _vp, _vp, _vp, _i, _i, _i, _i, _i, _i, _vp, _vp]),
     "t2p_op_gemm_r16": (_i, [_i, _vp, _i, _vp, _vp, _i, _i, _i, _i, _i64, _i64, _i64, _vp, _vp, _f, _vp]),
+    "t2p_op_gemm_geglu": (_i, [_i, _vp, _vp, _vp, _i, _i, _i, _i64, _vp, _vp]),
     "t2p_op_conv3x3": (_i, [_i, _vp, _i, _vp, _vp, _vp, _i, _i, _i, _i, _i, _i, _vp]),
     "t2p_op_groupnorm": (_i, [_vp, _vp, _i, _i, _i, _i, _i, _i, _vp, _vp, _f, _i, _i, _vp, _i, _vp]),
     "t2p_op_layernorm": (_i, [_vp, _vp, _vp, _vp, _i, _i64, _i, _f, _vp]),
@@ -139,6 +140,7 @@
     "t2p_op_philox_normal": (_i, [_vp, _i64, _u64, _u64, _vp]),
     "t2p_profile_begin": (_i, []),
     "t2p_debug_set": (_i, [_i, _i]),
+    "t2p_debug_rowres_launches": (_i64, []),
     "t2p_op_decode_6d": (_i, [_vp, _i, _i, _i, _vp, _vp, _vp, _vp]),
     "t2p_op_encode_6d": (_i, [_vp, _vp, _vp, _i, _i, _i, _vp, _i, _vp, _vp, _vp]),
     "t2p_op_embedding_gather": (_i, [_vp, _i, _vp, _vp, _i64, _i, _i, _vp, _vp]),
diff --git a/text2protein_amd/build.py b/text2protein_amd/build.py
--- a/text2protein_amd/build.py
+++ b/text2protein_amd/build.py
@@ -9,10 +9,10 @@
 CSRC = os.path.join(os.path.dirname(os.path.abspath(__file__)), "csrc")
 LIB = os.path.join(CSRC, "libt2p_hip.so")
 LIB_ABLATION = os.path.join(CSRC, "libt2p_hip_ablation.so")
-SOURCES = ["gemm.hip", "kernels.hip", "attention.hip", "smallconv.hip", "stfuse.hip", "ddim.hip", "weightpack.hip", "engine.cpp", "sampler.cpp", "capi.cpp",
+SOURCES = ["gemm.hip", "rowgemm.hip", "kernels.hip", "attention.hip", "smallconv.hip", "stfuse.hip", "ddim.hip", "weightpack.hip", "engine.cpp", "sampler.cpp", "capi.cpp",
            "train_kernels.hip", "train.cpp", "train_capi.cpp"]
 GEMM_PARTS = 7
-HEADERS = ["t2p_common.h", "t2p_kernels.h", "philox.h", "update_loop.h", "engine.h", "sampler.h", "ddim.h", "train_kernels.h", "train.h", os.path.join("..", "..", "include", "t2p.h")]
+HEADERS = ["t2p_common.h", "t2p_kernels.h", "gemm_mfma.h", "philox.h", "update_loop.h", "engine.h", "sampler.h", "ddim.h", "train_kernels.h", "train.h", os.path.join("..", "..", "include", "t2p.h")]
 ARCH = "gfx950"
 
 
diff --git a/text2protein_amd/csrc/capi.cpp b/text2protein_amd/csrc/capi.cpp
--- a/text2protein_amd/csrc/capi.cpp
+++ b/text2protein_amd/csrc/capi.cpp
@@ -317,12 +317,39 @@
   API_END
 }
 
+static void* g_op_rf = nullptr;
+static size_t g_op_rf_alloc = 0;
+static int attach_op_rowres(GemmParams& p, hipStream_t stream) {
+  if (!gemm_rowres_planned(p) || p.ldb < 512 || p.ldb % 8 != 0) return T2P_OK;
+  const size_t bytes = (size_t)p.N * 1024;
+  if (g_op_rf_alloc < bytes) {
+    if (g_op_rf) { T2P_HIP_CHECK(hipDeviceSynchronize()); T2P_HIP_CHECK(hipFree(g_op_rf)); g_op_rf = nullptr; g_op_rf_alloc = 0; }
+    T2P_HIP_CHECK(hipMalloc(&g_op_rf, bytes));
+    g_op_rf_alloc = bytes;
+  }
+  T2P_TRY(launch_rowres_pack(p.dtype, p.Bw, p.ldb, g_op_rf, p.N, stream));
+  p.Bw_rf = g_op_rf;
+  return T2P_OK;
+}
+
 int t2p_op_gemm(int dtype, const void* A, int a_f32, const void* Bw, void* C, int c_f32, int M, int N, int K, int64_t lda,
                 int64_t ldb, int64_t ldc, const float* bias_n, const float* residual, float alpha, void* stream) {
   API_BEGIN
   GemmParams p;
   p.dtype = dtype; p.A0 = A; p.a_f32 = a_f32; p.C0 = K; p.lda0 = lda; p.Bw = Bw; p.ldb = ldb; p.M = M; p.N = N;
   p.bias_n = bias_n; p.R = residual; p.ldr = ldc; p.alpha = alpha; p.C = C; p.c_f32 = c_f32; p.ldc = ldc;
+  T2P_TRY(attach_op_rowres(p, (hipStream_t)stream));
+  return launch_gemm(p, (hipStream_t)stream);
+  API_END
+}
+
+int t2p_op_gemm_geglu(int dtype, const void* A, const void* Bw, void* C, int M, int N, int K, int64_t ldc, const float* bias_n, void* stream) {
+  API_BEGIN
+  GemmParams p;
+  p.dtype = dtype; p.A0 = A; p.a_f32 = 0; p.C0 = K; p.lda0 = K; p.Bw = Bw; p.ldb = K; p.M = M; p.N = N;
+  p.bias_n = bias_n; p.C = C; p.c_f32 = 0; p.ldc = ldc; p.geglu = 1;
+  T2P_REQUIRE(gemm_fuses_geglu(p), "gemm_geglu: the product does not take the fused GEGLU epilogue (16-bit LDS-DMA plans, N % 4 == 0, ldc % 2 == 0)");
+  T2P_TRY(attach_op_rowres(p, (hipStream_t)stream));
   return launch_gemm(p, (hipStream_t)stream);
   API_END
 }
@@ -347,6 +374,7 @@
   p.dtype = dtype; p.A0 = A; p.a_f32 = a_f32; p.C0 = K; p.lda0 = lda; p.Bw = Bw; p.ldb = ldb; p.M = M; p.N = N;
   p.bias_n = bias_n; p.R = (const float*)residual16; p.r_lowp = 1; p.ldr = ldc; p.alpha = alpha; p.C = C; p.c_f32 = c_f32; p.ldc = ldc;
   T2P_TRY(attach_op_ws(p));
+  T2P_TRY(attach_op_rowres(p, (hipStream_t)stream));
   return launch_gemm(p, (hipStream_t)stream);
   API_END
 }
@@ -838,6 +866,8 @@
   return launch_apply_mask(x, mask, x_initial, n, (hipStream_t)stream);
   API_END
 }
+
+int64_t t2p_debug_rowres_launches(void) { return (int64_t)t2p::g_rowres_launches; }
 
 int t2p_debug_set(int key, int value) {
   if (key == 10) { g_op_ws_bytes = (size_t)value << 20; return T2P_OK; }
@@ -867,6 +897,11 @@
   if (key == 46) { t2p::g_attn_proj = value != 0; return T2P_OK; }
   if (key == 47) { set_gemm_dxs(value != 0); return T2P_OK; }
   if (key == 48) { t2p::g_train_plumbing16 = value != 0; return T2P_OK; }
+  if (key == 49) {
+    if (value < 0 || value > 2) { set_last_error("plan switch 49 takes 0 (off), 1 (the planner's choice) or 2 (wherever eligible)"); return T2P_ERR_INVALID; }
+    t2p::g_rowres = value;
+    return T2P_OK;
+  }
   if (key == 34) { set_gemm_a_norm(value != 0); return T2P_OK; }
   if (key == 32) { g_attn_merged = value != 0; return T2P_OK; }
   if (key == 33) { g_ffpo_merged = value != 0; return T2P_OK; }
diff --git a/text2protein_amd/csrc/engine.cpp b/text2protein_amd/csrc/engine.cpp
--- a/text2protein_amd/csrc/engine.cpp
+++ b/text2protein_amd/csrc/engine.cpp
@@ -512,6 +512,12 @@
   return launch_sf_frag_major(cfg_.compute_dtype, w, *slot, N, K, pack_stream_);
 }
 
+int Engine::pack_rowres(DevLinear* l) {
+  T2P_TRY(dest(&l->w_rf, (size_t)l->N * l->K * 2));
+  load_stats_[0] += (int64_t)l->N * l->K * 2; load_stats_[1] += (int64_t)l->N * l->K * 2; load_stats_[2] += 1;
+  return launch_rowres_pack(cfg_.compute_dtype, l->w, l->K, l->w_rf, l->N, pack_stream_);
+}
+
 int Engine::pack_linear(const std::string& wname, const std::string& bname, int N, int K, DevLinear* out, bool conv3x3, bool nin,
                         int force_dtype, int cin_pad) {
   const int dt = force_dtype >= 0 ? force_dtype : cfg_.compute_dtype;
@@ -690,6 +696,10 @@
           T2P_TRY(pack_frag(&l.fm_ff1, l.ff1.w, 8 * ci, ci));
         }
       }
+      if (dt != DT_F32 && ci == 512) {
+        for (DevLinear* pl : {&l.proj_in, &l.a1_qkv, &l.a1_out, &l.a2_q, &l.a2_out, &l.ff1})
+          if (pl->w && pl->K == 512 && pl->N % 64 == 0) T2P_TRY(pack_rowres(pl));
+      }
       if (dt != DT_F32 && ci % 64 == 0) {
         T2P_SRC(wpo, p + ".proj_out.weight", (int64_t)ci * ci);
         T2P_SRC(bpo, p + ".proj_out.bias", ci);
@@ -795,7 +805,7 @@
   GemmParams p;
   p.dtype = dtype();
   p.A0 = a; p.a_f32 = a_is_f32 || p.dtype == DT_F32; p.C0 = w.K; p.lda0 = w.K;
-  p.Bw = w.w; p.ldb = w.K;
+  p.Bw = w.w; p.ldb = w.K; p.Bw_rf = w.w_rf;
   p.M = (int)rows; p.N = w.N;
   p.bias_n = use_bias ? w.b : nullptr;
   p.R = residual; p.ldr = w.N; p.r_lowp = (residual && r_lowp) ? 1 : 0;
@@ -1361,7 +1371,7 @@
     POOL_GET(g, void*, (size_t)rows * 4 * C * es);
     GemmParams p;
     p.dtype = dt; p.A0 = ln; p.a_f32 = dt == DT_F32; p.C0 = C; p.lda0 = C;
-    p.Bw = L.ff1.w; p.ldb = C; p.M = (int)rows; p.N = 8 * C; p.bias_n = L.ff1.b;
+    p.Bw = L.ff1.w; p.ldb = C; p.Bw_rf = L.ff1.w_rf; p.M = (int)rows; p.N = 8 * C; p.bias_n = L.ff1.b;
     p.C = g; p.c_f32 = 0; p.ldc = 4 * C; p.geglu = 1;
     T2P_TRY(attach_ws(p));
     StEntryArgs e;
diff --git a/text2protein_amd/csrc/engine.h b/text2protein_amd/csrc/engine.h
--- a/text2protein_amd/csrc/engine.h
+++ b/text2protein_amd/csrc/engine.h
@@ -53,6 +53,7 @@
   void* w = nullptr;
   float* b = nullptr;
   int N = 0, K = 0;
+  void* w_rf = nullptr;
 };
 struct DevNorm {
   float* gamma = nullptr;
@@ -138,6 +139,7 @@
   const float* psrc(const std::string& name, int64_t numel);
   int pack(int kind, void* dst, int64_t off, int dtype, std::initializer_list<const float*> srcs, std::initializer_list<int64_t> dims);
   int pack_frag(void** slot, const void* w, int N, int K);
+  int pack_rowres(DevLinear* l);
   int pack_linear(const std::string& wname, const std::string& bname, int N, int K, DevLinear* out,
                   bool conv3x3 = false, bool nin = false, int force_dtype = -1, int cin_pad = 0);
   int pack_stack2(const std::string& w0, const std::string& b0, const std::string& w1, const std::string& b1,
diff --git a/text2protein_amd/csrc/gemm.hip b/text2protein_amd/csrc/gemm.hip
--- a/text2protein_amd/csrc/gemm.hip
+++ b/text2protein_amd/csrc/gemm.hip
@@ -8,12 +8,12 @@
 #include <vector>
 
 #include "t2p_common.h"
+#include "gemm_mfma.h"
+#include "t2p_kernels.h"
 
 namespace t2p {
 
 typedef float f32x16 __attribute__((ext_vector_type(16)));
-typedef __bf16 bf16x8_t __attribute__((ext_vector_type(8)));
-typedef _Float16 f16x8_t __attribute__((ext_vector_type(8)));
 
 [[maybe_unused]] static constexpr int ROWB = 144;
 
@@ -91,17 +91,9 @@
   }
 };
 
-typedef float f32x4_res_t __attribute__((ext_vector_type(4)));
-typedef unsigned u32x2_res_t __attribute__((ext_vector_type(2)));
 template <typename TC> __device__ inline float res_load1(const float* R, long idx, int lowp) {
   if constexpr (sizeof(TC) == 2) { if (lowp) return to_f32(((const TC*)R)[idx]); }
   return R[idx];
-}
-template <typename TC> __device__ inline f32x4_res_t unpack4(u32x2_res_t u) {
-  TC e[4];
-  e[0] = __builtin_bit_cast(TC, (uint16_t)u.x); e[1] = __builtin_bit_cast(TC, (uint16_t)(u.x >> 16));
-  e[2] = __builtin_bit_cast(TC, (uint16_t)u.y); e[3] = __builtin_bit_cast(TC, (uint16_t)(u.y >> 16));
-  return (f32x4_res_t){to_f32(e[0]), to_f32(e[1]), to_f32(e[2]), to_f32(e[3])};
 }
 template <typename TC> __device__ inline float4 res_load4(const float* R, long idx, int lowp) {
   if constexpr (sizeof(TC) == 2) {
@@ -320,49 +312,14 @@
 
 #endif
 
-typedef int v4i_t __attribute__((ext_vector_type(4)));
-typedef unsigned u32x4_t __attribute__((ext_vector_type(4)));
-#define T2P_LDS_PTR(p) ((__attribute__((address_space(3))) void*)(p))
-[[maybe_unused]] static constexpr unsigned DMA_OOB = 0x80000000u;
-
-__device__ inline float gelu_erf_fast(float g) {
-  const float x = g * 0.70710678118654752440f, ax = fabsf(x);
-  const float t = __builtin_amdgcn_rcpf(fmaf(0.3275911f, ax, 1.f));
-  float q = fmaf(t, 1.061405429f, -1.453152027f);
-  q = fmaf(q, t, 1.421413741f);
-  q = fmaf(q, t, -0.284496736f);
-  q = fmaf(q, t, 0.254829592f);
-  const float e = __builtin_amdgcn_exp2f(-ax * ax * 1.44269504088896340736f);
-  const float erf_abs = fmaf(-q * t, e, 1.f);
-  return 0.5f * g * (1.f + copysignf(erf_abs, x));
-}
-typedef unsigned u32x2_t __attribute__((ext_vector_type(2)));
-template <typename TC> __device__ inline uint32_t pack2(float a, float b) {
-  const TC x = from_f32<TC>(a), y = from_f32<TC>(b);
-  return (uint32_t)__builtin_bit_cast(uint16_t, x) | ((uint32_t)__builtin_bit_cast(uint16_t, y) << 16);
-}
+
 
 template <int I> __device__ inline void lds_read_b128(u32x4_t& dst, unsigned addr) {
   asm volatile("ds_read_b128 %0, %1 offset:%2" : "=v"(dst) : "v"(addr), "n"(I * 4096));
 }
 
-typedef float f32x4_t __attribute__((ext_vector_type(4)));
-template <typename TC> struct Mma16;
-template <> struct Mma16<bf16_t> {
-  __device__ static inline void run(const u32x4_t& a, const u32x4_t& b, f32x4_t& c) {
-    c = __builtin_amdgcn_mfma_f32_16x16x32_bf16(__builtin_bit_cast(bf16x8_t, a), __builtin_bit_cast(bf16x8_t, b), c, 0, 0, 0);
-  }
-};
-template <> struct Mma16<f16_t> {
-  __device__ static inline void run(const u32x4_t& a, const u32x4_t& b, f32x4_t& c) {
-    c = __builtin_amdgcn_mfma_f32_16x16x32_f16(__builtin_bit_cast(f16x8_t, a), __builtin_bit_cast(f16x8_t, b), c, 0, 0, 0);
-  }
-};
 #if T2P_PART_DMA
 __device__ inline bool g_stagger_dbg(int dbg) { return (dbg & 128) == 0; }
-template <int I> __device__ inline void lds_read_b128_2k(u32x4_t& dst, unsigned addr) {
-  asm volatile("ds_read_b128 %0, %1 offset:%2" : "=v"(dst) : "v"(addr), "n"(I * 2048));
-}
 template <int I> __device__ inline void lds_read_b128_1k(u32x4_t& dst, unsigned addr) {
   asm volatile("ds_read_b128 %0, %1 offset:%2" : "=v"(dst) : "v"(addr), "n"(I * 1024));
 }
@@ -455,13 +412,6 @@
 }
 
 
-__device__ __forceinline__ __amdgpu_buffer_rsrc_t make_rsrc(const void* base, int bytes) {
-  const unsigned long long b = (unsigned long long)base;
-  const unsigned lo = __builtin_amdgcn_readfirstlane((unsigned)b);
-  const unsigned hi = __builtin_amdgcn_readfirstlane((unsigned)(b >> 32));
-  const int nb = __builtin_amdgcn_readfirstlane(bytes);
-  return __builtin_amdgcn_make_buffer_rsrc((void*)(((unsigned long long)hi << 32) | lo), 0, nb, 0x00020000);
-}
 
 template <typename TC, int BM, int BN, int WM, int WN, bool MF16, int TI, int TJ>
 __device__ __forceinline__ void dma_epilogue(const GemmParams& p, unsigned char* smem, f32x16 (&acc)[MF16 ? 1 : TI][MF16 ? 1 : TJ],
@@ -671,10 +621,6 @@
   }
 }
 
-__device__ __forceinline__ int hperm(int rho) {
-  const int j = rho >> 4, g = (rho >> 2) & 3, v = rho & 3;
-  return 32 * (j >> 1) + 8 * g + 4 * (j & 1) + v;
-}
 __device__ __forceinline__ float row16_sum(float x) {
   x += __builtin_bit_cast(float, __builtin_amdgcn_update_dpp(0, __builtin_bit_cast(int, x), 0xB1, 0xF, 0xF, false));
   x += __builtin_bit_cast(float, __builtin_amdgcn_update_dpp(0, __builtin_bit_cast(int, x), 0x4E, 0xF, 0xF, false));
@@ -2381,6 +2327,13 @@
   return launch_thin_conv_ch<TC, 128>(a, stream);
 }
 
+bool gemm_rowres_planned(const GemmParams& p) {
+  if (!g_rowres || g_dbg || !dma_eligible(p) || !gemm_rowres_eligible(p)) return false;
+  const DmaPlan plan = dma_plan(p);
+  if (plan.nsplit != 1) return false;
+  return g_rowres == 2 || (p.M / 128 >= 128 && plan.geom == 1 && g_dma_ring == 2);
+}
+
 int launch_gemm(const GemmParams& p, hipStream_t stream) {
   const int vec = p.dtype == DT_F32 ? 4 : 8;
   const int Ctot = p.C0 + p.C1;
@@ -2441,6 +2394,23 @@
       T2P_HIP_CHECK(hipEventRecord(rec.a, stream));
     }
     const int rc = p.dtype == DT_BF16 ? launch_thin_conv<bf16_t>(p, stream) : launch_thin_conv<f16_t>(p, stream);
+    if (g_prof_on) {
+      T2P_HIP_CHECK(hipEventRecord(rec.b, stream));
+      g_prof.push_back(rec);
+    }
+    return rc;
+  }
+  if (p.Bw_rf && gemm_rowres_planned(p)) {
+    ProfRec rec;
+    if (g_prof_on) {
+      T2P_HIP_CHECK(hipEventCreate(&rec.a));
+      T2P_HIP_CHECK(hipEventCreate(&rec.b));
+      prof_shape(rec, p);
+      rec.flops = 2.0 * p.M * p.N * (double)p.C0; rec.kind = 1; rec.name = gemm_rowres_kernel_name(p.dtype);
+      rec.bytes = (double)p.M * p.C0 * 2 + (double)p.N * p.C0 * 2 + (double)p.M * (p.geglu ? p.N / 2 : p.N) * 2 + (p.R ? (double)p.M * p.N * 2 : 0.0);
+      T2P_HIP_CHECK(hipEventRecord(rec.a, stream));
+    }
+    const int rc = launch_gemm_rowres(p, stream);
     if (g_prof_on) {
       T2P_HIP_CHECK(hipEventRecord(rec.b, stream));
       g_prof.push_back(rec);
diff --git a/text2protein_amd/csrc/gemm_mfma.h b/text2protein_amd/csrc/gemm_mfma.h
--- /dev/null
+++ b/text2protein_amd/csrc/gemm_mfma.h
@@ -0,0 +1,68 @@
+#pragma once
+#include "t2p_common.h"
+
+namespace t2p {
+
+typedef __bf16 bf16x8_t __attribute__((ext_vector_type(8)));
+typedef _Float16 f16x8_t __attribute__((ext_vector_type(8)));
+typedef float f32x4_res_t __attribute__((ext_vector_type(4)));
+typedef unsigned u32x2_res_t __attribute__((ext_vector_type(2)));
+typedef int v4i_t __attribute__((ext_vector_type(4)));
+typedef unsigned u32x4_t __attribute__((ext_vector_type(4)));
+typedef unsigned u32x2_t __attribute__((ext_vector_type(2)));
+typedef float f32x4_t __attribute__((ext_vector_type(4)));
+#define T2P_LDS_PTR(p) ((__attribute__((address_space(3))) void*)(p))
+[[maybe_unused]] static constexpr unsigned DMA_OOB = 0x80000000u;
+
+template <typename TC> __device__ inline f32x4_res_t unpack4(u32x2_res_t u) {
+  TC e[4];
+  e[0] = __builtin_bit_cast(TC, (uint16_t)u.x); e[1] = __builtin_bit_cast(TC, (uint16_t)(u.x >> 16));
+  e[2] = __builtin_bit_cast(TC, (uint16_t)u.y); e[3] = __builtin_bit_cast(TC, (uint16_t)(u.y >> 16));
+  return (f32x4_res_t){to_f32(e[0]), to_f32(e[1]), to_f32(e[2]), to_f32(e[3])};
+}
+
+__device__ inline float gelu_erf_fast(float g) {
+  const float x = g * 0.70710678118654752440f, ax = fabsf(x);
+  const float t = __builtin_amdgcn_rcpf(fmaf(0.3275911f, ax, 1.f));
+  float q = fmaf(t, 1.061405429f, -1.453152027f);
+  q = fmaf(q, t, 1.421413741f);
+  q = fmaf(q, t, -0.284496736f);
+  q = fmaf(q, t, 0.254829592f);
+  const float e = __builtin_amdgcn_exp2f(-ax * ax * 1.44269504088896340736f);
+  const float erf_abs = fmaf(-q * t, e, 1.f);
+  return 0.5f * g * (1.f + copysignf(erf_abs, x));
+}
+template <typename TC> __device__ inline uint32_t pack2(float a, float b) {
+  const TC x = from_f32<TC>(a), y = from_f32<TC>(b);
+  return (uint32_t)__builtin_bit_cast(uint16_t, x) | ((uint32_t)__builtin_bit_cast(uint16_t, y) << 16);
+}
+
+template <typename TC> struct Mma16;
+template <> struct Mma16<bf16_t> {
+  __device__ static inline void run(const u32x4_t& a, const u32x4_t& b, f32x4_t& c) {
+    c = __builtin_amdgcn_mfma_f32_16x16x32_bf16(__builtin_bit_cast(bf16x8_t, a), __builtin_bit_cast(bf16x8_t, b), c, 0, 0, 0);
+  }
+};
+template <> struct Mma16<f16_t> {
+  __device__ static inline void run(const u32x4_t& a, const u32x4_t& b, f32x4_t& c) {
+    c = __builtin_amdgcn_mfma_f32_16x16x32_f16(__builtin_bit_cast(f16x8_t, a), __builtin_bit_cast(f16x8_t, b), c, 0, 0, 0);
+  }
+};
+template <int I> __device__ inline void lds_read_b128_2k(u32x4_t& dst, unsigned addr) {
+  asm volatile("ds_read_b128 %0, %1 offset:%2" : "=v"(dst) : "v"(addr), "n"(I * 2048));
+}
+
+__device__ __forceinline__ __amdgpu_buffer_rsrc_t make_rsrc(const void* base, int bytes) {
+  const unsigned long long b = (unsigned long long)base;
+  const unsigned lo = __builtin_amdgcn_readfirstlane((unsigned)b);
+  const unsigned hi = __builtin_amdgcn_readfirstlane((unsigned)(b >> 32));
+  const int nb = __builtin_amdgcn_readfirstlane(bytes);
+  return __builtin_amdgcn_make_buffer_rsrc((void*)(((unsigned long long)hi << 32) | lo), 0, nb, 0x00020000);
+}
+
+__host__ __device__ __forceinline__ int hperm(int rho) {
+  const int j = rho >> 4, g = (rho >> 2) & 3, v = rho & 3;
+  return 32 * (j >> 1) + 8 * g + 4 * (j & 1) + v;
+}
+
+}
diff --git a/text2protein_amd/csrc/rowgemm.hip b/text2protein_amd/csrc/rowgemm.hip
--- /dev/null
+++ b/text2protein_amd/csrc/rowgemm.hip
@@ -0,0 +1,244 @@
+#include <string>
+#include <type_traits>
+
+#include "gemm_mfma.h"
+#include "t2p_kernels.h"
+
+namespace t2p {
+
+int g_rowres = 1;
+long g_rowres_launches = 0;
+
+bool gemm_rowres_eligible(const GemmParams& p) {
+  if (p.dtype != DT_F16 && p.dtype != DT_BF16) return false;
+  if (p.a_f32 || p.c_f32 || p.taps != 1 || p.C0 != 512 || p.A1 || p.C1 || p.a_up) return false;
+  if (p.nz0 * p.nz1 != 1 || p.M % 128 != 0 || p.N % 64 != 0) return false;
+  if (p.c_frag || p.col_stats || p.gn_out || p.bias_m || p.bias_bn || p.r_up || p.c_nchw || p.X0 || p.an_stats) return false;
+  if (p.R && !p.r_lowp) return false;
+  if (p.geglu && p.R) return false;
+  if (p.lda0 % 8 != 0 || (p.geglu ? p.ldc % 4 != 0 : p.ldc % 8 != 0) || (p.R && p.ldr % 8 != 0)) return false;
+  const long lim = (1L << 31) - 64;
+  const long c_cols = p.geglu ? p.N / 2 : p.N;
+  if ((long)p.M * p.lda0 * 2 >= lim || ((long)(p.M - 1) * p.ldc + c_cols) * 2 >= lim || (p.R && ((long)(p.M - 1) * p.ldr + p.N) * 2 >= lim)) return false;
+  if ((long)p.N * 1024 >= lim) return false;
+  return true;
+}
+
+#define T2P_RR_RD4(F, ADDR, I0)                                                                     \
+  lds_read_b128_2k<I0>(F[0], ADDR); lds_read_b128_2k<I0 + 1>(F[1], ADDR);                            \
+  lds_read_b128_2k<I0 + 2>(F[2], ADDR); lds_read_b128_2k<I0 + 3>(F[3], ADDR);
+#define T2P_RR_W4(N, X)                                                                             \
+  asm volatile("s_waitcnt lgkmcnt(%4)" : "+v"(X[0]), "+v"(X[1]), "+v"(X[2]), "+v"(X[3]) : "n"(N));
+#define T2P_RR_M16(A, B, I0)                                                                        \
+  _Pragma("unroll") for (int i = 0; i < 4; ++i) _Pragma("unroll") for (int j = 0; j < 4; ++j)       \
+      Mma16<TC>::run(B[j], A[i], acc[I0 + i][j]);
+
+template <typename TC>
+__global__ __launch_bounds__(512) void gemm_rowres_kernel(const GemmParams p) {
+  constexpr int NKT = 8;
+  constexpr int ASTAGE = 128 * 128;
+  extern __shared__ __attribute__((aligned(16))) unsigned char smem[];
+
+  const int tid = threadIdx.x, lane = tid & 63;
+  const int wave = __builtin_amdgcn_readfirstlane(tid >> 6);
+  const int m0 = blockIdx.x * 128;
+  const int nslices = p.N >> 6;
+
+  const __amdgpu_buffer_rsrc_t rA = make_rsrc(p.A0, (int)((((long)p.M - 1) * p.lda0 + 512) * 2));
+  const int prow = lane >> 3, ppos = lane & 7;
+  unsigned a_off[2];
+#pragma unroll
+  for (int j = 0; j < 2; ++j) {
+    const int r = (wave * 2 + j) * 8 + prow;
+    a_off[j] = (unsigned)(m0 + r) * (unsigned)(p.lda0 * 2) + (unsigned)((ppos ^ ((r >> 1) & 7)) * 16);
+  }
+  auto issue_a = [&](int kt) __attribute__((always_inline)) {
+#pragma unroll
+    for (int j = 0; j < 2; ++j) {
+      unsigned char* dst = smem + kt * ASTAGE + (wave * 2 + j) * 1024;
+      __builtin_amdgcn_raw_ptr_buffer_load_lds(rA, T2P_LDS_PTR(dst), 16, a_off[j] + (unsigned)(kt * 128), 0, 0, 0);
+    }
+  };
+
+  const __amdgpu_buffer_rsrc_t rB = make_rsrc(p.Bw_rf, (int)((long)p.N * 1024));
+  const unsigned b_lane = (unsigned)lane * 16u;
+  u32x4_t Bf[2][2][4];
+  auto load_b = [&](auto SLOT, int slice, int kt) __attribute__((always_inline)) {
+    constexpr int slot = decltype(SLOT)::value;
+    const unsigned vo = slice < nslices ? b_lane + (unsigned)((slice * 16 + kt * 2) * 4096) : DMA_OOB;
+#pragma unroll
+    for (int ks = 0; ks < 2; ++ks)
+#pragma unroll
+      for (int j = 0; j < 4; ++j) Bf[slot][ks][j] = __builtin_amdgcn_raw_buffer_load_b128(rB, vo + (unsigned)(ks * 4096 + j * 1024), 0, 0);
+  };
+
+  const unsigned lds_base = (unsigned)(unsigned long long)T2P_LDS_PTR(smem);
+  unsigned a16[2];
+  {
+    const int r = lane & 15, g = lane >> 4;
+#pragma unroll
+    for (int ks = 0; ks < 2; ++ks) a16[ks] = lds_base + (unsigned)(r * 128 + (((4 * ks + g) ^ ((r >> 1) & 7)) << 4));
+  }
+
+  f32x4_t acc[8][4];
+  auto ktile = [&](auto SLOT, int kt) __attribute__((always_inline)) {
+    constexpr int slot = decltype(SLOT)::value;
+    u32x4_t AL[4], AH[4];
+    const unsigned aa0 = a16[0] + (unsigned)(kt * ASTAGE), aa1 = a16[1] + (unsigned)(kt * ASTAGE);
+    T2P_RR_RD4(AL, aa0, 0)
+    T2P_RR_RD4(AH, aa0, 4)
+    T2P_RR_W4(4, AL)
+    T2P_RR_M16(AL, Bf[slot][0], 0)
+    T2P_RR_RD4(AL, aa1, 0)
+    T2P_RR_W4(4, AH)
+    T2P_RR_M16(AH, Bf[slot][0], 4)
+    T2P_RR_RD4(AH, aa1, 4)
+    T2P_RR_W4(4, AL)
+    T2P_RR_M16(AL, Bf[slot][1], 0)
+    T2P_RR_W4(0, AH)
+    T2P_RR_M16(AH, Bf[slot][1], 4)
+  };
+
+  const long c_cols = p.geglu ? p.N / 2 : p.N;
+  const __amdgpu_buffer_rsrc_t rC = make_rsrc(p.C, (int)((((long)p.M - 1) * p.ldc + c_cols) * 2));
+  const __amdgpu_buffer_rsrc_t rR = make_rsrc(p.R ? (const void*)p.R : (const void*)p.C, p.R ? (int)((((long)p.M - 1) * p.ldr + p.N) * 2) : 0);
+  const bool has_r = p.R != nullptr, geglu = p.geglu != 0;
+  const float alpha = p.alpha;
+  const unsigned ldc_e = (unsigned)p.ldc, ldr_e = (unsigned)p.ldr;
+  auto epilogue = [&](int slice) __attribute__((always_inline)) {
+    int tx = threadIdx.x;
+    asm volatile("" : "+v"(tx));
+    const int l16 = tx & 15, g4 = (tx & 63) >> 4;
+    const int col0 = slice * 64 + 8 * g4;
+    float bs[16];
+#pragma unroll
+    for (int k = 0; k < 16; ++k) bs[k] = 0.f;
+    if (p.bias_n) {
+#pragma unroll
+      for (int h = 0; h < 2; ++h)
+#pragma unroll
+        for (int q = 0; q < 2; ++q) {
+          const float4 t = *(const float4*)(p.bias_n + col0 + 32 * h + 4 * q);
+          const int k = 8 * h + 4 * q;
+          bs[k] = t.x; bs[k + 1] = t.y; bs[k + 2] = t.z; bs[k + 3] = t.w;
+        }
+    }
+    float bm = 0.f;
+    asm volatile("" : "+v"(bm));
+    auto half = [&](auto HC) __attribute__((always_inline)) {
+      constexpr int i0 = 4 * decltype(HC)::value;
+      u32x4_t rr[4][2];
+      if (has_r) {
+#pragma unroll
+        for (int i = 0; i < 4; ++i)
+#pragma unroll
+          for (int h = 0; h < 2; ++h)
+            rr[i][h] = __builtin_amdgcn_raw_buffer_load_b128(rR, ((unsigned)(m0 + 16 * (i0 + i) + l16) * ldr_e + (unsigned)(col0 + 32 * h)) * 2u, 0, 0);
+      }
+#pragma unroll
+      for (int i = 0; i < 4; ++i) {
+        const unsigned row = (unsigned)(m0 + 16 * (i0 + i) + l16);
+        float v[16];
+#pragma unroll
+        for (int j = 0; j < 4; ++j)
+#pragma unroll
+          for (int e = 0; e < 4; ++e) v[4 * j + e] = acc[i0 + i][j][e];
+        if (geglu) {
+#pragma unroll
+          for (int k = 0; k < 16; ++k) v[k] += bm + bs[k];
+#pragma unroll
+          for (int h = 0; h < 2; ++h) {
+            const float* w = v + 8 * h;
+            __builtin_amdgcn_raw_buffer_store_b64((u32x2_t){pack2<TC>(w[0] * gelu_erf_fast(w[1]), w[2] * gelu_erf_fast(w[3])),
+                                                             pack2<TC>(w[4] * gelu_erf_fast(w[5]), w[6] * gelu_erf_fast(w[7]))},
+                                                  rC, (row * ldc_e + (unsigned)((col0 + 32 * h) >> 1)) * 2u, 0, 0);
+          }
+          continue;
+        }
+#pragma unroll
+        for (int k = 0; k < 16; ++k) v[k] += bs[k];
+        if (has_r) {
+#pragma unroll
+          for (int h = 0; h < 2; ++h) {
+            const f32x4_res_t a = unpack4<TC>((u32x2_res_t){rr[i][h][0], rr[i][h][1]}), b = unpack4<TC>((u32x2_res_t){rr[i][h][2], rr[i][h][3]});
+#pragma unroll
+            for (int e = 0; e < 4; ++e) { v[8 * h + e] += a[e]; v[8 * h + 4 + e] += b[e]; }
+          }
+        }
+        if (alpha != 1.0f) {
+#pragma unroll
+          for (int k = 0; k < 16; ++k) v[k] *= alpha;
+        }
+#pragma unroll
+        for (int h = 0; h < 2; ++h) {
+          const float* w = v + 8 * h;
+          const u32x4_t packed = {pack2<TC>(w[0], w[1]), pack2<TC>(w[2], w[3]), pack2<TC>(w[4], w[5]), pack2<TC>(w[6], w[7])};
+          __builtin_amdgcn_raw_buffer_store_b128(packed, rC, (row * ldc_e + (unsigned)(col0 + 32 * h)) * 2u, 0, 0);
+        }
+      }
+    };
+    half(std::integral_constant<int, 0>{});
+    half(std::integral_constant<int, 1>{});
+  };
+  auto zero_acc = [&]() __attribute__((always_inline)) {
+#pragma unroll
+    for (int i = 0; i < 8; ++i)
+#pragma unroll
+      for (int j = 0; j < 4; ++j) acc[i][j] = f32x4_t{0.f, 0.f, 0.f, 0.f};
+  };
+  using S0 = std::integral_constant<int, 0>; using S1 = std::integral_constant<int, 1>;
+
+  zero_acc();
+  issue_a(0); issue_a(1);
+  load_b(S0{}, wave, 0);
+  issue_a(2);
+  load_b(S1{}, wave, 1);
+#pragma unroll
+  for (int kt = 0; kt < NKT; ++kt) {
+    if (kt <= 5) asm volatile("s_waitcnt vmcnt(10)" ::: "memory");
+    else if (kt == 6) asm volatile("s_waitcnt vmcnt(8)" ::: "memory");
+    else asm volatile("s_waitcnt vmcnt(0)" ::: "memory");
+    __builtin_amdgcn_s_barrier();
+    if (kt & 1) ktile(S1{}, kt); else ktile(S0{}, kt);
+    if (kt + 3 < NKT) issue_a(kt + 3);
+    if (kt + 2 < NKT) { if (kt & 1) load_b(S1{}, wave, kt + 2); else load_b(S0{}, wave, kt + 2); }
+  }
+  if (wave < nslices) epilogue(wave);
+
+  for (int slice = wave + 8; slice < nslices; slice += 8) {
+    zero_acc();
+    load_b(S0{}, slice, 0);
+    load_b(S1{}, slice, 1);
+#pragma unroll
+    for (int kt = 0; kt < NKT; ++kt) {
+      if (kt & 1) ktile(S1{}, kt); else ktile(S0{}, kt);
+      if (kt + 2 < NKT) { if (kt & 1) load_b(S1{}, slice, kt + 2); else load_b(S0{}, slice, kt + 2); }
+    }
+    epilogue(slice);
+  }
+}
+#undef T2P_RR_RD4
+#undef T2P_RR_W4
+#undef T2P_RR_M16
+
+template <typename TC>
+static int launch_rowres_t(const GemmParams& p, hipStream_t stream) {
+  constexpr int smem = 8 * 128 * 128;
+  auto kern = gemm_rowres_kernel<TC>;
+  T2P_TRY(ensure_dynamic_lds((const void*)kern, smem));
+  hipLaunchKernelGGL(kern, dim3(p.M / 128), dim3(512), smem, stream, p);
+  T2P_HIP_CHECK(hipGetLastError());
+  return T2P_OK;
+}
+
+const char* gemm_rowres_kernel_name(int dtype) { return dtype == DT_F16 ? "gemm_rowres_kernel<f16_t>" : "gemm_rowres_kernel<bf16_t>"; }
+
+int launch_gemm_rowres(const GemmParams& p, hipStream_t stream) {
+  T2P_REQUIRE(gemm_rowres_eligible(p) && p.Bw_rf, "row-resident GEMM: not eligible (ask gemm_rowres_eligible) or no fragment-major weights");
+  T2P_REQUIRE(((uintptr_t)p.A0 % 16) == 0 && ((uintptr_t)p.Bw_rf % 16) == 0 && ((uintptr_t)p.C % 16) == 0 && ((uintptr_t)p.R % 16) == 0 &&
+              ((uintptr_t)p.bias_n % 16) == 0, "row-resident GEMM: operands must be 16-byte aligned");
+  ++g_rowres_launches;
+  return p.dtype == DT_BF16 ? launch_rowres_t<bf16_t>(p, stream) : launch_rowres_t<f16_t>(p, stream);
+}
+
+}
diff --git a/text2protein_amd/csrc/t2p_common.h b/text2protein_amd/csrc/t2p_common.h
--- a/text2protein_amd/csrc/t2p_common.h
+++ b/text2protein_amd/csrc/t2p_common.h
@@ -128,8 +128,13 @@
   void* c_frag = nullptr;
   int frag_col0 = 0, frag_ns = 0;
   long frag_bstride = 0;
+  const void* Bw_rf = nullptr;
 };
 bool gemm_writes_frag_major(const GemmParams& p);
+bool gemm_rowres_eligible(const GemmParams& p);
+bool gemm_rowres_planned(const GemmParams& p);
+extern long g_rowres_launches;
+extern int g_rowres;
 
 int launch_gemm(const GemmParams& p, hipStream_t stream);
 bool gemm_fuses_col_stats(const GemmParams& p);
diff --git a/text2protein_amd/csrc/t2p_kernels.h b/text2protein_amd/csrc/t2p_kernels.h
--- a/text2protein_amd/csrc/t2p_kernels.h
+++ b/text2protein_amd/csrc/t2p_kernels.h
@@ -198,6 +198,9 @@
 bool st_entry_eligible(const StEntryArgs& a);
 int launch_st_entry(const StEntryArgs& a, hipStream_t s);
 int launch_sf_frag_major(int dtype, const void* W, void* out, int N, int K, hipStream_t s);
+int launch_gemm_rowres(const GemmParams& p, hipStream_t s);
+const char* gemm_rowres_kernel_name(int dtype);
+int launch_rowres_pack(int dtype, const void* W, long ldb, void* out, int N, hipStream_t s);
 bool small_conv_eligible(const SmallConvArgs& a);
 int launch_small_conv_gn(const SmallConvArgs& a, hipStream_t s);
 
diff --git a/text2protein_amd/csrc/weightpack.hip b/text2protein_amd/csrc/weightpack.hip
--- a/text2protein_amd/csrc/weightpack.hip
+++ b/text2protein_amd/csrc/weightpack.hip
@@ -328,4 +328,21 @@
   }
 }
 
-}
+__global__ __launch_bounds__(256) void rowres_pack_kernel(const uint4* __restrict__ W, long ldb8, uint4* __restrict__ out, long npieces) {
+  const long i = (long)blockIdx.x * 256 + threadIdx.x;
+  if (i >= npieces) return;
+  const int lane = (int)(i & 63), j = (int)((i >> 6) & 3), step = (int)((i >> 8) & 15);
+  const long slice = i >> 12;
+  const int r = lane & 15, ch = 32 * (j >> 1) + 8 * (r >> 2) + 4 * (j & 1) + (r & 3);
+  out[i] = W[(slice * 64 + ch) * ldb8 + 4 * step + (lane >> 4)];
+}
+int launch_rowres_pack(int dtype, const void* W, long ldb, void* out, int N, hipStream_t s) {
+  T2P_REQUIRE(W && out && N > 0 && N % 64 == 0 && ldb >= 512 && ldb % 8 == 0 && (dtype == DT_F16 || dtype == DT_BF16), "rowres_pack arguments");
+  T2P_REQUIRE(((uintptr_t)W % 16) == 0 && ((uintptr_t)out % 16) == 0, "rowres_pack: 16-byte aligned matrices");
+  const long n = (long)N * 64;
+  hipLaunchKernelGGL(rowres_pack_kernel, dim3((unsigned)((n + 255) / 256)), dim3(256), 0, s, (const uint4*)W, ldb / 8, (uint4*)out, n);
+  T2P_HIP_CHECK(hipGetLastError());
+  return T2P_OK;
+}
+
+}
```

New measurement: 0.6552 samples/s (median of 6 runs). 1.01x the previous value.
